# KangWelly/Assignment-for-AAE6102_GNSS-SDR

Hardware: AMD Instinct MI355X
Metric: correlator Msamples/s (acq+track), whole job (higher is better)
Workload: dtype int8 in; acquisition: f64 correlation + f64 fine search; tracking: f64

## Files before the change

### assignment-for-aae6102_gnss-sdr_amd/abi.py

```python
from __future__ import annotations

import ctypes as C
import os
import sys

MAX_SV = 64
MAX_TAPS = 32

OK, ENODATA, EIO, EARG, EDEVICE, EINDEX = 0, 1, 2, 3, 4, 5

FIELDS = ["P_i", "P_q", "E_i", "E_q", "L_i", "L_q", "PLLdiscri", "DLLdiscri", "codedelay",
          "remChip", "codeFreq", "carrierFreq", "remPhase", "remSample", "numSample",
          "delayValue", "absoluteSample", "codedelay2"]
NFIELDS = len(FIELDS)
OUT_DEVICE = 1
FIELDS_POS = ["P_i", "P_q", "E_i", "E_q", "L_i", "L_q", "carrError", "codeError", "codedelay",
              "remChip", "codeFreq", "carrFreq", "remCarrPhase", "absoluteSampleCodedelay",
              "numSample", "delayValue", "absoluteSample", "codedelay2"]

MC_TAPS = 25
MC_TAP_NAMES = ([f"E_{{}}{s}" for s in ["_060", "_055", "", "_045", "_040", "_035", "_030", "_025",
                                         "_020", "_015", "_010", "_005"]] + ["P_{}"] +
                [f"L_{{}}{s}" for s in ["005", "010", "015", "020", "025", "030", "035", "040", "045",
                                         "", "055", "060"]])


EPH_FIELDS = ["TOW", "TOW1", "sfb", "sfb1", "weeknum", "N", "health", "IODC", "TGD", "toc", "af2",
              "af1", "af0", "IODE2", "Crs", "deltan", "M0", "Cuc", "ecc", "Cus", "sqrta", "toe", "Cic",
              "omegae", "Cis", "i0", "Crc", "w", "omegadot", "IODE3", "idot", "updatetime",
              "updatetime_tow"]
EPH_NFIELDS = len(EPH_FIELDS)


class GnssNavOut(C.Structure):
    _fields_ = [("eph_cap", C.c_int32), ("eph", C.POINTER(C.c_double)),
                ("eph_len", C.POINTER(C.c_int32)), ("updateflag", C.POINTER(C.c_int32)),
                ("nav1", C.POINTER(C.c_int64)), ("sfb1", C.POINTER(C.c_int64))]


class GnssFile(C.Structure):
    _fields_ = [("path", C.c_char_p), ("data", C.c_void_p), ("dev_data", C.c_void_p),
                ("nbytes", C.c_uint64), ("skip", C.c_int64), ("dataType", C.c_int32),
                ("dataPrecision", C.c_int32)]


class GnssSignal(C.Structure):
    _fields_ = [("IF", C.c_double), ("Fs", C.c_double), ("codeFreqBasis", C.c_double),
                ("ms", C.c_double), ("Sample", C.c_int64), ("codelength", C.c_double)]


class GnssAcq(C.Structure):
    _fields_ = [("freqNum", C.c_int32), ("freqMin", C.c_double), ("freqStep", C.c_double),
                ("datalen", C.c_int32), ("L", C.c_int32), ("n_prn", C.c_int32),
                ("prn_list", C.POINTER(C.c_int32))]


class GnssAcquired(C.Structure):
    _fields_ = [("n", C.c_int32), ("sv", C.c_int32 * MAX_SV), ("SNR", C.c_double * MAX_SV),
                ("Doppler", C.c_double * MAX_SV), ("codedelay", C.c_int32 * MAX_SV),
                ("fineFreq", C.c_double * MAX_SV)]


class GnssAcqDiag(C.Structure):
    _fields_ = [("n", C.c_int32), ("prn", C.c_int32 * MAX_SV), ("SNR", C.c_double * MAX_SV),
                ("fbin", C.c_int32 * MAX_SV), ("codePhase", C.c_int32 * MAX_SV),
                ("peak", C.c_double * MAX_SV), ("peak2", C.c_double * MAX_SV)]


class GnssTrack(C.Structure):
    _fields_ = [("CorrelatorSpacing", C.c_double), ("DLLBW", C.c_double), ("DLLDamp", C.c_double),
                ("DLLGain", C.c_double), ("PLLBW", C.c_double), ("PLLDamp", C.c_double),
                ("PLLGain", C.c_double), ("msToProcessCT_1ms", C.c_int32),
                ("msToProcessCT_10ms", C.c_int32), ("n_taps", C.c_int32),
                ("tap_offsets", C.POINTER(C.c_double)), ("n_chan", C.c_int32),
                ("chan", C.POINTER(C.c_int32))]


class GnssTrackOut(C.Structure):
    _fields_ = [("max_len", C.c_int64), ("rec", C.POINTER(C.c_double)),
                ("taps", C.POINTER(C.c_double)), ("len", C.POINTER(C.c_int64)),
                ("countinx", C.POINTER(C.c_int32)), ("CN0_Eph", C.POINTER(C.c_double)),
                ("cn0_cap", C.c_int32), ("cn0_rows", C.c_int32), ("flags", C.c_int32),
                ("reserved", C.c_int32)]


class GnssTiming(C.Structure):
    _fields_ = [("acq_ms", C.c_double), ("acq_corr_ms", C.c_double), ("acq_fine_ms", C.c_double),
                ("track_ms", C.c_double), ("track_kernel_ms", C.c_double),
                ("track_launches", C.c_int64), ("track_channel_samples", C.c_int64),
                ("acq_hypothesis_samples", C.c_int64), ("h2d_ms", C.c_double),
                ("track10_kernel_ms", C.c_double), ("track10_launches", C.c_int64),
                ("track10_channel_samples", C.c_int64), ("h2d_bytes", C.c_int64),
                ("track_segments", C.c_int64)]


class GnssVtChan(C.Structure):
    _fields_ = [("prn", C.c_int32), ("pad", C.c_int32), ("file_ptr", C.c_int64), ("remChip", C.c_double),
                ("remCarrPhase", C.c_double), ("codeFreq", C.c_double), ("carrFreq", C.c_double),
                ("carrFreqBasis", C.c_double), ("oldCarrNco", C.c_double), ("oldCarrError", C.c_double),
                ("index_int", C.c_int32), ("snrIndex", C.c_int32), ("Zk", C.c_double * 20)]


class GnssVtOut(C.Structure):
    _fields_ = [(f, C.c_double) for f in ("E_i", "E_q", "P_i", "P_q", "L_i", "L_q", "carrError", "codeError",
                                          "carrNco", "remChip", "remCarrPhase", "codeFreq", "carrFreq")] + \
               [("numSample", C.c_int64), ("absoluteSample", C.c_int64), ("codedelay", C.c_double),
                ("CN0", C.c_double), ("cn0_row", C.c_int32), ("status", C.c_int32),
                ("deltaPr", C.c_double), ("prRate", C.c_double), ("sv_vel", C.c_double * 3)]


class GnssVtMcOut(C.Structure):
    _fields_ = GnssVtOut._fields_ + [("tap_i", C.c_double * MC_TAPS), ("tap_q", C.c_double * MC_TAPS)]


ADDED_STRUCTS = {"gnss_vt_mc_out": "GnssVtMcOut"}

VT_MAX_CH = 32
EPH_SV_FIELDS = ["sqrta", "deltan", "toe", "M0", "ecc", "w", "Cus", "Cuc", "Crs", "Crc", "Cis", "Cic", "i0",
                 "idot", "omegae", "omegadot", "toc", "af0", "af1", "af2", "TGD"]
GEO_XYZ2LLH, GEO_LLH2XYZ, GEO_XYZ2ENU, GEO_EROTCORR, GEO_IONO, GEO_TROP = range(6)


class GnssEphSv(C.Structure):
    _fields_ = [(f, C.c_double) for f in EPH_SV_FIELDS]


class GnssVtNavCfg(C.Structure):
    _fields_ = [("cnslxyz", C.c_double * 3), ("ALPHA", C.c_double * 4), ("BETA", C.c_double * 4),
                ("doy", C.c_double), ("cSpeed", C.c_double), ("Fc", C.c_double)]


class GnssVtNav(C.Structure):
    _fields_ = [("n", C.c_int32), ("pdi", C.c_int32), ("msIndex", C.c_int32), ("counterUptR", C.c_int32),
                ("counter_r", C.c_int32), ("prn", C.c_int32 * VT_MAX_CH), ("cfg", GnssVtNavCfg),
                ("Fs", C.c_double), ("IF", C.c_double), ("codeFreqBasis", C.c_double), ("ms", C.c_double),
                ("cnslxyz", C.c_double * 3), ("total_state", C.c_double * 8), ("state_cov", C.c_double * 64),
                ("R", C.c_double * (2 * VT_MAX_CH)), ("recordR2", C.c_double * (2 * VT_MAX_CH))] + \
               [(f, C.c_double * VT_MAX_CH) for f in ("transmitTime", "tot_est_tck", "predictedPr_last",
                                                     "counter_corr", "ionodel", "tropodel", "el", "az")] + \
               [("numSample", C.c_int64 * VT_MAX_CH), ("eph", GnssEphSv * VT_MAX_CH)]


class GnssVtNavSol(C.Structure):
    _fields_ = [("localTime", C.c_double)] + \
               [(f, C.c_double * 3) for f in ("usrPos", "usrVel", "usrPosENU", "usrVelENU", "usrPosLLH")] + \
               [("clkBias", C.c_double), ("clkDrift", C.c_double), ("state", C.c_double * 8),
                ("state_cov", C.c_double * 8), ("newZ", C.c_double * (2 * VT_MAX_CH)),
                ("meas_inno", C.c_double * (2 * VT_MAX_CH)), ("satEA", C.c_double * VT_MAX_CH),
                ("satAZ", C.c_double * VT_MAX_CH), ("predicted_z", C.c_double * (2 * VT_MAX_CH)),
                ("satePos", C.c_double * 3), ("sateVel", C.c_double * 3),
                ("svxyz_pos", (C.c_double * 3) * VT_MAX_CH), ("kalman_gain", (C.c_double * (2 * VT_MAX_CH)) * 8),
                ("R", C.c_double * (2 * VT_MAX_CH)), ("r_row", C.c_int32),
                ("reserved", C.c_int32)]


ENOCONV = 6
CT_POS_UPDATED, CT_POS_MULTICORR = 0, 1
NAVSOL_CT_FIELDS = [("rawPseudorange", 0), ("usrPos", 3), ("usrVel", 3), ("usrPosENU", 3), ("usrPosLLH", 3),
                    ("clkBias", 1), ("usrVelENU", 3), ("clkDrift", 1), ("DOP", 4), ("satEA", 0), ("satAZ", 0),
                    ("timeTransmit", 0), ("codePhaseMeas", 0), ("localTime", 1)]


class GnssCtPosCfg(C.Structure):
    _fields_ = [("n", C.c_int32), ("mode", C.c_int32), ("dataType", C.c_int32), ("msToProcessCT_1ms", C.c_int32),
                ("pdi", C.c_int32), ("reserved", C.c_int32), ("navSolPeriod", C.c_double), ("Fs", C.c_double),
                ("IF", C.c_double), ("codelength", C.c_double), ("ms", C.c_double), ("cSpeed", C.c_double),
                ("doy", C.c_double), ("cnslxyz", C.c_double * 3), ("ALPHA", C.c_double * 4),
                ("BETA", C.c_double * 4), ("countinx", C.c_int32 * VT_MAX_CH), ("nav1", C.c_int64 * VT_MAX_CH),
                ("sfb1", C.c_int64 * VT_MAX_CH), ("sampleStart", C.c_int64 * VT_MAX_CH),
                ("TOW1", C.c_double * VT_MAX_CH), ("eph", GnssEphSv * VT_MAX_CH)]


class GnssNavSolCt(C.Structure):
    _fields_ = [("cap", C.c_int64), ("rows", C.c_int64)] + \
               [(f, C.POINTER(C.c_double)) for f, _ in NAVSOL_CT_FIELDS] + \
               [("Index", C.POINTER(C.c_int64)), ("index", C.POINTER(C.c_int64)),
                ("carrFreqMeas", C.POINTER(C.c_double)), ("iters", C.POINTER(C.c_int32))]


ADDED_STRUCTS.update({"gnss_ct_pos_cfg": "GnssCtPosCfg", "gnss_nav_sol_ct": "GnssNavSolCt"})

ACF_DEFAULTS = dict(ind_start=1, numOverLap=100, corrSpacing=0.05, maxDelay=0.6,
                    a=(4092.9779845217, 340.423503277404, -2.99026922880033, 0.0251763660254827))
ACF_FIELDS = ["meanMax", "F1", "F2", "varDelay", "meanCodeDisc", "varCodeDisc"]


class GnssAcfCfg(C.Structure):
    _fields_ = [("n", C.c_int32), ("ind_start", C.c_int32), ("numOverLap", C.c_int32), ("reserved", C.c_int32),
                ("corrSpacing", C.c_double), ("maxDelay", C.c_double), ("a", C.c_double * 4),
                ("prn", C.c_int32 * VT_MAX_CH), ("ele", C.c_double * VT_MAX_CH)]


class GnssAcfOut(C.Structure):
    _fields_ = [("cap", C.c_int64), ("windows", C.POINTER(C.c_int64))] + \
               [(f, C.POINTER(C.c_double)) for f in ACF_FIELDS] + \
               [("maxCorrInd", C.c_void_p), ("corr", C.c_void_p)]


ADDED_STRUCTS.update({"gnss_acf_cfg": "GnssAcfCfg", "gnss_acf_out": "GnssAcfOut"})


class GnssSynthSv(C.Structure):
    _fields_ = [("prn", C.c_int32), ("doppler_hz", C.c_double), ("code_phase0", C.c_double),
                ("carr_phase0", C.c_double), ("cn0_dbhz", C.c_double), ("bit_seed", C.c_uint64),
                ("bit_phase_chips", C.c_double), ("lnav", C.c_int32), ("reserved", C.c_int32)]


class GnssSynth(C.Structure):
    _fields_ = [("Fs", C.c_double), ("IF", C.c_double), ("noise_sigma", C.c_double),
                ("seed", C.c_uint64), ("n_sv", C.c_int32), ("sv", GnssSynthSv * MAX_SV)]


MAX_RAYS = 128


class GnssSynthRay(C.Structure):
    _fields_ = [("sv", C.c_int32), ("reserved", C.c_int32), ("delay_chips", C.c_double), ("gain", C.c_double),
                ("phase0_cycles", C.c_double), ("fade_hz", C.c_double), ("t_on", C.c_uint64),
                ("t_off", C.c_uint64)]


class GnssSynthScene(C.Structure):
    _fields_ = [("Fs", C.c_double), ("IF", C.c_double), ("noise_sigma", C.c_double),
                ("seed", C.c_uint64), ("n_sv", C.c_int32), ("sv", GnssSynthSv * MAX_SV),
                ("los_gain", C.c_double * MAX_SV), ("n_ray", C.c_int32), ("ray", GnssSynthRay * MAX_RAYS)]


ADDED_STRUCTS.update({"gnss_synth_ray": "GnssSynthRay", "gnss_synth_scene": "GnssSynthScene"})


PROTOTYPES = {
    "gnss_abi_version": (C.c_int, []),
    "gnss_strerror": (C.c_char_p, [C.c_int]),
    "gnss_ctx_create": (C.c_int, [C.c_int, C.POINTER(C.c_void_p)]),
    "gnss_ctx_create_multi": (C.c_int, [C.POINTER(C.c_int), C.c_int, C.POINTER(C.c_void_p)]),
    "gnss_ctx_members": (C.c_int, [C.c_void_p]),
    "gnss_ctx_drop_record": (C.c_int, [C.c_void_p, C.c_void_p]),
    "gnss_ctx_resident_records": (C.c_int, [C.c_void_p]),
    "gnss_device_count": (C.c_int, []),
    "gnss_ctx_destroy": (None, [C.c_void_p]),
    "gnss_last_error": (C.c_char_p, [C.c_void_p]),
    "gnss_last_timing": (C.c_int, [C.c_void_p, C.POINTER(GnssTiming)]),
    "gnss_ctx_set_profiling": (C.c_int, [C.c_void_p, C.c_int]),
    "gnss_ctx_set_acq_precision": (C.c_int, [C.c_void_p, C.c_int]),
    "gnss_ctx_set_window": (C.c_int, [C.c_void_p, C.c_uint64]),
    "gnss_ctx_set_option": (C.c_int, [C.c_void_p, C.c_int, C.c_int64]),
    "gnss_dev_alloc": (C.c_int, [C.c_void_p, C.c_uint64, C.POINTER(C.c_void_p)]),
    "gnss_dev_free": (C.c_int, [C.c_void_p, C.c_void_p]),
    "gnss_dev_upload": (C.c_int, [C.c_void_p, C.c_void_p, C.c_void_p, C.c_uint64]),
    "gnss_dev_download": (C.c_int, [C.c_void_p, C.c_void_p, C.c_void_p, C.c_uint64]),
    "gnss_acquisition": (C.c_int, [C.c_void_p, C.POINTER(GnssFile), C.POINTER(GnssSignal),
                                   C.POINTER(GnssAcq), C.POINTER(GnssAcquired),
                                   C.POINTER(GnssAcqDiag)]),
    "gnss_tracking_ct": (C.c_int, [C.c_void_p, C.POINTER(GnssFile), C.POINTER(GnssSignal),
                                   C.POINTER(GnssTrack), C.POINTER(GnssAcquired),
                                   C.POINTER(GnssTrackOut)]),
    "gnss_tracking_ct_pos": (C.c_int, [C.c_void_p, C.POINTER(GnssFile), C.POINTER(GnssSignal),
                                       C.POINTER(GnssTrack), C.POINTER(GnssAcquired), C.c_int32,
                                       C.POINTER(C.c_int32), C.POINTER(GnssTrackOut)]),
    "gnss_tracking_ct_mc": (C.c_int, [C.c_void_p, C.POINTER(GnssFile), C.POINTER(GnssSignal),
                                      C.POINTER(GnssTrack), C.POINTER(GnssAcquired), C.c_int32,
                                      C.c_int32, C.POINTER(GnssTrackOut)]),
    "gnss_tracking_ct_multicorr": (C.c_int, [C.c_void_p, C.POINTER(GnssFile), C.POINTER(GnssSignal),
                                             C.POINTER(GnssTrack), C.POINTER(GnssAcquired), C.c_int32,
                                             C.POINTER(GnssTrackOut)]),
    "gnss_navi_decode": (C.c_int, [C.POINTER(GnssAcquired), C.POINTER(C.c_double),
                                   C.POINTER(C.c_int64), C.c_int64, C.POINTER(GnssNavOut)]),
    "gnss_lnav_bits": (C.c_int, [C.c_int32, C.c_int32, C.c_void_p]),
    "gnss_ca_code": (C.c_int, [C.c_int, C.c_void_p]),
    "gnss_correlate_step": (C.c_int, [C.c_void_p, C.POINTER(GnssFile), C.POINTER(GnssSignal),
                                      C.c_int, C.c_int, C.c_double, C.c_double, C.c_double,
                                      C.c_double, C.c_int64, C.c_int, C.POINTER(C.c_double),
                                      C.POINTER(C.c_double), C.POINTER(C.c_int64)]),
    "gnss_synth_if_device": (C.c_int, [C.c_void_p, C.POINTER(GnssSynth), C.c_uint64, C.c_uint64,
                                       C.c_void_p]),
    "gnss_synth_scene_device": (C.c_int, [C.c_void_p, C.POINTER(GnssSynthScene), C.c_uint64, C.c_uint64,
                                          C.c_void_p]),
    "gnss_synth_scene_host": (C.c_int, [C.POINTER(GnssSynthScene), C.c_uint64, C.c_uint64, C.c_void_p, C.c_int]),
    "gnss_tracking_vt_run": (C.c_int, [C.c_void_p, C.POINTER(GnssFile), C.POINTER(GnssSignal),
                                       C.POINTER(GnssTrack), C.c_int32, C.c_int32, C.c_int32,
                                       C.POINTER(GnssVtChan), C.POINTER(C.c_double), C.POINTER(GnssVtOut)]),
    "gnss_tracking_vt_step": (C.c_int, [C.c_void_p, C.POINTER(GnssFile), C.POINTER(GnssSignal),
                                        C.POINTER(GnssTrack), C.c_int32, C.c_int32, C.POINTER(GnssVtChan),
                                        C.POINTER(C.c_double), C.POINTER(GnssVtOut)]),
    "gnss_vt_nco_step": (C.c_int, [C.POINTER(GnssSignal), C.POINTER(GnssTrack), C.c_int32,
                                   C.POINTER(GnssVtChan), C.c_double, C.c_double, C.c_double,
                                   C.POINTER(GnssVtOut)]),
    "gnss_vt_prepare": (C.c_int, [C.POINTER(GnssSignal), C.c_int32, C.POINTER(GnssVtChan), C.c_double,
                                  C.POINTER(C.c_int32), C.POINTER(C.c_int64)]),
    "gnss_sv_pos_vel": (C.c_int, [C.POINTER(GnssEphSv), C.c_double, C.POINTER(C.c_double),
                                  C.POINTER(C.c_double), C.POINTER(C.c_double), C.POINTER(C.c_double),
                                  C.POINTER(C.c_double)]),
    "gnss_geo": (C.c_int, [C.c_int, C.POINTER(C.c_double), C.POINTER(C.c_double)]),
    "gnss_vt_nav_init": (C.c_int, [C.POINTER(GnssVtNavCfg), C.POINTER(GnssSignal), C.c_int32, C.c_int32,
                                   C.POINTER(C.c_int32), C.POINTER(GnssEphSv), C.POINTER(C.c_double),
                                   C.POINTER(C.c_double), C.c_double, C.c_double, C.POINTER(C.c_double),
                                   C.POINTER(GnssVtNav)]),
    "gnss_vt_nav_predict": (C.c_int, [C.POINTER(GnssVtNav), C.c_int32, C.c_int64, C.POINTER(C.c_double),
                                      C.POINTER(C.c_double), C.POINTER(C.c_double)]),
    "gnss_vt_nav_update": (C.c_int, [C.POINTER(GnssVtNav), C.POINTER(C.c_double), C.POINTER(C.c_double),
                                     C.POINTER(C.c_double), C.POINTER(GnssVtNavSol)]),
    "gnss_tracking_vt": (C.c_int, [C.c_void_p, C.POINTER(GnssFile), C.POINTER(GnssSignal), C.POINTER(GnssTrack),
                                   C.c_int32, C.c_int32, C.POINTER(GnssVtChan), C.POINTER(GnssVtNav),
                                   C.POINTER(GnssVtOut), C.POINTER(GnssVtNavSol)]),
    "gnss_tracking_vt_mc_run": (C.c_int, [C.c_void_p, C.POINTER(GnssFile), C.POINTER(GnssSignal),
                                          C.POINTER(GnssTrack), C.c_int32, C.c_int32, C.c_int32,
                                          C.POINTER(GnssVtChan), C.POINTER(C.c_double), C.POINTER(GnssVtMcOut)]),
    "gnss_tracking_vt_mc": (C.c_int, [C.c_void_p, C.POINTER(GnssFile), C.POINTER(GnssSignal), C.POINTER(GnssTrack),
                                      C.c_int32, C.c_int32, C.POINTER(GnssVtChan), C.POINTER(GnssVtNav),
                                      C.POINTER(GnssVtMcOut), C.POINTER(GnssVtNavSol)]),
    "gnss_vt_mc_prepare": (C.c_int, [C.POINTER(GnssSignal), C.c_int32, C.POINTER(GnssVtChan), C.c_double,
                                     C.POINTER(C.c_double), C.POINTER(C.c_double), C.POINTER(C.c_int64)]),
    "gnss_vt_mc_nco_step": (C.c_int, [C.POINTER(GnssSignal), C.POINTER(GnssTrack), C.c_int32,
                                      C.POINTER(GnssVtChan), C.c_double, C.POINTER(C.c_double),
                                      C.POINTER(C.c_double), C.POINTER(GnssVtMcOut)]),
    "gnss_vt_mc_nav_update": (C.c_int, [C.POINTER(GnssVtNav), C.POINTER(C.c_double), C.POINTER(C.c_double),
                                        C.POINTER(C.c_double), C.POINTER(GnssVtNavSol)]),
    "gnss_ct_pos_solve": (C.c_int, [C.c_void_p, C.POINTER(GnssCtPosCfg), C.POINTER(GnssTrackOut),
                                    C.POINTER(GnssNavSolCt)]),
    "gnss_acf_features": (C.c_int, [C.c_void_p, C.POINTER(GnssAcfCfg), C.POINTER(GnssTrackOut), C.c_int32,
                                    C.POINTER(GnssAcfOut)]),
    "gnss_lane_boundaries": (C.c_int, [C.POINTER(C.c_double), C.POINTER(C.c_double), C.c_int, C.c_int, C.c_double]),
    "gnss_ctx_lane_path": (C.c_int, [C.c_void_p]),
}

LIB_PATH = os.path.join(os.path.dirname(os.path.abspath(__file__)), "lib", "libgnss_mi355x.so")
_lib = None
_torch_first = False
LOADED_PATH = None

(OPT_FORCE_SUB, OPT_NO_PERSIST, OPT_FORCE_VPB, OPT_ACQ_ROCFFT, OPT_FINE_ROCFFT, OPT_ACQ_BATCH, OPT_ACQ_FUSED,
 OPT_ACQ_RING, OPT_ACQ_PIPE, OPT_VT_BLOCKS, OPT_FORCE_PEER, OPT_VT_SPAN, OPT_SLOT_PATH) = range(13)
MAX_DEVICES = 16


def require_torch():
    import torch
    if _lib is not None and not _torch_first:
        raise RuntimeError("import torch before the first gnss Context / abi.load() "
                           "(PyTorch-ROCm must bring up its HIP runtime first)")
    return torch


class GnssError(RuntimeError):
    def __init__(self, status, msg=""):
        self.status = status
        super().__init__(f"gnss status {status}: {msg}")


def load(path: str | None = None):
    global _lib
    if _lib is not None and path is None:
        return _lib
    p = path or os.environ.get("GNSS_LIB") or LIB_PATH
    if not os.path.exists(p):
        raise ImportError(f"{p} missing: the HIP extension is not built "
                          "(run `python -c 'import __graft_entry__ as g; g.build()'`)")
    global _torch_first
    if _lib is None:
        if "torch" not in sys.modules and os.environ.get("GNSS_NO_TORCH", "0") != "1":
            try:
                import torch
            except Exception:
                pass
        _torch_first = "torch" in sys.modules
    lib = C.CDLL(p)
    for name, (res, args) in PROTOTYPES.items():
        if p != LIB_PATH and not hasattr(lib, name):
            continue
        fn = getattr(lib, name)
        fn.restype = res
        fn.argtypes = args
    if path is None:
        global LOADED_PATH
        _lib = lib
        LOADED_PATH = os.path.abspath(p)
    return lib
```

### assignment-for-aae6102_gnss-sdr_amd/csrc/acq_fft.hip

```cpp
#include "gnss_internal.h"

#pragma clang fp contract(fast)

namespace gnss {

namespace {

constexpr int kRow = 2000;
constexpr int kRowPad = 2100;
constexpr int kRowThreads = 256;
constexpr int kColThreads = 256;

template <int P> struct PrimeTab;
template <> struct PrimeTab<13> {
    static constexpr double c[13] = {1.0, 0.8854560256532099, 0.5680647467311559, 0.120536680255323, -0.35460488704253545, -0.7485107481711012, -0.970941817426052, -0.9709418174260521, -0.7485107481711013, -0.3546048870425359, 0.1205366802553232, 0.5680647467311548, 0.88545602565321};
    static constexpr double s[13] = {0.0, 0.4647231720437685, 0.8229838658936564, 0.992708874098054, 0.9350162426854148, 0.6631226582407952, 0.23931566428755768, -0.23931566428755743, -0.663122658240795, -0.9350162426854147, -0.992708874098054, -0.822983865893657, -0.4647231720437684};
};
template <> struct PrimeTab<29> {
    static constexpr double c[29] = {1.0, 0.9766205557100867, 0.907575419670957, 0.7960930657056438, 0.6473862847818277, 0.46840844069979015, 0.26752833852922075, 0.05413890858541761, -0.16178199655276473, -0.37013815533991423, -0.5611870653623823, -0.7259954919231306, -0.8568571761675893, -0.9476531711828025, -0.9941379571543596, -0.9941379571543597, -0.9476531711828025, -0.8568571761675892, -0.7259954919231311, -0.5611870653623825, -0.37013815533991445, -0.16178199655276476, 0.0541389085854167, 0.2675283385292201, 0.4684084406997903, 0.6473862847818279, 0.796093065705644, 0.9075754196709569, 0.9766205557100867};
    static constexpr double s[29] = {0.0, 0.21497044021102407, 0.4198891015602646, 0.6051742151937652, 0.7621620551276365, 0.8835120444460229, 0.963549992519223, 0.9985334138511238, 0.9868265225415261, 0.9289767198167915, 0.8276889981568906, 0.6876994588534235, 0.5155538571770216, 0.3193015301359798, 0.10811901842394192, -0.10811901842394124, -0.31930153013597995, -0.5155538571770218, -0.6876994588534231, -0.8276889981568905, -0.9289767198167914, -0.9868265225415261, -0.9985334138511239, -0.9635499925192231, -0.8835120444460228, -0.7621620551276362, -0.6051742151937649, -0.41988910156026493, -0.21497044021102438};
};

template <class V> struct RealOf;
template <> struct RealOf<float2> { using T = float; };
template <> struct RealOf<double2> { using T = double; };
template <class V> using Re = typename RealOf<V>::T;

template <class V> __device__ __forceinline__ V mk(Re<V> x, Re<V> y)
{
    V r;
    r.x = x;
    r.y = y;
    return r;
}
__device__ __forceinline__ float fma2(float a, float b, float cd) { return __builtin_fmaf(a, b, cd); }
__device__ __forceinline__ double fma2(double a, double b, double cd) { return __builtin_fma(a, b, cd); }
template <class V> __device__ __forceinline__ V cadd(V a, V b) { return mk<V>(a.x + b.x, a.y + b.y); }
template <class V> __device__ __forceinline__ V csub(V a, V b) { return mk<V>(a.x - b.x, a.y - b.y); }
template <class V> __device__ __forceinline__ V cmul(V a, V b)
{
    return mk<V>(fma2(a.x, b.x, -(a.y * b.y)), fma2(a.x, b.y, a.y * b.x));
}
template <class V> __device__ __forceinline__ V cmulc(V a, V b)
{
    return mk<V>(fma2(a.x, b.x, a.y * b.y), fma2(a.y, b.x, -(a.x * b.y)));
}
template <int DIR, class V> __device__ __forceinline__ V mul_dj(V a)
{
    return DIR < 0 ? mk<V>(a.y, -a.x) : mk<V>(-a.y, a.x);
}
template <int DIR, class V> __device__ __forceinline__ V twid(V a, V tw)
{
    return DIR < 0 ? cmul(a, tw) : cmulc(a, tw);
}

template <int DIR, class V> __device__ __forceinline__ void dft4(V& a, V& b, V& c, V& d)
{
    const V t0 = cadd(a, c), t1 = csub(a, c), t2 = cadd(b, d), t3 = mul_dj<DIR>(csub(b, d));
    a = cadd(t0, t2);
    c = csub(t0, t2);
    b = cadd(t1, t3);
    d = csub(t1, t3);
}

template <int DIR, class V> __device__ __forceinline__ void dft5(V (&v)[5])
{
    using R = Re<V>;
    constexpr R c1 = (R)0.30901699437494745, c2 = (R)-0.8090169943749475;
    constexpr R s1 = (R)0.9510565162951535, s2 = (R)0.5877852522924731;
    const V t1 = cadd(v[1], v[4]), t2 = cadd(v[2], v[3]);
    const V t3 = csub(v[1], v[4]), t4 = csub(v[2], v[3]);
    const V b1 = mk<V>(v[0].x + c1 * t1.x + c2 * t2.x, v[0].y + c1 * t1.y + c2 * t2.y);
    const V b2 = mk<V>(v[0].x + c2 * t1.x + c1 * t2.x, v[0].y + c2 * t1.y + c1 * t2.y);
    const V e1 = mul_dj<DIR>(mk<V>(fma2(s1, t3.x, s2 * t4.x), fma2(s1, t3.y, s2 * t4.y)));
    const V e2 = mul_dj<DIR>(mk<V>(fma2(s2, t3.x, -(s1 * t4.x)), fma2(s2, t3.y, -(s1 * t4.y))));
    v[0] = mk<V>(v[0].x + t1.x + t2.x, v[0].y + t1.y + t2.y);
    v[1] = cadd(b1, e1);
    v[4] = csub(b1, e1);
    v[2] = cadd(b2, e2);
    v[3] = csub(b2, e2);
}

template <int DIR, class V> __device__ __forceinline__ void dft10(V (&v)[10])
{
    using R = Re<V>;
    constexpr R c[5] = {(R)1.0, (R)0.8090169943749475, (R)0.30901699437494745, (R)-0.30901699437494745,
                        (R)-0.8090169943749475};
    constexpr R s[5] = {(R)0.0, (R)0.5877852522924731, (R)0.9510565162951535, (R)0.9510565162951535,
                        (R)0.5877852522924731};
    V e[5] = {v[0], v[2], v[4], v[6], v[8]}, o[5] = {v[1], v[3], v[5], v[7], v[9]};
    dft5<DIR>(e);
    dft5<DIR>(o);
#pragma unroll
    for (int k = 0; k < 5; k++) {
        const V t = cmul(o[k], mk<V>(c[k], DIR < 0 ? -s[k] : s[k]));
        v[k] = cadd(e[k], t);
        v[k + 5] = csub(e[k], t);
    }
}

constexpr double kC16 = 0.9238795325112867, kS16 = 0.3826834323650898, kR2 = 0.7071067811865476;
constexpr double kTc16[10] = {1., kC16, kR2, kS16, 0., -kS16, -kR2, -kC16, -1., -kC16};
constexpr double kTs16[10] = {0., kS16, kR2, kC16, 1., kC16, kR2, kS16, 0., -kS16};

template <int DIR, class V> __device__ __forceinline__ void dft16(V (&v)[16])
{
    using R = Re<V>;
#pragma unroll
    for (int n2 = 0; n2 < 4; n2++) dft4<DIR>(v[n2], v[4 + n2], v[8 + n2], v[12 + n2]);
#pragma unroll
    for (int k1 = 1; k1 < 4; k1++)
#pragma unroll
        for (int n2 = 1; n2 < 4; n2++) {
            const int m = n2 * k1;
            const V w = mk<V>((R)kTc16[m], DIR < 0 ? (R)-kTs16[m] : (R)kTs16[m]);
            v[4 * k1 + n2] = cmul(v[4 * k1 + n2], w);
        }
    V o[16];
#pragma unroll
    for (int k1 = 0; k1 < 4; k1++) {
        V a = v[4 * k1], b = v[4 * k1 + 1], c = v[4 * k1 + 2], d = v[4 * k1 + 3];
        dft4<DIR>(a, b, c, d);
        o[k1] = a; o[k1 + 4] = b; o[k1 + 8] = c; o[k1 + 12] = d;
    }
#pragma unroll
    for (int i = 0; i < 16; i++) v[i] = o[i];
}

template <int P, int DIR, class V, class Put>
__device__ __forceinline__ void dft_prime(V (&v)[P], Put put)
{
    using R = Re<V>;
    constexpr int H = (P - 1) / 2;
    using T = PrimeTab<P>;
    const V x0 = v[0];
    V sum = x0;
#pragma unroll
    for (int n = 1; n <= H; n++) {
        const V a = cadd(v[n], v[P - n]), d = csub(v[n], v[P - n]);
        v[n] = a;
        v[P - n] = d;
        sum = cadd(sum, a);
    }
    put(0, sum);
#pragma unroll
    for (int k = 1; k <= H; k++) {
        R re = x0.x, im = x0.y, sr = 0, si = 0;
#pragma unroll
        for (int n = 1; n <= H; n++) {
            const int m = (n * k) % P;
            re += v[n].x * (R)T::c[m];
            im += v[n].y * (R)T::c[m];
            sr += v[P - n].y * (R)T::s[m];
            si += v[P - n].x * (R)T::s[m];
        }
        if (DIR < 0) {
            put(k, mk<V>(re + sr, im - si));
            put(P - k, mk<V>(re - sr, im + si));
        } else {
            put(k, mk<V>(re - sr, im + si));
            put(P - k, mk<V>(re + sr, im - si));
        }
    }
}

template <int DIR, int NS, class V, class TW>
__device__ __forceinline__ void stage5(V* a, const TW& tw, int tid)
{
    constexpr int NB = kRow / 5, PER = (NB + kRowThreads - 1) / kRowThreads;
    V v[PER][5];
#pragma unroll
    for (int q = 0; q < PER; q++) {
        const int j0 = tid + q * kRowThreads, j = j0 < NB ? j0 : NB - 1;
        const int k = j % NS;
#pragma unroll
        for (int i = 0; i < 5; i++) v[q][i] = a[j + i * NB];
        if (NS > 1) {
#pragma unroll
            for (int i = 1; i < 5; i++) v[q][i] = twid<DIR>(v[q][i], tw[i * k * (kRow / (NS * 5))]);
        }
        dft5<DIR>(v[q]);
    }
    __syncthreads();
#pragma unroll
    for (int q = 0; q < PER; q++) {
        const int j = tid + q * kRowThreads;
        if (j < NB) {
            const int k = j % NS, d = (j / NS) * NS * 5 + k;
#pragma unroll
            for (int i = 0; i < 5; i++) a[d + i * NS] = v[q][i];
        }
    }
    __syncthreads();
}

template <int DIR, class V, class TW>
__device__ __forceinline__ void fft2000(V* a, const TW& tw, int tid)
{
    stage5<DIR, 1>(a, tw, tid);
    stage5<DIR, 5>(a, tw, tid);
    stage5<DIR, 25>(a, tw, tid);
    constexpr int NB = kRow / 16;
    const int j = tid < NB ? tid : NB - 1;
    V v[16];
#pragma unroll
    for (int i = 0; i < 16; i++) v[i] = a[j + i * NB];
#pragma unroll
    for (int i = 1; i < 16; i++) v[i] = twid<DIR>(v[i], tw[i * j]);
    dft16<DIR>(v);
    __syncthreads();
    if (tid < NB) {
#pragma unroll
        for (int i = 0; i < 16; i++) a[tid + i * NB] = v[i];
    }
    __syncthreads();
}

constexpr double kTc20[13] = {1., 0.9510565162951535, 0.8090169943749475, 0.5877852522924731,
                              0.30901699437494745, 0., -0.30901699437494745, -0.5877852522924731,
                              -0.8090169943749475, -0.9510565162951535, -1., -0.9510565162951535,
                              -0.8090169943749475};
constexpr double kTs20[13] = {0., 0.30901699437494745, 0.5877852522924731, 0.8090169943749475,
                              0.9510565162951535, 1., 0.9510565162951535, 0.8090169943749475,
                              0.5877852522924731, 0.30901699437494745, 0., -0.30901699437494745,
                              -0.5877852522924731};
template <int DIR, class V> __device__ __forceinline__ void dft20(V (&v)[20])
{
    using R = Re<V>;
    V y[4][5];
#pragma unroll
    for (int n2 = 0; n2 < 4; n2++) {
#pragma unroll
        for (int n1 = 0; n1 < 5; n1++) y[n2][n1] = v[4 * n1 + n2];
        dft5<DIR>(y[n2]);
    }
#pragma unroll
    for (int n2 = 1; n2 < 4; n2++)
#pragma unroll
        for (int k1 = 1; k1 < 5; k1++) {
            const int m = n2 * k1;
            y[n2][k1] = cmul(y[n2][k1], mk<V>((R)kTc20[m], DIR < 0 ? (R)-kTs20[m] : (R)kTs20[m]));
        }
#pragma unroll
    for (int k1 = 0; k1 < 5; k1++) {
        V a = y[0][k1], b = y[1][k1], c = y[2][k1], d = y[3][k1];
        dft4<DIR>(a, b, c, d);
        v[k1] = a; v[k1 + 5] = b; v[k1 + 10] = c; v[k1 + 15] = d;
    }
}

template <int R, int DIR, class V> __device__ __forceinline__ void dft_r(V (&v)[R])
{
    if constexpr (R == 5) dft5<DIR>(v);
    else if constexpr (R == 10) dft10<DIR>(v);
    else if constexpr (R == 16) dft16<DIR>(v);
    else dft20<DIR>(v);
}

template <class V> struct TwIK {
    const V* t2;
    const V* t3;
};
template <int NS, class V>
__device__ __forceinline__ V tw_get(const V* tw, int, int, int m) { return tw[m]; }
template <int NS, class V>
__device__ __forceinline__ V tw_get(const TwIK<V>& tw, int i, int k, int m)
{
    static_assert(NS == 20 || NS == 200, "split twiddles: the radix-20-first stages");
    return NS == 20 ? tw.t2[(i - 1) * 20 + k] : tw.t3[(i - 1) * 200 + k];
}
constexpr int kTwIK = 9 * 20 + 9 * 200;
#ifndef GNSS_STAGED_LOADS
#define GNSS_STAGED_LOADS 1
#endif
template <class V>
__device__ __forceinline__ TwIK<V> load_row_tw_ik(V* s_t, const V* tw_row, int tid)
{
    auto src = [&](int e) {
        const bool t2 = e < 9 * 20;
        const int f = t2 ? e : e - 9 * 20;
        const int i = t2 ? f / 20 + 1 : f / 200 + 1, k = t2 ? f % 20 : f % 200;
        return t2 ? 10 * i * k : i * k;
    };
    if constexpr (GNSS_STAGED_LOADS) {
        constexpr int NIT = (kTwIK + kRowThreads - 1) / kRowThreads;
        V r[NIT];
#pragma unroll
        for (int q = 0; q < NIT; q++) {
            const int e0 = tid + q * kRowThreads;
            r[q] = tw_row[src(e0 < kTwIK ? e0 : kTwIK - 1)];
        }
#pragma unroll
        for (int q = 0; q < NIT; q++)
            if (tid + q * kRowThreads < kTwIK) s_t[tid + q * kRowThreads] = r[q];
    } else {
        for (int e = tid; e < kTwIK; e += kRowThreads) s_t[e] = tw_row[src(e)];
    }
    return TwIK<V>{s_t, s_t + 9 * 20};
}

template <int DIR, int R, int NS, int BATCH, class V, class TW, int SW = 0>
__device__ __forceinline__ void stage_batch(V* a, const TW& tw, int tid)
{
    constexpr int NB = kRow / R, TOT = NB * BATCH, PER = (TOT + kRowThreads - 1) / kRowThreads;
    static_assert(SW == 0 || (BATCH == 1 && ((SW == 1 && R == 20 && NS == 1) || (SW == 2 && R == 10 && NS == 20))),
                  "padded layout");
    V v[PER][R];
#pragma unroll
    for (int q = 0; q < PER; q++) {
        const int u0 = tid + q * kRowThreads, u = u0 < TOT ? u0 : TOT - 1;
        const int b = u / NB, j = u - b * NB, k = j % NS;
        const V* src = a + b * kRow;
        if constexpr (SW == 2) {
            const V* s0 = src + j + j / 20;
#pragma unroll
            for (int i = 0; i < R; i++) v[q][i] = s0[210 * i];
        } else {
#pragma unroll
            for (int i = 0; i < R; i++) v[q][i] = src[j + i * NB];
        }
        if constexpr (NS > 1) {
#pragma unroll
            for (int i = 1; i < R; i++) v[q][i] = twid<DIR>(v[q][i], tw_get<NS>(tw, i, k, i * k * (kRow / (NS * R))));
        }
        dft_r<R, DIR>(v[q]);
    }
    __syncthreads();
#pragma unroll
    for (int q = 0; q < PER; q++) {
        const int u = tid + q * kRowThreads;
        if (u < TOT) {
            const int b = u / NB, j = u - b * NB, k = j % NS, d = (j / NS) * NS * R + k;
            V* dst = a + b * kRow;
            if constexpr (SW == 1) {
#pragma unroll
                for (int i = 0; i < R; i++) dst[d + j + i] = v[q][i];
            } else {
#pragma unroll
                for (int i = 0; i < R; i++) dst[d + i * NS] = v[q][i];
            }
        }
    }
    __syncthreads();
}

template <int DIR, int BATCH, class V, class TW>
__device__ __forceinline__ void fft2000_batch(V* a, const TW& tw, int tid)
{
    stage_batch<DIR, 10, 1, BATCH>(a, tw, tid);
    stage_batch<DIR, 10, 10, BATCH>(a, tw, tid);
    stage_batch<DIR, 20, 100, BATCH>(a, tw, tid);
}

constexpr int kR20Out = 10;
template <int DIR, class V, class TW, class Put>
__device__ __forceinline__ void fft2000_r20first_put(V* a, const TW& tw, int tid, Put put)
{
    stage_batch<DIR, 20, 1, 1, V, TW, 1>(a, tw, tid);
    stage_batch<DIR, 10, 20, 1, V, TW, 2>(a, tw, tid);
    constexpr int R = 10, NB = kRow / R;
    const bool on = tid < NB;
    const int j = on ? tid : NB - 1;
    V v[R];
#pragma unroll
    for (int i = 0; i < R; i++) v[i] = a[j + i * NB];
#pragma unroll
    for (int i = 1; i < R; i++) v[i] = twid<DIR>(v[i], tw_get<NB>(tw, i, j, i * j));
    dft10<DIR>(v);
    if (on) {
#pragma unroll
        for (int i = 0; i < R; i++) put(i, j + i * NB, v[i]);
    }
    __syncthreads();
}

constexpr int kInvOut = kR20Out;
template <class TW>
__device__ __forceinline__ void inv_row_power_f64(double2* a, const TW& s_tw, double scale,
                                                  double (&acc)[kInvOut], int tid)
{
    fft2000_r20first_put<1>(a, s_tw, tid, [&](int i, int, double2 v) {
        acc[i] = __builtin_fma(__builtin_fma(v.x, v.x, v.y * v.y), scale, acc[i]);
    });
}

__device__ __forceinline__ double2 ld_nt(const double2* p)
{
    double2 v;
    v.x = __builtin_nontemporal_load(&p->x);
    v.y = __builtin_nontemporal_load(&p->y);
    return v;
}

template <class V>
__device__ __forceinline__ void load_row_tw(V* s_tw, const V* tw_row, int tid)
{
    for (int i = tid; i < kRow; i += kRowThreads) s_tw[i] = tw_row[i];
}


struct FwdSet {
    int nbins, nsig, nprn, bin0, nbc, codes;
    __device__ __forceinline__ int transform(int y) const
    {
        if (codes && y < nprn) return nsig + y;
        const int u = y - (codes ? nprn : 0), idx = u / nbc;
        return idx * nbins + bin0 + (u - idx * nbc);
    }
};

template <int P, class Src, class V>
__global__ __launch_bounds__(kRowThreads) void fwd_rows_kernel(
    const Src src, FwdSet fs, double IF, double freqMin, double freqStep,
    double Fs, const float* __restrict__ ca, double code_step, const V* __restrict__ tw_row,
    const V* __restrict__ tw_col, V* __restrict__ B)
{
    using R = Re<V>;
    constexpr int64_t S = (int64_t)P * kRow;
    __shared__ V s_a[kRowPad], s_tw[kTwIK];
    const int nbins = fs.nbins, nsig = fs.nsig;
    const int n2 = blockIdx.x, s = fs.transform(blockIdx.y), tid = threadIdx.x;
    const TwIK<V> twk = load_row_tw_ik(s_tw, tw_row, tid);
    constexpr int NIT = (kRow + kRowThreads - 1) / kRowThreads;
    if (s < nsig) {
        const int idx = s / nbins, bin = s - idx * nbins;
        const double f = (IF + (freqMin + freqStep * (double)bin)) / Fs;
        auto put = [&](int n1, double2 r) {
            const int64_t n = (int64_t)P * n1 + n2;
            double cyc = f * (double)(n + 1);
            cyc -= floor(cyc);
            R c, sn;
            if constexpr (sizeof(R) == 4) {
                const float ph = (float)cyc;
                c = __builtin_amdgcn_cosf(ph);
                sn = __builtin_amdgcn_sinf(ph);
            } else {
                sincospi(2.0 * cyc, &sn, &c);
            }
            const R xr = (R)r.x, xi = (R)r.y;
            s_a[n1] = mk<V>(fma2(xr, c, -(xi * sn)), fma2(xr, sn, xi * c));
        };
        if constexpr (GNSS_STAGED_LOADS) {
            double2 raw[NIT];
#pragma unroll
            for (int q = 0; q < NIT; q++) {
                const int m0 = tid + q * kRowThreads, n1 = m0 < kRow ? m0 : kRow - 1;
                raw[q] = src.at((int64_t)idx * S + (int64_t)P * n1 + n2);
            }
#pragma unroll
            for (int q = 0; q < NIT; q++)
                if (tid + q * kRowThreads < kRow) put(tid + q * kRowThreads, raw[q]);
        } else {
            for (int n1 = tid; n1 < kRow; n1 += kRowThreads) put(n1, src.at((int64_t)idx * S + (int64_t)P * n1 + n2));
        }
    } else {
        const float* cp = ca + (int64_t)(s - nsig) * 1023;
        auto chip = [&](int n1) {
            const int64_t n = (int64_t)P * n1 + n2;
            const int64_t ci = (int64_t)ceil((double)(n + 1) * code_step);
            return (ci - 1) % 1023;
        };
        if constexpr (GNSS_STAGED_LOADS) {
            float cv[NIT];
#pragma unroll
            for (int q = 0; q < NIT; q++) {
                const int m0 = tid + q * kRowThreads;
                cv[q] = cp[chip(m0 < kRow ? m0 : kRow - 1)];
            }
#pragma unroll
            for (int q = 0; q < NIT; q++)
                if (tid + q * kRowThreads < kRow) s_a[tid + q * kRowThreads] = mk<V>((R)cv[q], (R)0);
        } else {
            for (int n1 = tid; n1 < kRow; n1 += kRowThreads) s_a[n1] = mk<V>((R)cp[chip(n1)], (R)0);
        }
    }
    __syncthreads();
    V* o = B + ((int64_t)s * P + n2) * kRow;
    const V* twc = tw_col + (int64_t)n2 * kRow;
    fft2000_r20first_put<-1>(s_a, twk, tid, [&](int, int k1, V v) { o[k1] = cmul(v, twc[k1]); });
}

template <int P, class V>
__global__ __launch_bounds__(kColThreads) void fwd_cols_kernel(FwdSet fs, const V* __restrict__ B, V* __restrict__ X)
{
    const int k1 = blockIdx.x * kColThreads + threadIdx.x, s = fs.transform(blockIdx.y);
    if (k1 >= kRow) return;
    const V* b = B + (int64_t)s * P * kRow + k1;
    V v[P];
#pragma unroll
    for (int i = 0; i < P; i++) v[i] = b[(int64_t)i * kRow];
    V* x = X + (int64_t)s * P * kRow + k1;
    dft_prime<P, -1>(v, [&](int k, V y) { x[(int64_t)k * kRow] = y; });
}

template <class V> __device__ __forceinline__ V buf_ld(__amdgpu_buffer_rsrc_t r, int voff, int soff);
template <> __device__ __forceinline__ double2 buf_ld<double2>(__amdgpu_buffer_rsrc_t r, int voff, int soff)
{
    typedef unsigned u4 __attribute__((ext_vector_type(4)));
    const u4 v = __builtin_amdgcn_raw_buffer_load_b128(r, voff, soff, 0);
    return make_double2(__hiloint2double((int)v.y, (int)v.x), __hiloint2double((int)v.w, (int)v.z));
}
template <> __device__ __forceinline__ float2 buf_ld<float2>(__amdgpu_buffer_rsrc_t r, int voff, int soff)
{
    typedef unsigned u2 __attribute__((ext_vector_type(2)));
    const u2 v = __builtin_amdgcn_raw_buffer_load_b64(r, voff, soff, 0);
    return make_float2(__uint_as_float(v.x), __uint_as_float(v.y));
}
#ifndef GNSS_COLS_BUF
#define GNSS_COLS_BUF 1
#endif
#ifndef GNSS_COLS_GROUP
#define GNSS_COLS_GROUP 8
#endif
#ifndef GNSS_TW_ROWS
#define GNSS_TW_ROWS 1
#endif
#ifndef GNSS_INVCOLS_WPE
#define GNSS_INVCOLS_WPE 0
#endif
template <int P, class V>
__device__ __forceinline__ void inv_cols_body(
    int bx, int t, const V* __restrict__ C, const V* __restrict__ X, int nbins, int nprn, int datalen,
    int first_pair, const V* __restrict__ tw_col, V* __restrict__ A)
{
    const int k1 = bx * kColThreads + threadIdx.x;
    if (k1 >= kRow) return;
    const int q = first_pair + t / datalen, idx = t % datalen;
    const int bin = q / nprn, p = q - bin * nprn;
    V v[P];
    if (GNSS_COLS_BUF == 2) {
        constexpr int kB = P * kRow * (int)sizeof(V), G = GNSS_COLS_GROUP;
        const __amdgpu_buffer_rsrc_t rc = __builtin_amdgcn_make_buffer_rsrc(
            (void*)(C + (int64_t)p * P * kRow), (short)0, kB, 0x00020000);
        const __amdgpu_buffer_rsrc_t rx = __builtin_amdgcn_make_buffer_rsrc(
            (void*)(X + ((int64_t)idx * nbins + bin) * P * kRow), (short)0, kB, 0x00020000);
        const int vo = k1 * (int)sizeof(V);
        V ca[G], xa[G];
#pragma unroll
        for (int i = 0; i < G; i++) {
            const int r = (i < P ? i : P - 1) * kRow * (int)sizeof(V);
            ca[i] = buf_ld<V>(rc, vo, r);
            xa[i] = buf_ld<V>(rx, vo, r);
        }
#pragma unroll
        for (int g = 0; g < P; g += G) {
            V cb[G], xb[G];
#pragma unroll
            for (int i = 0; i < G; i++)
                if (g + G + i < P) {
                    cb[i] = buf_ld<V>(rc, vo, (g + G + i) * kRow * (int)sizeof(V));
                    xb[i] = buf_ld<V>(rx, vo, (g + G + i) * kRow * (int)sizeof(V));
                }
            __builtin_amdgcn_sched_barrier(0);
#pragma unroll
            for (int i = 0; i < G; i++)
                if (g + i < P) v[g + i] = cmulc(ca[i], xa[i]);
#pragma unroll
            for (int i = 0; i < G; i++) { ca[i] = cb[i]; xa[i] = xb[i]; }
        }
    } else if (GNSS_COLS_BUF) {
        constexpr int kB = P * kRow * (int)sizeof(V), G = GNSS_COLS_GROUP;
        const __amdgpu_buffer_rsrc_t rc = __builtin_amdgcn_make_buffer_rsrc(
            (void*)(C + (int64_t)p * P * kRow), (short)0, kB, 0x00020000);
        const __amdgpu_buffer_rsrc_t rx = __builtin_amdgcn_make_buffer_rsrc(
            (void*)(X + ((int64_t)idx * nbins + bin) * P * kRow), (short)0, kB, 0x00020000);
        const int vo = k1 * (int)sizeof(V);
#pragma unroll
        for (int i = 0; i < P; i++) v[i] = buf_ld<V>(rc, vo, i * kRow * (int)sizeof(V));
        V xa[G];
#pragma unroll
        for (int i = 0; i < G; i++) xa[i] = buf_ld<V>(rx, vo, (i < P ? i : P - 1) * kRow * (int)sizeof(V));
#pragma unroll
        for (int g = 0; g < P; g += G) {
            V xb[G];
#pragma unroll
            for (int i = 0; i < G; i++)
                if (g + G + i < P) xb[i] = buf_ld<V>(rx, vo, (g + G + i) * kRow * (int)sizeof(V));
            __builtin_amdgcn_sched_barrier(0);
#pragma unroll
            for (int i = 0; i < G; i++)
                if (g + i < P) v[g + i] = cmulc(v[g + i], xa[i]);
#pragma unroll
            for (int i = 0; i < G; i++) xa[i] = xb[i];
        }
    } else {
        const V* c = C + (int64_t)p * P * kRow + k1;
        const V* x = X + ((int64_t)idx * nbins + bin) * P * kRow + k1;
#pragma unroll
        for (int i = 0; i < P; i++) v[i] = cmulc(c[(int64_t)i * kRow], x[(int64_t)i * kRow]);
    }
    V* a = A + (int64_t)t * P * kRow + k1;
    const V* tw = tw_col + k1;
    dft_prime<P, 1>(v, [&](int k, V y) {
        const V z = GNSS_TW_ROWS ? y : cmulc(y, tw[(int64_t)k * kRow]);
        __builtin_nontemporal_store(z.x, &a[(int64_t)k * kRow].x);
        __builtin_nontemporal_store(z.y, &a[(int64_t)k * kRow].y);
    });
}

template <int P, class V>
__global__ __launch_bounds__(kColThreads)
#if GNSS_INVCOLS_WPE > 0
__attribute__((amdgpu_waves_per_eu(GNSS_INVCOLS_WPE, GNSS_INVCOLS_WPE)))
#endif
void inv_cols_kernel(
    const V* __restrict__ C, const V* __restrict__ X, int nbins, int nprn, int datalen,
    int first_pair, const V* __restrict__ tw_col, V* __restrict__ A)
{
    inv_cols_body<P, V>(blockIdx.x, blockIdx.y, C, X, nbins, nprn, datalen, first_pair, tw_col, A);
}

template <int P>
__global__ __launch_bounds__(kRowThreads) void inv_rows_kernel(
    const float2* __restrict__ A, int nprn, int datalen, int first_pair, float scale,
    const float2* __restrict__ tw_row, const float2* __restrict__ tw_col, float* __restrict__ corr, int nbins)
{
    constexpr int Q = (kRow + kRowThreads - 1) / kRowThreads;
    constexpr int V4 = kRow / 2;
    constexpr int QV = (V4 + kRowThreads - 1) / kRowThreads;
    static_assert(QV == 4, "row copy is written for 4 float4 per lane");
    __shared__ float4 s_a4[2 * V4];
    __shared__ float2 s_tw[kRow];
    float2* s_a = reinterpret_cast<float2*>(s_a4);
    const int tau2 = blockIdx.x, g = blockIdx.y, tid = threadIdx.x;
    load_row_tw(s_tw, tw_row, tid);
    float acc[Q];
#pragma unroll
    for (int i = 0; i < Q; i++) acc[i] = 0.f;
    const float4* src = reinterpret_cast<const float4*>(A + ((int64_t)g * datalen * P + tau2) * kRow);
    auto ld = [&](int idx, int i) {
        const int e = tid + i * kRowThreads;
        const int r = idx < datalen ? idx : datalen - 1;
        const float4* q = src + (int64_t)r * P * V4 + (e < V4 ? e : V4 - 1);
        float4 v;
        v.x = __builtin_nontemporal_load(&q->x);
        v.y = __builtin_nontemporal_load(&q->y);
        v.z = __builtin_nontemporal_load(&q->z);
        v.w = __builtin_nontemporal_load(&q->w);
        return v;
    };
    float4 tw4[QV];
#pragma unroll
    for (int i = 0; i < QV; i++) {
        const int e = tid + i * kRowThreads;
        tw4[i] = reinterpret_cast<const float4*>(tw_col + (int64_t)tau2 * kRow)[e < V4 ? e : V4 - 1];
    }
    auto st = [&](int h, int i, float4 v) {
        const int e = tid + i * kRowThreads;
        if (GNSS_TW_ROWS) {
            const float2 lo = cmulc(make_float2(v.x, v.y), make_float2(tw4[i].x, tw4[i].y));
            const float2 hi = cmulc(make_float2(v.z, v.w), make_float2(tw4[i].z, tw4[i].w));
            v = make_float4(lo.x, lo.y, hi.x, hi.y);
        }
        if (e < V4) s_a4[h * V4 + e] = v;
    };
    float4 a0 = ld(0, 0), a1 = ld(0, 1), a2 = ld(0, 2), a3 = ld(0, 3);
    float4 b0 = ld(1, 0), b1 = ld(1, 1), b2 = ld(1, 2), b3 = ld(1, 3);
    for (int idx = 0; idx < datalen; idx += 2) {
        st(0, 0, a0); st(0, 1, a1); st(0, 2, a2); st(0, 3, a3);
        st(1, 0, b0); st(1, 1, b1); st(1, 2, b2); st(1, 3, b3);
        if (idx + 2 < datalen) {
            a0 = ld(idx + 2, 0); a1 = ld(idx + 2, 1); a2 = ld(idx + 2, 2); a3 = ld(idx + 2, 3);
            b0 = ld(idx + 3, 0); b1 = ld(idx + 3, 1); b2 = ld(idx + 3, 2); b3 = ld(idx + 3, 3);
        }
        __syncthreads();
        fft2000_batch<1, 2>(s_a, s_tw, tid);
        const bool second = idx + 1 < datalen;
#pragma unroll
        for (int i = 0; i < Q; i++) {
            const int t1 = tid + i * kRowThreads, t = t1 < kRow ? t1 : kRow - 1;
            const float2 v = s_a[t], w = s_a[kRow + t];
            acc[i] += fma2(v.x, v.x, v.y * v.y) * scale;
            if (second) acc[i] += fma2(w.x, w.x, w.y * w.y) * scale;
        }
        __syncthreads();
    }
    const int q = first_pair + g;
    const int bin = q / nprn, p = q - bin * nprn;
    float* o = corr + (((int64_t)p * nbins + bin) * P + tau2) * kRow;
#pragma unroll
    for (int i = 0; i < Q; i++) {
        const int t1 = tid + i * kRowThreads;
        if (t1 < kRow) o[t1] = acc[i];
    }
}

template <int P>
__device__ __forceinline__ void inv_rows_f64_body(
    int tau2, int g, const double2* __restrict__ A, int nprn, int datalen, int first_pair, double scale,
    const double2* __restrict__ tw_row, const double2* __restrict__ tw_col, double* __restrict__ corr, int nbins)
{
    constexpr int Q = (kRow + kRowThreads - 1) / kRowThreads;
    __shared__ double2 s_a[kRowPad], s_tw[kTwIK];
    const int tid = threadIdx.x;
    const TwIK<double2> twk = load_row_tw_ik(s_tw, tw_row, tid);
    double acc[kInvOut];
#pragma unroll
    for (int i = 0; i < kInvOut; i++) acc[i] = 0.0;
    const double2* src = A + ((int64_t)g * datalen * P + tau2) * kRow;
    static_assert(Q == 8, "row prefetch is written for 8 values per lane");
    const int e7 = tid + 7 * kRowThreads < kRow ? tid + 7 * kRowThreads : kRow - 1;
    double2 n0, n1, n2, n3, n4, n5, n6, n7;
#define GNSS_LD(IDX)                                                                         \
    {                                                                                        \
        const double2* r = src + (int64_t)(IDX) * P * kRow + tid;                              \
        n0 = ld_nt(r); n1 = ld_nt(r + kRowThreads); n2 = ld_nt(r + 2 * kRowThreads);           \
        n3 = ld_nt(r + 3 * kRowThreads); n4 = ld_nt(r + 4 * kRowThreads);                      \
        n5 = ld_nt(r + 5 * kRowThreads); n6 = ld_nt(r + 6 * kRowThreads); n7 = ld_nt(r + e7 - tid); \
    }
    double2 w0, w1, w2, w3, w4, w5, w6, w7;
    if (GNSS_TW_ROWS) {
        const double2* t = tw_col + (int64_t)tau2 * kRow + tid;
        w0 = t[0]; w1 = t[kRowThreads]; w2 = t[2 * kRowThreads]; w3 = t[3 * kRowThreads];
        w4 = t[4 * kRowThreads]; w5 = t[5 * kRowThreads]; w6 = t[6 * kRowThreads]; w7 = t[e7 - tid];
    }
    GNSS_LD(0)
    for (int idx = 0; idx < datalen; idx++) {
        if (GNSS_TW_ROWS) {
            n0 = cmulc(n0, w0); n1 = cmulc(n1, w1); n2 = cmulc(n2, w2); n3 = cmulc(n3, w3);
            n4 = cmulc(n4, w4); n5 = cmulc(n5, w5); n6 = cmulc(n6, w6); n7 = cmulc(n7, w7);
        }
        s_a[tid] = n0; s_a[tid + kRowThreads] = n1; s_a[tid + 2 * kRowThreads] = n2;
        s_a[tid + 3 * kRowThreads] = n3; s_a[tid + 4 * kRowThreads] = n4;
        s_a[tid + 5 * kRowThreads] = n5; s_a[tid + 6 * kRowThreads] = n6;
        if (tid + 7 * kRowThreads < kRow) s_a[tid + 7 * kRowThreads] = n7;
        if (idx + 1 < datalen) GNSS_LD(idx + 1)
#undef GNSS_LD
        __syncthreads();
        inv_row_power_f64(s_a, twk, scale, acc, tid);
    }
    const int q = first_pair + g;
    const int bin = q / nprn, p = q - bin * nprn;
    double* o = corr + (((int64_t)p * nbins + bin) * P + tau2) * kRow;
    if (tid < kRow / kInvOut) {
#pragma unroll
        for (int i = 0; i < kInvOut; i++) o[tid + i * (kRow / kInvOut)] = acc[i];
    }
}

template <int P>
__global__ __launch_bounds__(kRowThreads) void inv_rows_kernel_f64(
    const double2* __restrict__ A, int nprn, int datalen, int first_pair, double scale,
    const double2* __restrict__ tw_row, const double2* __restrict__ tw_col, double* __restrict__ corr, int nbins)
{
    inv_rows_f64_body<P>(blockIdx.x, blockIdx.y, A, nprn, datalen, first_pair, scale, tw_row, tw_col, corr, nbins);
}

template <int P>
__global__ __launch_bounds__(kRowThreads) void inv_pair_kernel_f64(
    const double2* __restrict__ C, const double2* __restrict__ X, int nbins, int nprn, int datalen,
    int cols_first, int cols_n, double2* __restrict__ Acols, int rows_first, int rows_n,
    const double2* __restrict__ Arows, double scale, const double2* __restrict__ tw_row,
    const double2* __restrict__ tw_col, double* __restrict__ corr, int front)
{
    constexpr int kCx = (kRow + kColThreads - 1) / kColThreads;
    const int64_t nr = (int64_t)P * rows_n, T = nr + (int64_t)kCx * cols_n * datalen;
    const int64_t F = nr ? std::max<int64_t>(nr, T * front / 100) : 1;
    const int64_t i = blockIdx.x;
    const int64_t r0 = i < F ? i * nr / F : nr, r1 = i < F ? (i + 1) * nr / F : nr;
    if (r1 > r0) {
        const int g = (int)(r0 / P), tau2 = (int)(r0 - (int64_t)g * P);
        inv_rows_f64_body<P>(tau2, g, Arows, nprn, datalen, rows_first, scale, tw_row, tw_col, corr, nbins);
    } else {
        const int c = (int)(i - r0), t = c / kCx;
        inv_cols_body<P, double2>(c - t * kCx, t, C, X, nbins, nprn, datalen, cols_first, tw_col, Acols);
    }
}

constexpr int kFuseX = 8;
constexpr int kFuseSlots = 4;
constexpr int kFuseLine = 32;
constexpr int kFuseChunks = (kRow + kColThreads - 1) / kColThreads;
constexpr unsigned kFuseSpin = 1u << 22;
struct FuseSync {
    unsigned arrive[kFuseX * kFuseLine];
    unsigned total[kFuseLine];
    unsigned err[kFuseLine];
    unsigned ready[kFuseX * kFuseSlots * kFuseLine];
    unsigned freed[kFuseX * kFuseSlots * kFuseLine];
};

__device__ __forceinline__ unsigned ld_sc1(const unsigned* p)
{
    return __hip_atomic_load(p, __ATOMIC_RELAXED, __HIP_MEMORY_SCOPE_AGENT);
}
__device__ __forceinline__ unsigned add_dev(unsigned* p, unsigned v)
{
    return __hip_atomic_fetch_add(p, v, __ATOMIC_RELAXED, __HIP_MEMORY_SCOPE_AGENT);
}
__device__ __forceinline__ bool wait_ge(const unsigned* p, unsigned want, FuseSync* sy)
{
    for (unsigned n = 0; n < kFuseSpin; n++) {
        if (ld_sc1(p) >= want) return true;
        if (ld_sc1(sy->err)) return false;
        __builtin_amdgcn_s_sleep(8);
    }
    add_dev(sy->err, 1u);
    return false;
}

template <int P>
__global__ __launch_bounds__(kRowThreads, 2) void inv_fused_kernel_f64(
    const double2* __restrict__ C, const double2* __restrict__ X, int nbins, int nprn, int datalen,
    int npairs, int nslot, double scale, const double2* __restrict__ tw_row, const double2* __restrict__ tw_col,
    double2* __restrict__ ring, FuseSync* __restrict__ sy, double* __restrict__ corr)
{
    constexpr int Q = (kRow + kRowThreads - 1) / kRowThreads;
    constexpr int64_t S = (int64_t)P * kRow;
    __shared__ double2 s_a[kRowPad], s_tw[kTwIK];
    __shared__ int s_role[6];
    const int tid = threadIdx.x;
    if (tid == 0) {
        unsigned xcc;
        asm volatile("s_getreg_b32 %0, hwreg(HW_REG_XCC_ID, 0, 4)" : "=s"(xcc));
        xcc &= kFuseX - 1;
        const unsigned rank = add_dev(&sy->arrive[xcc * kFuseLine], 1u);
        add_dev(sy->total, 1u);
        int ok = wait_ge(sy->total, gridDim.x, sy) ? 1 : 0;
        int na = 0, xa = -1, nw = 0;
        for (int x = 0; x < kFuseX; x++) {
            const int w = (int)ld_sc1(&sy->arrive[x * kFuseLine]);
            if (w >= P + 4) {
                if (x == (int)xcc) { xa = na; nw = w; }
                na++;
            }
        }
        if (na == 0) ok = 0;
        if (!ok && rank == 0 && xcc == 0) add_dev(sy->err, 1u);
        s_role[0] = (int)xcc; s_role[1] = (int)rank; s_role[2] = nw; s_role[3] = xa; s_role[4] = na;
        s_role[5] = ok;
    }
    __syncthreads();
    const int xcc = s_role[0], rank = s_role[1], nw = s_role[2], xa = s_role[3], na = s_role[4];
    if (!s_role[5] || xa < 0) return;
    const int nr = P, nc = nw - P;
    const int npx = (npairs - xa + na - 1) / na;
    const int ntr = npx * datalen;
    unsigned* ready = &sy->ready[xcc * kFuseSlots * kFuseLine];
    unsigned* freed = &sy->freed[xcc * kFuseSlots * kFuseLine];
    double2* ring_x = ring + (int64_t)xcc * kFuseSlots * S;

    if (rank >= nr) {
        const int w = rank - nr;
        for (int it = w; it < ntr * kFuseChunks; it += nc) {
            const int j = it / kFuseChunks, ch = it - j * kFuseChunks, slot = j % nslot;
            if (tid == 0) s_role[5] = wait_ge(&freed[slot * kFuseLine], (unsigned)(j / nslot * nr), sy);
            __syncthreads();
            if (!s_role[5]) return;
            const int pi = j / datalen, ms = j - pi * datalen;
            const int q = xa + pi * na, bin = q / nprn, p = q - bin * nprn;
            const int k1 = ch * kColThreads + tid;
            if (k1 < kRow) {
                const double2* c = C + (int64_t)p * S + k1;
                const double2* x = X + ((int64_t)ms * nbins + bin) * S + k1;
                double2 v[P];
#pragma unroll
                for (int i = 0; i < P; i++) v[i] = cmulc(c[(int64_t)i * kRow], ld_nt(x + (int64_t)i * kRow));
                double2* a = ring_x + (int64_t)slot * S + k1;
                const double2* tw = tw_col + k1;
                dft_prime<P, 1>(v, [&](int k, double2 y) {
                    a[(int64_t)k * kRow] = GNSS_TW_ROWS ? y : cmulc(y, tw[(int64_t)k * kRow]);
                });
            }
            asm volatile("s_waitcnt vmcnt(0)" ::: "memory");
            __syncthreads();
            if (tid == 0) add_dev(&ready[slot * kFuseLine], 1u);
        }
        return;
    }
    const int tau2 = rank;
    const TwIK<double2> twk = load_row_tw_ik(s_tw, tw_row, tid);
    double acc[kInvOut];
#pragma unroll
    for (int i = 0; i < kInvOut; i++) acc[i] = 0.0;
    const __amdgpu_buffer_rsrc_t rs = __builtin_amdgcn_make_buffer_rsrc(
        ring_x, (short)0, (int)(kFuseSlots * S * sizeof(double2)), 0x00020000);
    for (int j = 0; j < ntr; j++) {
        const int slot = j % nslot;
        if (tid == 0) s_role[5] = wait_ge(&ready[slot * kFuseLine], (unsigned)((j / nslot + 1) * kFuseChunks), sy);
        __syncthreads();
        if (!s_role[5]) return;
        const int row0 = (int)(((int64_t)slot * S + (int64_t)tau2 * kRow) * 16);
#pragma unroll
        for (int i = 0; i < Q; i++) {
            const int e = tid + i * kRowThreads;
            if (e < kRow) {
                typedef unsigned u4 __attribute__((ext_vector_type(4)));
                const u4 v = __builtin_amdgcn_raw_buffer_load_b128(rs, row0 + e * 16, 0, 16 );
                const double2 y = make_double2(__hiloint2double((int)v.y, (int)v.x), __hiloint2double((int)v.w, (int)v.z));
                s_a[e] = GNSS_TW_ROWS ? cmulc(y, tw_col[(int64_t)tau2 * kRow + e]) : y;
            }
        }
        __syncthreads();
        if (tid == 0) add_dev(&freed[slot * kFuseLine], 1u);
        inv_row_power_f64(s_a, twk, scale, acc, tid);
        const int pi = j / datalen, ms = j - pi * datalen;
        if (ms == datalen - 1) {
            const int q = xa + pi * na, bin = q / nprn, p = q - bin * nprn;
            double* o = corr + (((int64_t)p * nbins + bin) * P + tau2) * kRow;
#pragma unroll
            for (int i = 0; i < kInvOut; i++) {
                if (tid < kRow / kInvOut) o[tid + i * (kRow / kInvOut)] = acc[i];
                acc[i] = 0.0;
            }
        }
    }
}


constexpr int kFineT = 10;
constexpr int kFineJC = 16;

__global__ void fine_twiddle_kernel(double2* __restrict__ t, int64_t len, int64_t div, int64_t row)
{
    const int64_t x = (int64_t)blockIdx.x * blockDim.x + threadIdx.x;
    if (x >= len) return;
    const int64_t m = row ? (x / row) * (x % row) : x;
    double s, c;
    sincospi(-2.0 * (double)m / (double)div, &s, &c);
    t[x] = make_double2(c, s);
}

__global__ void fine_twik_kernel(const double2* __restrict__ tw_row, double2* __restrict__ t)
{
    const int e = blockIdx.x * blockDim.x + threadIdx.x;
    if (e >= kTwIK) return;
    const bool t2 = e < 9 * 20;
    const int f = t2 ? e : e - 9 * 20;
    const int i = t2 ? f / 20 + 1 : f / 200 + 1, k = t2 ? f % 20 : f % 200;
    t[e] = tw_row[t2 ? 10 * i * k : i * k];
}

__device__ __forceinline__ int64_t fine_code_of(int64_t n, double invFs, double invFc, double codelength)
{
    const double cvi = floor((invFs * (double)(n + 1)) / invFc);
    return (int64_t)fmod(cvi, codelength);
}

#ifndef GNSS_FINE_PREP
#define GNSS_FINE_PREP 1
#endif
#ifndef GNSS_FINE_TWIK
#define GNSS_FINE_TWIK 1
#endif
template <class Src> struct SrcElem;
template <> struct SrcElem<SrcIQ8> {
    using T = char2;
    static constexpr int kTM = 32;
    __device__ static T get(const SrcIQ8& s, int64_t n) { return reinterpret_cast<const char2*>(s.p)[n]; }
    static SrcIQ8 wrap(const T* p) { return SrcIQ8{reinterpret_cast<const int8_t*>(p)}; }
};
template <> struct SrcElem<SrcC64> {
    using T = double2;
    static constexpr int kTM = 8;
    __device__ static T get(const SrcC64& s, int64_t n) { return s.p[n]; }
    static SrcC64 wrap(const T* p) { return SrcC64{p}; }
};
template <int P, class Src>
__global__ __launch_bounds__(kRowThreads) void fine_prep_kernel(
    const Src src, const int32_t* __restrict__ cd, int64_t S, double invFs, double invFc, double codelength,
    const float* __restrict__ ca0, typename SrcElem<Src>::T* __restrict__ xt0, float* __restrict__ ct0)
{
    using T = typename SrcElem<Src>::T;
    constexpr int PT = P * kFineT, TM = SrcElem<Src>::kTM;
    constexpr int64_t M = (int64_t)PT * kRow;
    __shared__ T s_x[TM * PT];
    __shared__ float s_c[TM * PT];
    const float* ca = ca0 + (int64_t)blockIdx.y * 1023;
    const int m0 = blockIdx.x * TM, tid = threadIdx.x;
    const int tm = kRow - m0 < TM ? kRow - m0 : TM;
    const int64_t base = S - cd[blockIdx.y] - 1, n0 = (int64_t)PT * m0;
    for (int e = tid; e < tm * PT; e += kRowThreads) {
        s_x[e] = SrcElem<Src>::get(src, base + n0 + e);
        s_c[e] = ca[fine_code_of(n0 + e, invFs, invFc, codelength)];
    }
    __syncthreads();
    T* xt = xt0 + (int64_t)blockIdx.y * M;
    float* ct = ct0 + (int64_t)blockIdx.y * M;
    for (int e = tid; e < tm * PT; e += kRowThreads) {
        const int rho = e / tm, c = e - rho * tm;
        xt[(int64_t)rho * kRow + m0 + c] = s_x[c * PT + rho];
        ct[(int64_t)rho * kRow + m0 + c] = s_c[c * PT + rho];
    }
}

template <int P, class Src>
__global__ __launch_bounds__(kRowThreads) void fine_rows_kernel(
    const Src src, const float* __restrict__ ct, const int32_t* __restrict__ cd, int64_t S,
    const float* __restrict__ ca0, double invFs, double invFc, double codelength, int D, int64_t N,
    const double2* __restrict__ tw_row, const double2* __restrict__ twik, const double2* __restrict__ tabA,
    const double2* __restrict__ tabB, double2* __restrict__ E0)
{
    constexpr int T = kFineT;
    const int64_t base = S - cd[blockIdx.z] - 1;
    const float* ca = ca0 + (int64_t)blockIdx.z * 1023;
    double2* E = E0 + (int64_t)blockIdx.z * N;
    __shared__ double2 s_a[kRowPad];
    const int rho = blockIdx.x, r = blockIdx.y, tid = threadIdx.x;
    const int m2 = rho / P, n2 = rho - m2 * P;
    auto sample = [&](int m1) { return (int64_t)P * T * m1 + (int64_t)P * m2 + n2; };
    auto code_of = [&](int64_t n) { return fine_code_of(n, invFs, invFc, codelength); };
    if constexpr (GNSS_FINE_PREP) {
        constexpr int NIT = (kRow + kRowThreads - 1) / kRowThreads;
        const int64_t row0 = ((int64_t)blockIdx.z * P * T + rho) * kRow;
        double2 raw[NIT], ta[NIT];
        float cv[NIT];
#pragma unroll
        for (int q = 0; q < NIT; q++) {
            const int m10 = tid + q * kRowThreads, m1 = m10 < kRow ? m10 : kRow - 1;
            cv[q] = ct[row0 + m1];
            raw[q] = src.at(row0 + m1);
            ta[q] = tabA[(int64_t)r * kRow + m1];
        }
#pragma unroll
        for (int q = 0; q < NIT; q++) {
            const int m1 = tid + q * kRowThreads;
            const double code = (double)cv[q];
            const double2 x = make_double2(raw[q].x * code, raw[q].y * code);
            if (m1 < kRow) s_a[m1] = cmul(x, ta[q]);
        }
    } else if constexpr (GNSS_STAGED_LOADS) {
        constexpr int NIT = (kRow + kRowThreads - 1) / kRowThreads;
        double2 raw[NIT], ta[NIT];
        float cv[NIT];
#pragma unroll
        for (int q = 0; q < NIT; q++) {
            const int m10 = tid + q * kRowThreads, m1 = m10 < kRow ? m10 : kRow - 1;
            const int64_t n = sample(m1);
            cv[q] = ca[code_of(n)];
            raw[q] = src.at(base + n);
            ta[q] = tabA[(int64_t)r * kRow + m1];
        }
#pragma unroll
        for (int q = 0; q < NIT; q++) {
            const int m1 = tid + q * kRowThreads;
            const double code = (double)cv[q];
            const double2 x = make_double2(raw[q].x * code, raw[q].y * code);
            if (m1 < kRow) s_a[m1] = cmul(x, ta[q]);
        }
    } else {
        for (int m1 = tid; m1 < kRow; m1 += kRowThreads) {
            const int64_t n = sample(m1);
            const double code = (double)ca[code_of(n)];
            const double2 raw = src.at(base + n);
            const double2 x = make_double2(raw.x * code, raw.y * code);
            s_a[m1] = cmul(x, tabA[(int64_t)r * kRow + m1]);
        }
    }
    __syncthreads();
    double sn, cs;
    const int64_t e = ((int64_t)(P * m2 + n2) * r) % N;
    sincospi(-2.0 * (double)e / (double)N, &sn, &cs);
    const double2 cb = make_double2(cs, sn);
    double2* o = E + (((int64_t)r * P + n2) * T + m2) * kRow;
    const double2* tb = tabB + m2 * kRow;
    auto put = [&](int, int j1, double2 v) { o[j1] = cmul(cmul(v, cb), tb[j1]); };
    if constexpr (GNSS_FINE_TWIK)
        fft2000_r20first_put<-1>(s_a, TwIK<double2>{twik, twik + 9 * 20}, tid, put);
    else
        fft2000_r20first_put<-1>(s_a, tw_row, tid, put);
}

struct FineBest {
    double m;
    int64_t i;
};

__device__ __forceinline__ void best_merge(double& m, int64_t& i, double m2, int64_t i2)
{
    if (m2 > m || (m2 == m && i2 < i)) { m = m2; i = i2; }
}

template <int P>
__global__ __launch_bounds__(kColThreads) void fine_cols_kernel(
    const double2* __restrict__ E0, int D, int64_t N, int shifted, const double2* __restrict__ tabK,
    const double2* __restrict__ tabS, FineBest* __restrict__ part0)
{
    constexpr int T = kFineT, JC = kFineJC;
    const double2* E = E0 + (int64_t)blockIdx.z * N;
    FineBest* part = part0 + (int64_t)blockIdx.z * gridDim.x * gridDim.y;
    static_assert(P * T * JC * sizeof(double2) + (kColThreads / 64) * sizeof(double) * 2 <= 80 * 1024,
                  "fine_cols LDS tile: two blocks per CU of gfx950's 160 KiB");
    __shared__ double2 s_e[P * T * JC];
    __shared__ FineBest s_b[kColThreads / 64];
    const int r = blockIdx.y, j10 = blockIdx.x * JC, tid = threadIdx.x;
    auto at = [&](int e) {
        const int jj = e % JC, nm = e / JC;
        return E + ((int64_t)r * P * T + nm) * kRow + j10 + jj;
    };
    if constexpr (GNSS_STAGED_LOADS) {
        constexpr int NE = P * T * JC, NIT = (NE + kColThreads - 1) / kColThreads;
        double2 st[NIT];
#pragma unroll
        for (int q = 0; q < NIT; q++) {
            const int e0 = tid + q * kColThreads;
            st[q] = *at(e0 < NE ? e0 : NE - 1);
        }
#pragma unroll
        for (int q = 0; q < NIT; q++)
            if (tid + q * kColThreads < NE) s_e[tid + q * kColThreads] = st[q];
    } else {
        for (int e = tid; e < P * T * JC; e += kColThreads) s_e[e] = *at(e);
    }
    __syncthreads();
    for (int pr = tid; pr < P * JC; pr += kColThreads) {
        const int n2 = pr / JC, jj = pr - n2 * JC;
        double2 v[T];
#pragma unroll
        for (int m2 = 0; m2 < T; m2++) v[m2] = s_e[(n2 * T + m2) * JC + jj];
        dft10<-1>(v);
        const double2 tk = tabK[n2 * kRow + j10 + jj];
#pragma unroll
        for (int j2 = 0; j2 < T; j2++)
            s_e[(n2 * T + j2) * JC + jj] = cmul(v[j2], j2 ? cmul(tk, tabS[(n2 * j2) % (P * T)]) : tk);
    }
    __syncthreads();
    double bm = -1.0;
    int64_t bi = INT64_MAX;
    const int64_t half = N / 2;
    for (int pr = tid; pr < T * JC; pr += kColThreads) {
        const int j2 = pr / JC, jj = pr - j2 * JC;
        double2 v[P];
#pragma unroll
        for (int n2 = 0; n2 < P; n2++) v[n2] = s_e[(n2 * T + j2) * JC + jj];
        const int64_t k1 = j10 + jj + (int64_t)kRow * j2;
        dft_prime<P, -1>(v, [&](int k2, double2 y) {
            const int64_t q = k1 + (int64_t)T * kRow * k2;
            const int64_t k = (int64_t)D * q + r;
            int64_t i = k;
            if (shifted == 1) { i = k + half; if (i >= N) i -= N; }
            else if (shifted == 2 && N - k < k) i = N - k;
            best_merge(bm, bi, hypot(y.x, y.y), i);
        });
    }
#pragma unroll
    for (int o = 32; o > 0; o >>= 1) {
        const double m2 = __shfl_xor(bm, o, 64);
        const int64_t i2 = __shfl_xor(bi, o, 64);
        best_merge(bm, bi, m2, i2);
    }
    if ((tid & 63) == 0) s_b[tid >> 6] = FineBest{bm, bi};
    __syncthreads();
    if (tid == 0) {
        for (int w = 1; w < kColThreads / 64; w++) best_merge(bm, bi, s_b[w].m, s_b[w].i);
        part[(int64_t)r * gridDim.x + blockIdx.x] = FineBest{bm, bi};
    }
}

__global__ void fine_best_final_kernel(const FineBest* __restrict__ part0, int nblk,
                                       int64_t* __restrict__ kbest0)
{
    const FineBest* part = part0 + (int64_t)blockIdx.x * nblk;
    int64_t* kbest = kbest0 + blockIdx.x;
    double bm = -1.0;
    int64_t bi = INT64_MAX;
    for (int k = threadIdx.x; k < nblk; k += blockDim.x) best_merge(bm, bi, part[k].m, part[k].i);
#pragma unroll
    for (int o = 32; o > 0; o >>= 1) {
        const double m2 = __shfl_xor(bm, o, 64);
        const int64_t i2 = __shfl_xor(bi, o, 64);
        best_merge(bm, bi, m2, i2);
    }
    __shared__ FineBest s_b[4];
    if ((threadIdx.x & 63) == 0) s_b[threadIdx.x >> 6] = FineBest{bm, bi};
    __syncthreads();
    if (threadIdx.x == 0) {
        for (int w = 1; w < (int)(blockDim.x >> 6); w++) best_merge(bm, bi, s_b[w].m, s_b[w].i);
        *kbest = bi + 1;
    }
}

}

bool acq_fft_supported(int64_t S) { return S == 13 * kRow || S == 29 * kRow; }

template <class V>
hipError_t launch_acq_fft_forward(const int8_t* iq, const double2* xs, int64_t S, int datalen, int nbins,
                                  double IF, double freqMin, double freqStep, double Fs, const float* ca,
                                  int nprn, double codeFreqBasis, const V* tw_row,
                                  const V* tw_col, V* B, V* X, hipStream_t s, int bin0, int nbc, bool codes)
{
    const int nsig = datalen * nbins;
    if (nbc < 0) nbc = nbins - bin0;
    if (bin0 < 0 || nbc < 0 || bin0 + nbc > nbins) return hipErrorInvalidValue;
    const FwdSet fs{nbins, nsig, nprn, bin0, nbc > 0 ? nbc : 1, codes ? 1 : 0};
    const int ntr = (codes ? nprn : 0) + datalen * nbc;
    if (ntr == 0) return hipSuccess;
    const double step = codeFreqBasis / Fs;
#define GNSS_FWD(P_)                                                                            \
    if (S == (int64_t)P_ * kRow) {                                                              \
        if (xs)                                                                                 \
            hipLaunchKernelGGL((fwd_rows_kernel<P_, SrcC64, V>), dim3(P_, ntr), dim3(kRowThreads), 0, s, \
                               SrcC64{xs}, fs, IF, freqMin, freqStep, Fs, ca, step, tw_row, tw_col, B); \
        else                                                                                    \
            hipLaunchKernelGGL((fwd_rows_kernel<P_, SrcIQ8, V>), dim3(P_, ntr), dim3(kRowThreads), 0, s, \
                               SrcIQ8{iq}, fs, IF, freqMin, freqStep, Fs, ca, step, tw_row, tw_col, B); \
        hipLaunchKernelGGL((fwd_cols_kernel<P_, V>), dim3((kRow + kColThreads - 1) / kColThreads, ntr), \
                           dim3(kColThreads), 0, s, fs, B, X);                                  \
        return hipGetLastError();                                                               \
    }
    GNSS_FWD(13) GNSS_FWD(29)
#undef GNSS_FWD
    return hipErrorInvalidValue;
}
template hipError_t launch_acq_fft_forward<float2>(const int8_t*, const double2*, int64_t, int, int, double,
                                                   double, double, double, const float*, int, double,
                                                   const float2*, const float2*, float2*, float2*, hipStream_t, int,
                                                   int, bool);
template hipError_t launch_acq_fft_forward<double2>(const int8_t*, const double2*, int64_t, int, int, double,
                                                    double, double, double, const float*, int, double,
                                                    const double2*, const double2*, double2*, double2*,
                                                    hipStream_t, int, int, bool);

hipError_t launch_acq_fft_correlate(const float2* C, const float2* X, int64_t S, int datalen,
                                    int nbins, int nprn, int first_pair, int npair,
                                    const float2* tw_row, const float2* tw_col, float2* A,
                                    float* corr, hipStream_t s, int parts)
{
    const float scale = (float)(1.0 / ((double)S * (double)S));
#define GNSS_INV(P_)                                                                            \
    if (S == (int64_t)P_ * kRow) {                                                              \
        if (parts & kAcqCols)                                                                   \
        hipLaunchKernelGGL((inv_cols_kernel<P_, float2>),                                       \
                           dim3((kRow + kColThreads - 1) / kColThreads, npair * datalen),       \
                           dim3(kColThreads), 0, s, C, X, nbins, nprn, datalen, first_pair,     \
                           tw_col, A);                                                          \
        if (parts & kAcqRows)                                                                   \
        hipLaunchKernelGGL(inv_rows_kernel<P_>, dim3(P_, npair), dim3(kRowThreads), 0, s, A, nprn, \
                           datalen, first_pair, scale, tw_row, tw_col, corr, nbins);            \
        return hipGetLastError();                                                               \
    }
    GNSS_INV(13) GNSS_INV(29)
#undef GNSS_INV
    return hipErrorInvalidValue;
}

hipError_t launch_acq_fft_correlate(const double2* C, const double2* X, int64_t S, int datalen,
                                    int nbins, int nprn, int first_pair, int npair,
                                    const double2* tw_row, const double2* tw_col, double2* A,
                                    double* corr, hipStream_t s, int parts)
{
    const double scale = 1.0 / ((double)S * (double)S);
#define GNSS_INV(P_)                                                                            \
    if (S == (int64_t)P_ * kRow) {                                                              \
        if (parts & kAcqCols)                                                                   \
        hipLaunchKernelGGL((inv_cols_kernel<P_, double2>),                                      \
                           dim3((kRow + kColThreads - 1) / kColThreads, npair * datalen),       \
                           dim3(kColThreads), 0, s, C, X, nbins, nprn, datalen, first_pair,     \
                           tw_col, A);                                                          \
        if (parts & kAcqRows)                                                                   \
        hipLaunchKernelGGL(inv_rows_kernel_f64<P_>, dim3(P_, npair), dim3(kRowThreads), 0, s, A, nprn, \
                           datalen, first_pair, scale, tw_row, tw_col, corr, nbins);            \
        return hipGetLastError();                                                               \
    }
    GNSS_INV(13) GNSS_INV(29)
#undef GNSS_INV
    return hipErrorInvalidValue;
}

hipError_t launch_acq_fft_pair(const double2* C, const double2* X, int64_t S, int datalen, int nbins, int nprn,
                               int cols_first, int cols_n, double2* Acols, int rows_first, int rows_n,
                               const double2* Arows, const double2* tw_row, const double2* tw_col, double* corr,
                               int front, hipStream_t s)
{
    if (front < 1 || front > 100 || cols_n < 0 || rows_n < 0) return hipErrorInvalidValue;
    const double scale = 1.0 / ((double)S * (double)S);
    constexpr int kCx = (kRow + kColThreads - 1) / kColThreads;
#define GNSS_PAIR(P_)                                                                           \
    if (S == (int64_t)P_ * kRow) {                                                              \
        const int64_t nblk = (int64_t)P_ * rows_n + (int64_t)kCx * cols_n * datalen;             \
        if (nblk == 0) return hipSuccess;                                                       \
        if (nblk > INT32_MAX) return hipErrorInvalidConfiguration;                              \
        hipLaunchKernelGGL(inv_pair_kernel_f64<P_>, dim3((unsigned)nblk), dim3(kRowThreads), 0, s, C, X, nbins, \
                           nprn, datalen, cols_first, cols_n, Acols, rows_first, rows_n, Arows, scale, tw_row, \
                           tw_col, corr, front);                                                \
        return hipGetLastError();                                                               \
    }
    static_assert(kColThreads == kRowThreads, "the paired launch runs both bodies in one block shape");
    GNSS_PAIR(13) GNSS_PAIR(29)
#undef GNSS_PAIR
    return hipErrorInvalidValue;
}

size_t acq_fused_sync_bytes() { return sizeof(FuseSync); }
size_t acq_fused_err_offset() { return offsetof(FuseSync, err); }
size_t acq_fused_ring_bytes(int64_t S) { return sizeof(double2) * (size_t)kFuseX * kFuseSlots * (size_t)S; }

hipError_t launch_acq_fft_correlate_fused(const double2* C, const double2* X, int64_t S, int datalen, int nbins,
                                          int nprn, int nslot, const double2* tw_row, const double2* tw_col,
                                          double2* ring, void* sync, double* corr, hipStream_t s)
{
    if (nslot < 2 || nslot > kFuseSlots) return hipErrorInvalidValue;
    const double scale = 1.0 / ((double)S * (double)S);
    int dev = 0, ncu = 0;
    hipError_t e = hipGetDevice(&dev);
    if (e == hipSuccess) e = hipDeviceGetAttribute(&ncu, hipDeviceAttributeMultiprocessorCount, dev);
    if (e == hipSuccess) e = hipMemsetAsync(sync, 0, sizeof(FuseSync), s);
    if (e != hipSuccess) return e;
    FuseSync* sy = static_cast<FuseSync*>(sync);
#define GNSS_FUSED(P_)                                                                          \
    if (S == (int64_t)P_ * kRow) {                                                              \
        int occ = 0;                                                                            \
        e = hipOccupancyMaxActiveBlocksPerMultiprocessor(&occ, inv_fused_kernel_f64<P_>, kRowThreads, 0); \
        if (e != hipSuccess) return e;                                                          \
        const int grid = ncu * std::min(occ, 2);                                                \
        if (grid < 1) return hipErrorInvalidConfiguration;                                      \
        hipLaunchKernelGGL(inv_fused_kernel_f64<P_>, dim3(grid), dim3(kRowThreads), 0, s, C, X, nbins, nprn, \
                           datalen, nbins * nprn, nslot, scale, tw_row, tw_col, ring, sy, corr); \
        return hipGetLastError();                                                               \
    }
    GNSS_FUSED(13) GNSS_FUSED(29)
#undef GNSS_FUSED
    return hipErrorInvalidValue;
}

bool fine_fft_supported(int64_t S, int L) { return acq_fft_supported(S) && L == kFineT; }

namespace {
struct FineLayout {
    int64_t M, N, tabs, slab, part;
};
FineLayout fine_layout(int64_t S, int L, int datalen)
{
    FineLayout f;
    f.M = (int64_t)L * S;
    f.N = f.M * datalen;
    f.tabs = kRow + (int64_t)kRow * datalen + (int64_t)kFineT * kRow + S + f.M / kRow + kTwIK;
    f.slab = f.N;
    f.part = (int64_t)datalen * (kRow / kFineJC);
    return f;
}
}

static size_t fine_prep_offset(const FineLayout& f, int nsv)
{
    const size_t b = sizeof(double2) * (size_t)(f.tabs + (int64_t)nsv * f.slab) + sizeof(FineBest) * (size_t)(nsv * f.part);
    return (b + 255) & ~(size_t)255;
}
size_t fine_fft_scratch_bytes(int64_t S, int L, int datalen, int nsv)
{
    const FineLayout f = fine_layout(S, L, datalen);
    if (!GNSS_FINE_PREP) return fine_prep_offset(f, nsv);
    return fine_prep_offset(f, nsv) + (size_t)nsv * f.M * (sizeof(double2) + sizeof(float));
}

hipError_t launch_fine_fft_tables(int64_t S, int L, int datalen, void* scratch, hipStream_t s)
{
    const int64_t M = (int64_t)L * S;
    double2* tw_row = static_cast<double2*>(scratch);
    double2* tabA = tw_row + kRow;
    double2* tabB = tabA + (int64_t)kRow * datalen;
    double2* tabK = tabB + (int64_t)kFineT * kRow;
    double2* tabS = tabK + S;
    const int64_t lens[5] = {kRow, (int64_t)kRow * datalen, (int64_t)kFineT * kRow, S, M / kRow};
    const int64_t divs[5] = {kRow, (int64_t)kRow * datalen, (int64_t)kFineT * kRow, M, M / kRow};
    const int64_t rows[5] = {0, kRow, kRow, kRow, 0};
    double2* tabs[5] = {tw_row, tabA, tabB, tabK, tabS};
    for (int t = 0; t < 5; t++)
        hipLaunchKernelGGL(fine_twiddle_kernel, dim3((unsigned)((lens[t] + 255) / 256)), dim3(256), 0,
                           s, tabs[t], lens[t], divs[t], rows[t]);
    hipLaunchKernelGGL(fine_twik_kernel, dim3((kTwIK + 255) / 256), dim3(256), 0, s, tw_row, tabS + M / kRow);
    return hipGetLastError();
}

hipError_t launch_fine_fft_argmax(const int8_t* iq, const double2* xs, int64_t S, int L, int datalen,
                                  const int32_t* cd, int nsv, const float* ca, double Fs, double codeFreqBasis,
                                  double codelength, int shifted, void* scratch, int64_t* kbest, hipStream_t s)
{
    if (nsv < 1 || nsv > 65535) return hipErrorInvalidValue;
    const FineLayout f = fine_layout(S, L, datalen);
    const int64_t N = f.N;
    double2* tw_row = static_cast<double2*>(scratch);
    double2* tabA = tw_row + kRow;
    double2* tabB = tabA + (int64_t)kRow * datalen;
    double2* tabK = tabB + (int64_t)kFineT * kRow;
    double2* tabS = tabK + S;
    double2* E = tw_row + f.tabs;
    FineBest* part = reinterpret_cast<FineBest*>(E + (int64_t)nsv * f.slab);
    char* prep = static_cast<char*>(scratch) + fine_prep_offset(f, nsv);
    float* ct = reinterpret_cast<float*>(prep + (size_t)nsv * f.M * sizeof(double2));
    const int nblk = kRow / kFineJC;
    auto rows = [&](auto src, auto* xt, auto kern, auto prep_kern, int tm) {
        using SrcT = decltype(src);
        if (GNSS_FINE_PREP) {
            hipLaunchKernelGGL(prep_kern, dim3((kRow + tm - 1) / tm, nsv), dim3(kRowThreads), 0, s, src, cd, S, 1 / Fs,
                               1 / codeFreqBasis, codelength, ca, xt, ct);
            src = SrcElem<SrcT>::wrap(xt);
        }
        hipLaunchKernelGGL(kern, dim3((unsigned)(f.M / kRow), datalen, nsv), dim3(kRowThreads), 0, s, src, ct, cd, S,
                           ca, 1 / Fs, 1 / codeFreqBasis, codelength, datalen, N, tw_row, tabS + f.M / kRow, tabA,
                           tabB, E);
    };
#define GNSS_FINE(P_)                                                                           \
    if (S == (int64_t)P_ * kRow) {                                                              \
        if (xs)                                                                                 \
            rows(SrcC64{xs}, reinterpret_cast<double2*>(prep), fine_rows_kernel<P_, SrcC64>,    \
                 fine_prep_kernel<P_, SrcC64>, SrcElem<SrcC64>::kTM);                           \
        else                                                                                    \
            rows(SrcIQ8{iq}, reinterpret_cast<char2*>(prep), fine_rows_kernel<P_, SrcIQ8>,      \
                 fine_prep_kernel<P_, SrcIQ8>, SrcElem<SrcIQ8>::kTM);                           \
        hipLaunchKernelGGL(fine_cols_kernel<P_>, dim3(nblk, datalen, nsv), dim3(kColThreads), 0, s, E, \
                           datalen, N, shifted, tabK, tabS, part);                                    \
        hipLaunchKernelGGL(fine_best_final_kernel, dim3(nsv), dim3(256), 0, s, part, nblk * datalen, \
                           kbest);                                                              \
        return hipGetLastError();                                                               \
    }
    GNSS_FINE(13) GNSS_FINE(29)
#undef GNSS_FINE
    return hipErrorInvalidValue;
}

}
```

### assignment-for-aae6102_gnss-sdr_amd/csrc/api_acq.cpp

```cpp
#include <cmath>
#include <cstring>
#include <vector>

#include "host.h"

using namespace gnss;
using namespace gnss::host;

namespace {
constexpr int kAcqPipeDefault = 2;
#ifndef GNSS_ACQ_FWD_SPLIT
#define GNSS_ACQ_FWD_SPLIT 1
#endif
constexpr bool kAcqFwdSplit = GNSS_ACQ_FWD_SPLIT;
constexpr int kAcqPairFront = 60;
constexpr int kFineBatch = 16;

template <class V> struct CplxReal;
template <> struct CplxReal<float2> { using T = float; };
template <> struct CplxReal<double2> { using T = double; };

template <class V>
int acq_search(gnss_ctx* ctx, const int8_t* blk, const double2* xa, int64_t S, int dl, int nb, int np,
               const gnss_signal* sg, const gnss_acq* acq, const float* ca, typename CplxReal<V>::T* corr,
               Events& e_all, int* perm, DevBuf& fsync)
{
    const int dbl = sizeof(V) == sizeof(double2) ? 1 : 0;
    const size_t csz = sizeof(V);
    const int nsig = dl * nb;
    int st = GNSS_OK;
    if (acq_fft_supported(S) && !ctx->opt[GNSS_OPT_ACQ_ROCFFT]) {
        DevBuf d_twr, d_twc, B, X, A;
        const int P = (int)(S / 2000);
        *perm = P;
        const bool have_tw = ctx->acq_tw_S == S && ctx->acq_tw_dbl == dbl;
        HIP_TRY(d_twr.alloc(ctx, "acq.d_twr", 2000 * csz));
        HIP_TRY(d_twc.alloc(ctx, "acq.d_twc", (size_t)P * 2000 * csz));
        if (!have_tw) {
            std::vector<V> twr(2000), twc((size_t)P * 2000);
            for (int m = 0; m < 2000; m++) {
                const double a = -2.0 * M_PI * (double)m / 2000.0;
                twr[m].x = std::cos(a);
                twr[m].y = std::sin(a);
            }
            for (int m = 0; m < P; m++)
                for (int k = 0; k < 2000; k++) {
                    const double a = -2.0 * M_PI * (double)((int64_t)m * k % S) / (double)S;
                    twc[(size_t)m * 2000 + k].x = std::cos(a);
                    twc[(size_t)m * 2000 + k].y = std::sin(a);
                }
            HIP_TRY(hipMemcpyAsync(d_twr.p, twr.data(), twr.size() * csz, hipMemcpyHostToDevice, ctx->stream));
            HIP_TRY(hipMemcpyAsync(d_twc.p, twc.data(), twc.size() * csz, hipMemcpyHostToDevice, ctx->stream));
            HIP_TRY(hipStreamSynchronize(ctx->stream));
            ctx->acq_tw_S = S;
            ctx->acq_tw_dbl = dbl;
        }
        const size_t ntr = (size_t)nsig + np;
        HIP_TRY(B.alloc(ctx, "acq.B", csz * ntr * S));
        HIP_TRY(X.alloc(ctx, "acq.X", csz * ntr * S));
        const int npairs = nb * np;
        if (dbl && ctx->opt[GNSS_OPT_ACQ_FUSED]) {
            DevBuf ring;
            const int nslot = ctx->opt[GNSS_OPT_ACQ_RING] ? (int)ctx->opt[GNSS_OPT_ACQ_RING] : 3;
            HIP_TRY(ring.alloc(ctx, "acq.ring", acq_fused_ring_bytes(S)));
            HIP_TRY(fsync.alloc(ctx, "acq.fsync", acq_fused_sync_bytes()));
            HIP_TRY(hipStreamSynchronize(ctx->stream));
            HIP_TRY(hipEventRecord(e_all.a, ctx->stream));
            HIP_TRY(launch_acq_fft_forward<V>(blk, xa, S, dl, nb, sg->IF, acq->freqMin, acq->freqStep, sg->Fs, ca,
                                              np, sg->codeFreqBasis, d_twr.as<V>(), d_twc.as<V>(), B.as<V>(),
                                              X.as<V>(), ctx->stream));
            const V* C = X.as<V>() + (size_t)nsig * S;
            HIP_TRY(launch_acq_fft_correlate_fused(reinterpret_cast<const double2*>(C), X.as<double2>(), S, dl, nb,
                                                   np, nslot, d_twr.as<double2>(), d_twc.as<double2>(),
                                                   ring.as<double2>(), fsync.p, reinterpret_cast<double*>(corr),
                                                   ctx->stream));
            return GNSS_OK;
        }
        const int target = (int)std::max<int64_t>(1, ((int64_t)1 << 30) / ((int64_t)dl * S * (int64_t)csz));
        const int nbat = (npairs + target - 1) / target;
        int batch = (npairs + nbat - 1) / nbat;
        if (ctx->opt[GNSS_OPT_ACQ_BATCH] > 0)
            batch = (int)std::min<int64_t>(ctx->opt[GNSS_OPT_ACQ_BATCH], (int64_t)npairs);
        batch = std::max(1, std::min(batch, npairs));
        const int64_t pipe = ctx->opt[GNSS_OPT_ACQ_PIPE] ? ctx->opt[GNSS_OPT_ACQ_PIPE] : kAcqPipeDefault;
        const bool pair = dbl && pipe == 3 && npairs > batch;
        const bool two = (pipe == 2 || (pipe == 3 && !dbl)) && npairs > batch;
        hipStream_t s_cols = ctx->stream, s_rows = ctx->stream2;
        const size_t abuf = (size_t)batch * dl * S;
        HIP_TRY(A.alloc(ctx, "acq.A", csz * abuf * (two || pair ? 2 : 1)));
        HIP_TRY(hipStreamSynchronize(ctx->stream));
        HIP_TRY(hipEventRecord(e_all.a, ctx->stream));
        const bool fwd_split = kAcqFwdSplit && two;
        auto fwd = [&](int bin0, int nbc, bool codes) {
            return launch_acq_fft_forward<V>(blk, xa, S, dl, nb, sg->IF, acq->freqMin, acq->freqStep, sg->Fs, ca, np,
                                             sg->codeFreqBasis, d_twr.as<V>(), d_twc.as<V>(), B.as<V>(), X.as<V>(),
                                             ctx->stream, bin0, nbc, codes);
        };
        int fwd_bins = 0;
        if (fwd_split) {
            const int need = std::min(nb, (std::min(batch, npairs) - 1) / np + 1);
            HIP_TRY(fwd(0, need, true));
            fwd_bins = need;
        } else {
            HIP_TRY(fwd(0, -1, true));
            fwd_bins = nb;
        }
        const V* C = X.as<V>() + (size_t)nsig * S;
        if (pair) {
            const char* fe = probe_env("GNSS_PAIR_FRONT");
            const int front = fe ? atoi(fe) : kAcqPairFront;
            const int nbt = (npairs + batch - 1) / batch;
            double2* Ah[2] = {reinterpret_cast<double2*>(A.p), reinterpret_cast<double2*>(A.p) + abuf};
            for (int b = 0; b <= nbt; b++) {
                const int cq = b * batch, rq = (b - 1) * batch;
                const int nc = b < nbt ? std::min(batch, npairs - cq) : 0;
                const int nr = b > 0 ? std::min(batch, npairs - rq) : 0;
                HIP_TRY(launch_acq_fft_pair(reinterpret_cast<const double2*>(C), X.as<double2>(), S, dl, nb, np, cq,
                                            nc, Ah[b & 1], rq, nr, Ah[(b + 1) & 1], d_twr.as<double2>(),
                                            d_twc.as<double2>(), reinterpret_cast<double*>(corr), front,
                                            ctx->stream));
            }
            return GNSS_OK;
        }
        if (!two) {
            for (int q0 = 0; q0 < npairs; q0 += batch) {
                const int nq = std::min(batch, npairs - q0);
                HIP_TRY(launch_acq_fft_correlate(C, X.as<V>(), S, dl, nb, np, q0, nq, d_twr.as<V>(),
                                                 d_twc.as<V>(), A.as<V>(), corr, ctx->stream));
            }
            return GNSS_OK;
        }
        auto pipelined = [&]() -> int {
            int last = 0;
            for (int q0 = 0, b = 0; q0 < npairs; q0 += batch, b++) {
                const int nq = std::min(batch, npairs - q0);
                const int h = b & 1;
                V* Ah = A.as<V>() + (size_t)h * abuf;
                if (fwd_split) {
                    const int need = std::min(nb, (q0 + nq - 1) / np + 1);
                    if (need > fwd_bins) HIP_TRY(fwd(fwd_bins, need - fwd_bins, false));
                    fwd_bins = std::max(fwd_bins, need);
                }
                if (b >= 2) HIP_TRY(hipStreamWaitEvent(s_cols, ctx->ev_rows[h], 0));
                HIP_TRY(launch_acq_fft_correlate(C, X.as<V>(), S, dl, nb, np, q0, nq, d_twr.as<V>(), d_twc.as<V>(),
                                                 Ah, corr, s_cols, kAcqCols));
                HIP_TRY(hipEventRecord(ctx->ev_cols[h], s_cols));
                HIP_TRY(hipStreamWaitEvent(s_rows, ctx->ev_cols[h], 0));
                HIP_TRY(launch_acq_fft_correlate(C, X.as<V>(), S, dl, nb, np, q0, nq, d_twr.as<V>(), d_twc.as<V>(),
                                                 Ah, corr, s_rows, kAcqRows));
                HIP_TRY(hipEventRecord(ctx->ev_rows[h], s_rows));
                last = h;
            }
            HIP_TRY(hipStreamWaitEvent(ctx->stream, ctx->ev_rows[last], 0));
            return GNSS_OK;
        };
        const int pst = pipelined();
        if (pst != GNSS_OK) (void)hipStreamSynchronize(s_rows);
        return pst;
    }
    *perm = 0;
    DevBuf sig, code, y;
    HIP_TRY(sig.alloc(ctx, "acq.sig", csz * (size_t)nsig * S));
    HIP_TRY(code.alloc(ctx, "acq.code", csz * (size_t)np * S));
    const size_t per_prn = csz * (size_t)nsig * S;
    const int chunk = (int)std::max<size_t>(1, std::min<size_t>((size_t)np, ((size_t)4 << 30) / per_prn));
    HIP_TRY(y.alloc(ctx, "acq.y", per_prn * (size_t)chunk));
    rocfft_plan pl;
    if ((st = get_plan(ctx, S, nsig, dbl, 0, &pl))) return st;
    if ((st = get_plan(ctx, S, np, dbl, 0, &pl))) return st;
    for (int p0 = 0; p0 < np; p0 += chunk) {
        const int pc = std::min(chunk, np - p0);
        if ((st = get_plan(ctx, S, (size_t)pc * nsig, dbl, 1, &pl))) return st;
    }
    HIP_TRY(hipEventRecord(e_all.a, ctx->stream));
    HIP_TRY(launch_acq_wipe(blk, xa, S, dl, nb, sg->IF, acq->freqMin, acq->freqStep, sg->Fs, sig.as<V>(), ctx->stream));
    if ((st = run_fft(ctx, sig.p, S, nsig, dbl, 0))) return st;
    HIP_TRY(launch_acq_code(ca, nullptr, np, S, sg->codeFreqBasis, sg->Fs, code.as<V>(), ctx->stream));
    if ((st = run_fft(ctx, code.p, S, np, dbl, 0))) return st;
    for (int p0 = 0; p0 < np; p0 += chunk) {
        const int pc = std::min(chunk, np - p0);
        HIP_TRY(launch_acq_mul(code.as<V>() + (size_t)p0 * S, sig.as<V>(), pc, nsig, S, y.as<V>(), ctx->stream));
        if ((st = run_fft(ctx, y.p, S, (size_t)pc * nsig, dbl, 1))) return st;
        HIP_TRY(launch_acq_power(y.as<V>(), pc, nb, dl, S, 0, corr + (size_t)p0 * nb * S, ctx->stream));
    }
    return GNSS_OK;
}
}

static int group_acquisition(gnss_ctx* g, const gnss_file* file, const gnss_signal* sg, const gnss_acq* acq,
                             gnss_acquired* out, gnss_acq_diag* diag)
{
    if (!file || !sg || !acq || !out) return GNSS_EARG;
    memset(out, 0, sizeof(*out));
    if (diag) memset(diag, 0, sizeof(*diag));
    g->timing = gnss_timing{};
    std::vector<int32_t> prns;
    if (acq->n_prn > 0 && acq->prn_list) prns.assign(acq->prn_list, acq->prn_list + acq->n_prn);
    else for (int i = 1; i <= 32; i++) prns.push_back(i);
    if (prns.size() > GNSS_MAX_SV) return fail(g, GNSS_EARG, "too many PRNs");
    const int M = (int)g->members.size();
    const auto shards = group::deal((int)prns.size(), M);
    std::vector<std::vector<int32_t>> plist((size_t)M);
    for (int k = 0; k < M; k++)
        for (int i : shards[(size_t)k]) plist[(size_t)k].push_back(prns[(size_t)i]);
    std::vector<gnss_acquired> outs((size_t)M);
    std::vector<gnss_acq_diag> diags((size_t)M);
    std::vector<int> st((size_t)M, GNSS_ENODATA);
    std::vector<char> ran((size_t)M, 0);
    for_members(g, [&](int k) {
        memset(&outs[(size_t)k], 0, sizeof(gnss_acquired));
        memset(&diags[(size_t)k], 0, sizeof(gnss_acq_diag));
        if (plist[(size_t)k].empty()) return;
        gnss_acq a = *acq;
        a.n_prn = (int32_t)plist[(size_t)k].size();
        a.prn_list = plist[(size_t)k].data();
        st[(size_t)k] = gnss_acquisition(g->members[(size_t)k], file, sg, &a, &outs[(size_t)k],
                                         diag ? &diags[(size_t)k] : nullptr);
        ran[(size_t)k] = 1;
    });
    std::vector<gnss_timing> tm;
    for (int k = 0; k < M; k++)
        if (ran[(size_t)k]) tm.push_back(g->members[(size_t)k]->timing);
    g->timing = group::combine_timing(tm);
    for (int k = 0; k < M; k++)
        if (st[(size_t)k] != GNSS_OK && st[(size_t)k] != GNSS_ENODATA)
            return fail(g, st[(size_t)k], "member %d (device %d): %s", k, g->members[(size_t)k]->device,
                        g->members[(size_t)k]->err.c_str());
    if (!group::merge_acquired(prns, shards, outs, diag ? &diags : nullptr, out, diag))
        return fail(g, GNSS_EDEVICE, "multi-device acquisition: member results do not match their PRN shards");
    const int status = group::acquisition_status(st, out->n);
    if (status == GNSS_ENODATA) return fail(g, GNSS_ENODATA, "No satellites acquired");
    return status;
}

extern "C" {

int gnss_acquisition(gnss_ctx* ctx, const gnss_file* file, const gnss_signal* sg,
                     const gnss_acq* acq, gnss_acquired* out, gnss_acq_diag* diag)
{
    if (!ctx || !file || !sg || !acq || !out) return GNSS_EARG;
    if (!ctx->members.empty()) return group_acquisition(ctx, file, sg, acq, out, diag);
    memset(out, 0, sizeof(*out));
    if (diag) memset(diag, 0, sizeof(*diag));
    ctx->timing = gnss_timing{};
    HIP_TRY(hipSetDevice(ctx->device));
    const int prec = file->dataPrecision, dtyp = file->dataType;
    if ((prec != 1 && prec != 2) || (dtyp != 1 && dtyp != 2))
        return fail(ctx, GNSS_EARG, "dataPrecision must be 1 (int8) or 2 (int16), dataType 1 (I) or 2 (I/Q)");
    if (prec == 2 && dtyp == 1)
        return fail(ctx, GNSS_EINDEX, "int16 real record: rawsignal has Sample*datalen/2 samples (MATLAB index error)");
    const int64_t bps = (int64_t)prec * dtyp;
    const bool iq8 = prec == 1 && dtyp == 2;
    const int64_t S = sg->Sample;
    const int nb = acq->freqNum, dl = acq->datalen, L = acq->L;
    if (S <= 0 || nb <= 0 || dl <= 0 || L <= 0) return fail(ctx, GNSS_EARG, "bad acquisition sizes");

    std::vector<int32_t> prns;
    if (acq->n_prn > 0 && acq->prn_list) prns.assign(acq->prn_list, acq->prn_list + acq->n_prn);
    else for (int i = 1; i <= 32; i++) prns.push_back(i);
    if (prns.size() > GNSS_MAX_SV) return fail(ctx, GNSS_EARG, "too many PRNs");
    for (int p : prns) if (p < 1 || p > 51) return fail(ctx, GNSS_EARG, "PRN %d out of range", p);
    const int np = (int)prns.size();

    const int64_t off = file->skip * S * file->dataPrecision * file->dataType;
    const int64_t need = S * bps * std::max<int64_t>(dl, L + 1);
    const int64_t flen = file_length(file);
    if (flen < off + S * bps * dl) return fail(ctx, GNSS_EIO, "IF record too short for acquisition");
    IfWindow w;
    int st = stage_window(ctx, file, off, off + need, w);
    if (st) return st;
    const int8_t* blk = w.ptr + (off - w.base);
    DevBuf xs_acq, xs_fine, xs_sums;
    Events e_conv;
    if (!iq8) {
        const int64_t nfine = flen >= off + S * bps * (L + 1) ? S * (L + 1) : 0;
        HIP_TRY(xs_acq.alloc(ctx, "acq.xs", sizeof(double2) * (size_t)(S * dl)));
        if (nfine) HIP_TRY(xs_fine.alloc(ctx, "acq.xs_fine", sizeof(double2) * (size_t)nfine));
        HIP_TRY(xs_sums.alloc(ctx, "acq.xs_sums", 32));
        HIP_TRY(hipEventRecord(e_conv.a, ctx->stream));
        HIP_TRY(launch_stage_cpx(blk, prec, dtyp, S * dl, xs_acq.as<double2>(), xs_sums.as<unsigned long long>(),
                                 ctx->stream));
        if (nfine)
            HIP_TRY(launch_stage_cpx(blk, prec, dtyp, nfine, xs_fine.as<double2>(),
                                     xs_sums.as<unsigned long long>() + 2, ctx->stream));
        HIP_TRY(hipEventRecord(e_conv.b, ctx->stream));
    }
    const double2* xa = iq8 ? nullptr : xs_acq.as<double2>();
    const double2* xf = iq8 ? nullptr : xs_fine.as<double2>();

    std::vector<float> cah((size_t)np * 1023);
    for (int i = 0; i < np; i++) generate_ca(prns[i], &cah[(size_t)i * 1023]);
    DevBuf ca, corr, peaks, scratch;
    HIP_TRY(ca.alloc(ctx, "acq.ca", cah.size() * sizeof(float)));
    HIP_TRY(hipMemcpyAsync(ca.p, cah.data(), cah.size() * sizeof(float), hipMemcpyHostToDevice, ctx->stream));
    const int dbl = ctx->acq_fp64 ? 1 : 0;
    HIP_TRY(corr.alloc(ctx, "acq.corr", (dbl ? sizeof(double) : sizeof(float)) * (size_t)np * nb * S));
    HIP_TRY(peaks.alloc(ctx, "acq.peaks", sizeof(AcqPeak) * (size_t)np));
    HIP_TRY(scratch.alloc(ctx, "acq.scratch", acq_scratch_bytes(np, np)));
    Events e_all, e_corr;
    int perm = 0;
    DevBuf fsync;
    if (dbl)
        st = acq_search<double2>(ctx, blk, xa, S, dl, nb, np, sg, acq, ca.as<float>(), corr.as<double>(), e_all,
                                 &perm, fsync);
    else
        st = acq_search<float2>(ctx, blk, xa, S, dl, nb, np, sg, acq, ca.as<float>(), corr.as<float>(), e_all,
                                &perm, fsync);
    if (st) return st;
    const int cshift = (int)std::ceil(sg->Fs / sg->codeFreqBasis);
    if (dbl)
        HIP_TRY(launch_acq_peak(corr.as<double>(), np, nb, S, cshift, perm, peaks.as<AcqPeak>(), scratch.p,
                                ctx->stream));
    else
        HIP_TRY(launch_acq_peak(corr.as<float>(), np, nb, S, cshift, perm, peaks.as<AcqPeak>(), scratch.p,
                                ctx->stream));
    HIP_TRY(hipEventRecord(e_corr.b, ctx->stream));
    std::vector<AcqPeak> ph((size_t)np);
    HIP_TRY(hipMemcpyAsync(ph.data(), peaks.p, sizeof(AcqPeak) * (size_t)np, hipMemcpyDeviceToHost, ctx->stream));
    unsigned fused_err = 0;
    if (fsync.p)
        HIP_TRY(hipMemcpyAsync(&fused_err, static_cast<char*>(fsync.p) + acq_fused_err_offset(), sizeof(unsigned),
                               hipMemcpyDeviceToHost, ctx->stream));
    HIP_TRY(hipStreamSynchronize(ctx->stream));
    if (fused_err)
        return fail(ctx, GNSS_EDEVICE, "fused correlator: a pipeline wait timed out (grid not resident)");
    ctx->timing.acq_hypothesis_samples = (int64_t)np * nb * dl * S;

    std::vector<int> acq_idx;
    for (int i = 0; i < np; i++) {
        if (diag) {
            int k = diag->n++;
            diag->prn[k] = prns[i];
            diag->SNR[k] = ph[i].snr;
            diag->fbin[k] = ph[i].fbin + 1;
            diag->codePhase[k] = ph[i].cp + 1;
            diag->peak[k] = ph[i].peak;
            diag->peak2[k] = ph[i].peak2;
        }
        if (ph[i].snr >= 12) {
            int k = out->n++;
            out->sv[k] = prns[i];
            out->SNR[k] = ph[i].snr;
            out->Doppler[k] = acq->freqMin + acq->freqStep * (double)ph[i].fbin;
            out->codedelay[k] = ph[i].cp;
            acq_idx.push_back(i);
        }
    }
    if (out->n == 0) {
        HIP_TRY(hipEventRecord(e_all.b, ctx->stream));
        HIP_TRY(hipEventSynchronize(e_all.b));
        ctx->timing.acq_ms = e_all.ms();
        ctx->timing.acq_corr_ms = ctx->timing.acq_ms;
        return fail(ctx, GNSS_ENODATA, "No satellites acquired");
    }

    if (flen < off + S * bps * (L + 1)) return fail(ctx, GNSS_EIO, "IF record too short for fine search");
    const int fshift = dtyp == 2 ? 1 : 2;
    const int na = out->n;
    const int64_t N = (int64_t)L * S * dl;
    if (N % 2) return fail(ctx, GNSS_EINDEX, "odd fftlength: MATLAB indexes past the end (:116)");
    std::vector<float> caf((size_t)na * 1023);
    std::vector<int32_t> cdh((size_t)na);
    for (int k = 0; k < na; k++) {
        generate_ca(out->sv[k], &caf[(size_t)k * 1023]);
        cdh[k] = out->codedelay[k];
    }
    DevBuf fca, fcd, fx, kb;
    HIP_TRY(fca.alloc(ctx, "acq.fca", caf.size() * sizeof(float)));
    HIP_TRY(fcd.alloc(ctx, "acq.fcd", cdh.size() * sizeof(int32_t)));
    HIP_TRY(kb.alloc(ctx, "acq.kb", sizeof(int64_t) * (size_t)na));
    HIP_TRY(hipMemcpyAsync(fca.p, caf.data(), caf.size() * sizeof(float), hipMemcpyHostToDevice, ctx->stream));
    HIP_TRY(hipMemcpyAsync(fcd.p, cdh.data(), cdh.size() * sizeof(int32_t), hipMemcpyHostToDevice, ctx->stream));
    const bool own_fine = fine_fft_supported(S, L) && !ctx->opt[GNSS_OPT_FINE_ROCFFT];
    Events e_fine;
    if (own_fine) {
        const int fb = std::min(na, kFineBatch);
        HIP_TRY(fx.alloc(ctx, "acq.fx", fine_fft_scratch_bytes(S, L, dl, fb)));
        HIP_TRY(hipEventRecord(e_fine.a, ctx->stream));
        HIP_TRY(launch_fine_fft_tables(S, L, dl, fx.p, ctx->stream));
        for (int k0 = 0; k0 < na; k0 += fb) {
            const int nk = std::min(fb, na - k0);
            HIP_TRY(launch_fine_fft_argmax(blk, xf, S, L, dl, fcd.as<int32_t>() + k0, nk,
                                           fca.as<float>() + (size_t)k0 * 1023, sg->Fs, sg->codeFreqBasis,
                                           sg->codelength, fshift, fx.p, kb.as<int64_t>() + k0, ctx->stream));
        }
    } else {
        HIP_TRY(fx.alloc(ctx, "acq.fx", sizeof(double2) * (size_t)na * N));
        rocfft_plan pl;
        if ((st = get_plan(ctx, N, na, 1, 0, &pl))) return st;
        HIP_TRY(hipEventRecord(e_fine.a, ctx->stream));
        HIP_TRY(launch_fine_build(blk, xf, S, L, fcd.as<int32_t>(), fca.as<float>(), na, sg->Fs, sg->codeFreqBasis,
                                  sg->codelength, N, fx.as<double2>(), ctx->stream));
        if ((st = run_fft(ctx, fx.p, N, na, 1, 0))) return st;
        DevBuf fscr;
        HIP_TRY(fscr.alloc(ctx, "acq.fscr", acq_scratch_bytes(1, na)));
        HIP_TRY(launch_fine_argmax(fx.as<double2>(), na, N, fshift, fscr.p, kb.as<int64_t>(), ctx->stream));
    }
    HIP_TRY(hipEventRecord(e_fine.b, ctx->stream));
    HIP_TRY(hipEventRecord(e_all.b, ctx->stream));
    std::vector<int64_t> kh((size_t)na);
    HIP_TRY(hipMemcpyAsync(kh.data(), kb.p, sizeof(int64_t) * (size_t)na, hipMemcpyDeviceToHost, ctx->stream));
    HIP_TRY(hipStreamSynchronize(ctx->stream));
    for (int k = 0; k < na; k++) {
        const double K = (double)kh[k];
        out->fineFreq[k] = (file->dataType == 2) ? (-K * (sg->Fs / (double)N) + sg->Fs / 2) : (K * (sg->Fs / (double)N));
    }
    {
        float f = 0;
        (void)hipEventElapsedTime(&f, e_all.a, e_corr.b);
        ctx->timing.acq_corr_ms = f;
    }
    ctx->timing.acq_fine_ms = e_fine.ms();
    ctx->timing.acq_ms = e_all.ms() + (iq8 ? 0.0 : e_conv.ms());
    return GNSS_OK;
}

}
```

### assignment-for-aae6102_gnss-sdr_amd/csrc/gnss_internal.h

```cpp
#pragma once

#include <hip/hip_runtime.h>
#include <stdint.h>

#include "../../include/gnss_mi355x.h"

#define GNSS_HD __host__ __device__ __forceinline__

namespace gnss {

struct Colon {
    double a, d, c;
    int64_t n;
};

GNSS_HD Colon colon_make(double a, double d, double b)
{
    Colon r{a, d, b, -1};
    if (!(a - a == 0) || !(d - d == 0) || !(b - b == 0)) return r;
    if (d == 0 || (a < b && d < 0) || (b < a && d > 0)) return r;
    double tol = 2.0 * 2.220446049250313e-16 * fmax(fabs(a), fabs(b));
    double sig = d > 0 ? 1.0 : -1.0;
    double n;
    if (a == floor(a) && d == 1) {
        n = floor(b) - a;
    } else if (a == floor(a) && d == floor(d)) {
        double q = floor(a / d);
        double rr = a - q * d;
        n = floor((b - rr) / d) - q;
    } else {
        n = round((b - a) / d);
        if (sig * (a + n * d - b) > tol) n = n - 1;
    }
    double c = a + n * d;
    if (sig * (c - b) > -tol) c = b;
    r.c = c;
    r.n = (int64_t)n;
    return r;
}

GNSS_HD Colon colon_make_hint(double a, double d, double b, int64_t hint)
{
    const double X = b - a;
    const double r = fma(-(double)hint, d, X);
    if (!(d > 0) || !(fabs(r) < 0.4 * d) || a == floor(a)) return colon_make(a, d, b);
    Colon o{a, d, b, hint};
    const double tol = 2.0 * 2.220446049250313e-16 * fmax(fabs(a), fabs(b));
    double n = (double)hint;
    if (a + n * d - b > tol) n = n - 1;
    double c = a + n * d;
    if (c - b > -tol) c = b;
    o.c = c;
    o.n = (int64_t)n;
    return o;
}

GNSS_HD Colon colon_make_hint2(double a, double d, double b, int64_t hint, double hd)
{
    const double X = b - a;
    const double r = fma(-hd, d, X);
    if (!(d > 0) || !(fabs(r) < 0.4 * d) || a == floor(a)) return colon_make(a, d, b);
    const double tol = 2.0 * 2.220446049250313e-16 * fmax(fabs(a), fabs(b));
    const bool dec = a + hd * d - b > tol;
    const double nd = dec ? hd - 1 : hd;
    double c = a + nd * d;
    if (c - b > -tol) c = b;
    return Colon{a, d, c, dec ? hint - 1 : hint};
}

GNSS_HD double colon_elem(const Colon& r, int64_t k)
{
    if (2 * k == r.n) return (r.a + r.c) / 2;
    if (k <= r.n / 2) return r.a + (double)k * r.d;
    return r.c - (double)(r.n - k) * r.d;
}

GNSS_HD int ca_index(int64_t chip)
{
    int64_t r = (chip + 1022) % 1023;
    return (int)(r < 0 ? r + 1023 : r);
}

GNSS_HD unsigned ca_index32(int chip)
{
    return (unsigned)(chip + 1022) % 1023u;
}

GNSS_HD double fmod_pos(double x, double y)
{
    const double q = trunc(x / y);
    double r = __builtin_fma(-q, y, x);
    if (r < 0) r += y;
    return r;
}

constexpr double kTwoPi = 2.0 * 3.14159265358979323846;
constexpr double kTwoPiLo = 2.4492935982947064e-16;
constexpr double kInvTwoPi = 1.0 / kTwoPi;

GNSS_HD double div_round_fix(double x, double b, double q1)
{
    const double r1 = __builtin_fma(-q1, b, x);
    int64_t bits = __builtin_bit_cast(int64_t, q1);
    const int64_t mag = bits & 0x7fffffffffffffffLL;
    const bool away = (r1 > 0) == (q1 > 0);
    const double ulp = __builtin_bit_cast(double, (mag & 0x7ff0000000000000LL) - (52LL << 52));
    const double h = ((mag & 0x000fffffffffffffLL) != 0 || away) ? 0.5 * ulp : 0.25 * ulp;
    if (r1 != 0 && __builtin_fabs(r1) > h * b) bits += away ? 1 : -1;
    return __builtin_bit_cast(double, bits);
}

GNSS_HD double div_const(double x, double b, double rb)
{
    const double q = x * rb;
    const double r = __builtin_fma(-q, b, x);
    return div_round_fix(x, b, __builtin_fma(r, rb, q));
}

GNSS_HD double div_markstein(double x, double b, double rb)
{
    const double q = x * rb;
    const double r = __builtin_fma(-q, b, x);
    return __builtin_fma(r, rb, q);
}

__device__ __forceinline__ void sincos_small(double x, double* sn, double* cs)
{
    constexpr double kTwoOverPi = 6.36619772367581382433e-01;
    constexpr double kPio2Hi = 1.57079632673412561417e+00;
    constexpr double kPio2Lo = 6.07710050650619224932e-11;
    const double q = rint(x * kTwoOverPi);
    double y = __builtin_fma(-q, kPio2Hi, x);
    const double t = q * kPio2Lo;
    const double yh = y - t;
    const double yl = (y - yh) - t;
    y = yh;
    const double z = y * y;
    const double rs = __builtin_fma(z, __builtin_fma(z, __builtin_fma(z, __builtin_fma(z,
        1.58969099521155010221e-10, -2.50507602534068634195e-08), 2.75573137070700676789e-06),
        -1.98412698298579493134e-04), 8.33333333332248946124e-03);
    const double rc = z * __builtin_fma(z, __builtin_fma(z, __builtin_fma(z, __builtin_fma(z,
        __builtin_fma(z, -1.13596475577881948265e-11, 2.08757232129817482790e-09),
        -2.75573143513906633035e-07), 2.48015872894767294178e-05), -1.38888888888741095749e-03),
        4.16666666666666019037e-02);
    const double v = z * y;
    const double s = y - ((z * (0.5 * yl - v * rs) - yl) - v * -1.66666666666666324348e-01);
    const double hz = 0.5 * z;
    const double w = 1.0 - hz;
    const double c = w + (((1.0 - w) - hz) + (z * rc - y * yl));
    const int n = (int)q & 3;
    const double a = (n & 1) ? c : s, b = (n & 1) ? s : c;
    *sn = (n & 2) ? -a : a;
    *cs = ((n + 1) & 2) ? -b : b;
}


typedef unsigned u32x4 __attribute__((ext_vector_type(4)));
constexpr int kBufRsrcWord3 = 0x00020000;
constexpr int kPolSc1 = 16;

__device__ __forceinline__ void publish16(__amdgpu_buffer_rsrc_t r, int unit, double v, unsigned tag)
{
    const unsigned long long w = (unsigned long long)__double_as_longlong(v);
    const u32x4 g = {(unsigned)w, tag, (unsigned)(w >> 32), tag};
    __builtin_amdgcn_raw_buffer_store_b128(g, r, unit * 16, 0, kPolSc1);
}
__device__ __forceinline__ u32x4 load16(__amdgpu_buffer_rsrc_t r, int unit)
{
    return __builtin_amdgcn_raw_buffer_load_b128(r, unit * 16, 0, kPolSc1);
}
constexpr int kPolSys = 17;
__device__ __forceinline__ void publish16_sys(__amdgpu_buffer_rsrc_t r, int unit, double v, unsigned tag)
{
    const unsigned long long w = (unsigned long long)__double_as_longlong(v);
    const u32x4 g = {(unsigned)w, tag, (unsigned)(w >> 32), tag};
    __builtin_amdgcn_raw_buffer_store_b128(g, r, unit * 16, 0, kPolSys);
}
__device__ __forceinline__ u32x4 load16_sys(__amdgpu_buffer_rsrc_t r, int unit)
{
    return __builtin_amdgcn_raw_buffer_load_b128(r, unit * 16, 0, kPolSys);
}
__device__ __forceinline__ double value16(u32x4 g)
{
    return __longlong_as_double((long long)(((unsigned long long)g.z << 32) | g.x));
}

struct TrkChan {
    double remChip, remPhase, remSample;
    double carrier_outputLast, PLLdiscriLast, code_outputLast, DLLdiscriLast;
    double codeFreq, carrierFreqBasis, carrierFreq;
    double Zk[20];
    int64_t numSample;
    int64_t pos;
    int64_t Index;
    int64_t nstep;
    int64_t slot;
    int64_t n1_target;
    int64_t codedelay0;
    int32_t index_int, snrIndex;
    int32_t sv1;
    int32_t prn;
    int32_t status;
    int32_t countinx;
};

struct TrkParams {
    double Fs, codeFreqBasis, ms, codelength;
    double S;
    double tau1code, tau2code, tau1carr, tau2carr;
    double dataBytesPerSample;
    double inv_Fs;
    int32_t exact_div;
    int64_t buf_base;
    int64_t buf_len;
    int64_t file_len;
    int32_t ntaps, iE, iP, iL;
    int32_t nsv;
    int32_t nch;
    int32_t rec_cap;
    int32_t cn0_cap;
    int32_t probe;
    int32_t bps, fmt;
    const long long* pref_i;
    const long long* pref_q;
    const short* stage16;
    double taps[GNSS_MAX_TAPS];
    double qcap_dmax;
    double dll_r, dll_t1, dll_t10, pll_r, pll_t1, pll_t10;
    int32_t conv;
    int32_t chip_off;
    int32_t given;
    double tap_post[GNSS_MAX_TAPS];
    int32_t regcap;
};

constexpr int kLaneMax = 32;

struct StepDesc {
    int64_t n, delayValue, A, g_first, g_last, Index;
    double remSample, d, inv_d, f, phi0, dhi, dlo, remChip_next, remPhase_next;
    double mu_r, mu_i;
    double phi[kLaneMax];
    double2 rcs[kLaneMax];
    double tap_a[GNSS_MAX_TAPS], tap_c[GNSS_MAX_TAPS];
    double rc0;
    int32_t pdi, phaseC;
    int32_t bad;
    int32_t bad_tap;
};

struct TrkBuffers {
    const int8_t* iq;
    TrkChan* chan;
    TrkChan* snap;
    StepDesc* desc;
    const unsigned* ca_bits;
    double* partial;
    unsigned int* arrive;
    double* rec;
    double* taps_rec;
    double* cn0_1;
    double* cn0_10;
    int64_t* dvpre;
    double* p_i_1ms;
    double* dbg_sums;
    unsigned long long* stamps;
    unsigned long long* pgran;
    unsigned* run_err;
    int32_t n1;
};

struct TrkDev {
    const TrkParams* p;
    const TrkBuffers* b;
};

hipError_t launch_track_step(const TrkParams& p, const TrkBuffers& b, const TrkDev& d,
                             int blocks_per_chan, int sub, hipStream_t s);
hipError_t launch_track_run(const TrkParams& p, const TrkBuffers& b, const TrkDev& d,
                            int blocks_per_chan, int vblocks_per_block, int sub, int nsteps, unsigned tag0,
                            hipStream_t s);
int track_run_blocks_per_cu(const TrkParams& p, int sub, bool vblocks = false);
hipError_t launch_track_prepare(const TrkParams& p, const TrkBuffers& b, const TrkDev& d, int pdi,
                                int phaseC, hipStream_t s);
hipError_t launch_track_snapshot(const TrkParams& p, const TrkBuffers& b, const TrkDev& d, hipStream_t s);
hipError_t launch_track_bitedge(const TrkParams& p, const TrkBuffers& b, const TrkDev& d, hipStream_t s);
hipError_t launch_track_phase_c_init(const TrkParams& p, const TrkBuffers& b, const TrkDev& d,
                                     int64_t skip, hipStream_t s);
hipError_t launch_track_expand(const double* src, int64_t rec_cap, int stride, int nf, int nch,
                               const int64_t* job, double* dst, int64_t ML, int64_t n10, int ntaps,
                               hipStream_t s);

#ifndef GNSS_PROBE_BUILD
#define GNSS_PROBE_BUILD 0
#endif
constexpr bool kProbe = GNSS_PROBE_BUILD != 0;
#ifndef GNSS_XCHG_SLEEP
#define GNSS_XCHG_SLEEP 0
#endif
#ifndef GNSS_XCD_LOCAL
#define GNSS_XCD_LOCAL 0
#endif

constexpr int kTrkThreads = 256;
constexpr int kArriveStride = 64;
constexpr int kArrivePerChan = 9;
constexpr int kStampSlots = 2200;
constexpr int kMaxBpc = 1024;
constexpr int kMaxBpcRun = 256;
constexpr int run_bpc_cap(int ntaps) { return ntaps > 3 ? 192 : kMaxBpcRun; }
constexpr int kMaxVpb = 16;
#ifndef GNSS_QCAP
#define GNSS_QCAP 0
#endif
constexpr double kTapSpan = 30.0;
constexpr int kQcapMax = 8;

inline int max_taps_in_lane(const double* taps, const double* post, int n, int M, double dmax)
{
    const double w = (M - 1) * dmax + 1e-9;
    int best = 0;
    for (int a = 0; a < n; a++) {
        const double x = taps[a] + (post ? post[a] : 0.0);
        int c = 0;
        for (int b = 0; b < n; b++) {
            double f = (taps[b] + (post ? post[b] : 0.0)) - x;
            f -= floor(f);
            if (f < w || f > 1.0 - 1e-9) c++;
        }
        best = c > best ? c : best;
    }
    return best;
}
inline int lane_boundaries(const double* taps, const double* post, int n, int M, double dmax)
{
    const double w = (M - 1) * dmax + 1e-9;
    auto off = [&](int s) { return taps[s] + (post ? post[s] : 0.0); };
    auto same = [&](int a, int b) {
        const double f = off(a) - off(b), r = f - floor(f);
        return r < 1e-9 || r > 1.0 - 1e-9;
    };
    int best = 0;
    for (int a = 0; a < n; a++) {
        int c = 0, multi = 0;
        for (int b = 0; b < n; b++) {
            bool first = true;
            int size = 0;
            for (int e = 0; e < n; e++) {
                if (!same(b, e)) continue;
                if (e < b) first = false;
                size++;
            }
            if (!first) continue;
            double f = off(b) - off(a);
            f -= floor(f);
            if (f < w || f > 1.0 - 1e-9) {
                c++;
                multi += size > 1;
            }
        }
        c += multi > 1 ? multi : 1;
        best = c > best ? c : best;
    }
    return best;
}
constexpr int kRegCapMax = 2;
inline bool lane_regcap(const TrkParams& p, int sub) { return p.ntaps <= 3 && ((p.regcap >> sub) & 1) != 0; }
inline int regcap_mask(const TrkParams& p, double dmax, int64_t force)
{
    int m = 0;
    for (int sub = 1; sub <= 4 && force != 1 && p.ntaps <= 3; sub++)
        if (force == 2 || lane_boundaries(p.taps, p.tap_post, p.ntaps, 8 * sub, dmax) <= kRegCapMax) m |= 1 << sub;
    return m;
}
constexpr int kDeferSlots = 4;
constexpr int gran_region_b(int ntaps) { return ntaps > 3 ? 2 * kMaxBpcRun * 6 : 0; }
constexpr int gran_slot_b(int ntaps) { return 2 * ntaps * kMaxBpcRun; }
constexpr int gran_per_chan(int ntaps)
{
    return ntaps > 3 ? gran_region_b(ntaps) + kDeferSlots * gran_slot_b(ntaps) : 2 * kMaxBpcRun * 2 * ntaps;
}
constexpr int kDescWords = (int)(sizeof(StepDesc) / 4);

struct AcqPeak {
    double peak;
    int32_t fbin;
    int32_t cp;
    double snr;
    double peak2;
};

hipError_t launch_acq_wipe(const int8_t* iq, const double2* xs, int64_t S, int datalen, int nbins, double IF,
                           double freqMin, double freqStep, double Fs, float2* out, hipStream_t s);
hipError_t launch_acq_code(const float* ca, const int32_t* prn_slot, int nprn, int64_t S,
                           double codeFreqBasis, double Fs, float2* out, hipStream_t s);
hipError_t launch_acq_mul(const float2* code_spec, const float2* sig_spec, int nprn, int nsig,
                          int64_t S, float2* out, hipStream_t s);
hipError_t launch_acq_power(const float2* y, int nprn, int nbins, int datalen, int64_t S,
                            int first_ms, float* corr, hipStream_t s);
hipError_t launch_acq_wipe(const int8_t* iq, const double2* xs, int64_t S, int datalen, int nbins, double IF,
                           double freqMin, double freqStep, double Fs, double2* out, hipStream_t s);
hipError_t launch_acq_code(const float* ca, const int32_t* prn_slot, int nprn, int64_t S,
                           double codeFreqBasis, double Fs, double2* out, hipStream_t s);
hipError_t launch_acq_mul(const double2* code_spec, const double2* sig_spec, int nprn, int nsig,
                          int64_t S, double2* out, hipStream_t s);
hipError_t launch_acq_power(const double2* y, int nprn, int nbins, int datalen, int64_t S,
                            int first_ms, double* corr, hipStream_t s);
hipError_t launch_acq_peak(const float* corr, int nprn, int nbins, int64_t S, int cshift,
                           int perm, AcqPeak* out, void* scratch, hipStream_t s);
hipError_t launch_acq_peak(const double* corr, int nprn, int nbins, int64_t S, int cshift,
                           int perm, AcqPeak* out, void* scratch, hipStream_t s);

bool acq_fft_supported(int64_t S);
template <class V>
hipError_t launch_acq_fft_forward(const int8_t* iq, const double2* xs, int64_t S, int datalen, int nbins, double IF,
                                  double freqMin, double freqStep, double Fs, const float* ca,
                                  int nprn, double codeFreqBasis, const V* tw_row,
                                  const V* tw_col, V* B, V* X, hipStream_t s, int bin0 = 0, int nbc = -1,
                                  bool codes = true);
constexpr int kAcqCols = 1, kAcqRows = 2;
hipError_t launch_acq_fft_correlate(const float2* C, const float2* X, int64_t S, int datalen,
                                    int nbins, int nprn, int first_pair, int npair,
                                    const float2* tw_row, const float2* tw_col, float2* A,
                                    float* corr, hipStream_t s, int parts = kAcqCols | kAcqRows);
hipError_t launch_acq_fft_correlate(const double2* C, const double2* X, int64_t S, int datalen,
                                    int nbins, int nprn, int first_pair, int npair,
                                    const double2* tw_row, const double2* tw_col, double2* A,
                                    double* corr, hipStream_t s, int parts = kAcqCols | kAcqRows);
hipError_t launch_acq_fft_pair(const double2* C, const double2* X, int64_t S, int datalen, int nbins, int nprn,
                               int cols_first, int cols_n, double2* Acols, int rows_first, int rows_n,
                               const double2* Arows, const double2* tw_row, const double2* tw_col, double* corr,
                               int front, hipStream_t s);
size_t acq_fused_sync_bytes();
size_t acq_fused_err_offset();
size_t acq_fused_ring_bytes(int64_t S);
hipError_t launch_acq_fft_correlate_fused(const double2* C, const double2* X, int64_t S, int datalen, int nbins,
                                          int nprn, int nslot, const double2* tw_row, const double2* tw_col,
                                          double2* ring, void* sync, double* corr, hipStream_t s);
bool fine_fft_supported(int64_t S, int L);
size_t fine_fft_scratch_bytes(int64_t S, int L, int datalen, int nsv);
hipError_t launch_fine_fft_tables(int64_t S, int L, int datalen, void* scratch, hipStream_t s);
hipError_t launch_fine_fft_argmax(const int8_t* iq, const double2* xs, int64_t S, int L, int datalen,
                                  const int32_t* cd, int nsv, const float* ca, double Fs, double codeFreqBasis,
                                  double codelength, int shifted, void* scratch, int64_t* kbest, hipStream_t s);
hipError_t launch_fine_build(const int8_t* iq, const double2* xs, int64_t S, int L, const int32_t* codedelay,
                             const float* ca, int nsv, double Fs, double codeFreqBasis,
                             double codelength, int64_t N, double2* out, hipStream_t s);
hipError_t launch_fine_argmax(const double2* F, int nsv, int64_t N, int shifted, void* scratch,
                              int64_t* kbest, hipStream_t s);

size_t acq_scratch_bytes(int nprn, int nsv);

hipError_t launch_stage_cpx(const int8_t* src, int prec, int type, int64_t nsamp, double2* out,
                            unsigned long long* sums, hipStream_t s);
hipError_t launch_real8_to_iq8(const int8_t* src, int64_t n, int8_t* dst, hipStream_t s);
size_t prefix16_scratch_bytes(int64_t ngroups);
hipError_t launch_prefix16(const short* src, int64_t ngroups, long long* pref_i, long long* pref_q,
                           void* scratch, size_t scratch_bytes, hipStream_t s);

struct SrcIQ8 {
    const int8_t* p;
    __device__ __forceinline__ double2 at(int64_t n) const
    {
        const char2 r = *reinterpret_cast<const char2*>(p + 2 * n);
        return make_double2((double)r.x, (double)r.y);
    }
};
struct SrcC64 {
    const double2* p;
    __device__ __forceinline__ double2 at(int64_t n) const { return p[n]; }
};


GNSS_HD double cn0_moment(const double* Z, double T)
{
    double mean = 0;
    for (int k = 0; k < 20; k++) mean += Z[k];
    mean = mean / 20;
    double var = 0;
    for (int k = 0; k < 20; k++) var += (Z[k] - mean) * (Z[k] - mean);
    var = var / 19;
    const double m2v = mean * mean - var;
    const double scale = 1 / T;
    if (m2v >= 0) {
        const double NA2 = sqrt(m2v);
        const double varIQ = 0.5 * (mean - NA2);
        return fabs(10 * log10(scale * NA2 / (2 * varIQ)));
    }
    const double y = sqrt(-m2v);
    const double nr = 0, ni = scale * y;
    const double dr = 2 * (0.5 * mean), di = 2 * (0.5 * -y);
    const double den = dr * dr + di * di;
    const double zr = (nr * dr + ni * di) / den, zi = (ni * dr - nr * di) / den;
    const double lr = 10 * (log(hypot(zr, zi)) / log(10.0));
    const double li = 10 * (atan2(zi, zr) / log(10.0));
    return hypot(lr, li);
}

GNSS_HD double vt_spacing(int i1)
{
    return colon_elem(colon_make(0.7, -0.05, -0.7), i1 - 1);
}

struct VtPrep {
    int64_t n;
    int64_t j[3];
    int bad;
};
GNSS_HD VtPrep vt_prepare(double Fs, double codelength, int pdi, double remChip, double codeFreq_old,
                          double codeFreq_new)
{
    VtPrep p{0, {1, 1, 1}, GNSS_OK};
    const double ns = ceil((codelength * pdi - remChip) / (codeFreq_old / Fs));
    if (!(ns >= 1) || ns > 1e9) {
        p.bad = GNSS_EINDEX;
        return p;
    }
    p.n = (int64_t)ns;
    const double cps = codeFreq_new / Fs;
    const int sp[3] = {5, 15, 25};
    const int64_t len = 1023 * (int64_t)pdi + 2;
    for (int s = 0; s < 3; s++) {
        const double spc = vt_spacing(sp[s]);
        const double a = (0 + spc) + remChip;
        const Colon c = colon_make(a, cps, ((double)(p.n - 1) * cps + spc) + remChip);
        if (c.n != p.n - 1) p.bad = GNSS_EINDEX;
        double j = ceil(a) + 1;
        if (j > 1025) j = 1025;
        if (!(j >= 1) || j > (double)len) p.bad = GNSS_EINDEX;
        p.j[s] = p.bad ? 1 : (int64_t)j;
    }
    return p;
}

template <class CaAt>
GNSS_HD int vt_code_at(int64_t j, int pdi, CaAt ca)
{
    const int64_t len = 1023 * (int64_t)pdi + 2;
    return j == 1 ? ca(1022) : j == len ? ca(0) : ca((int)((j - 2) % 1023));
}

GNSS_HD double vt_rem_carr_phase(double carrFreq, int64_t n, double Fs, double remCarrPhase)
{
    const double W = kTwoPi * (carrFreq * ((double)n / Fs)) + remCarrPhase;
    return fmod(W, kTwoPi);
}

struct VtPll {
    double carrError, carrNco, carrFreq;
};
GNSS_HD VtPll vt_pll(const gnss_vt_chan& c, int pdi, double tau1carr, double tau2carr, double P_i, double P_q)
{
    VtPll r;
    r.carrError = atan(P_q / P_i) / (2.0 * 3.14159265358979323846);
    r.carrNco = c.oldCarrNco + (tau2carr / tau1carr) * (r.carrError - c.oldCarrError) +
                r.carrError * (pdi * 1e-3 / tau1carr);
    r.carrFreq = c.carrFreqBasis + r.carrNco;
    return r;
}

GNSS_HD int vt_finish(double Fs, double ms, int pdi, int bps, double tau1carr, double tau2carr,
                      gnss_vt_chan* c, const VtPrep& p, const int* code, double codeFreq_new, double sI,
                      double sQ, gnss_vt_out* o)
{
    const int64_t n = p.n;
    const double cps = codeFreq_new / Fs;
    const double sp = vt_spacing(15);
    const Colon col = colon_make((0 + sp) + c->remChip, cps, ((double)(n - 1) * cps + sp) + c->remChip);
    if (col.n != n - 1) return GNSS_EINDEX;
    const double remChip = (colon_elem(col, n - 1) + cps) - 1023 * pdi;
    const double remCarrPhase = vt_rem_carr_phase(c->carrFreq, n, Fs, c->remCarrPhase);
    o->E_i = code[0] * sI;
    o->E_q = code[0] * sQ;
    o->P_i = code[1] * sI;
    o->P_q = code[1] * sQ;
    o->L_i = code[2] * sI;
    o->L_q = code[2] * sQ;
    o->CN0 = 0;
    o->cn0_row = 0;
    c->index_int += 1;
    c->Zk[c->index_int - 1] = o->P_i * o->P_i + o->P_q * o->P_q;
    if (c->index_int % 20 == 0) {
        o->CN0 = cn0_moment(c->Zk, 1 * ms * pdi);
        o->cn0_row = c->snrIndex;
        c->index_int = 0;
        c->snrIndex += 1;
    }
    const VtPll pll = vt_pll(*c, pdi, tau1carr, tau2carr, o->P_i, o->P_q);
    const double carrError = pll.carrError, carrNco = pll.carrNco, carrFreq = pll.carrFreq;
    const double E = sqrt(o->E_i * o->E_i + o->E_q * o->E_q);
    const double L = sqrt(o->L_i * o->L_i + o->L_q * o->L_q);
    o->codeError = -0.5 * (E - L) / (E + L);
    o->carrError = carrError;
    o->carrNco = carrNco;
    o->remChip = remChip;
    o->remCarrPhase = remCarrPhase;
    o->codeFreq = codeFreq_new;
    o->carrFreq = carrFreq;
    o->numSample = n;
    const int64_t absS = c->file_ptr + n * bps;
    o->absoluteSample = absS;
    o->codedelay = fmod_pos((double)absS / bps, Fs * ms);
    o->status = GNSS_OK;
    c->file_ptr = absS;
    c->remChip = remChip;
    c->remCarrPhase = remCarrPhase;
    c->codeFreq = codeFreq_new;
    c->carrFreq = carrFreq;
    c->oldCarrNco = carrNco;
    c->oldCarrError = carrError;
    return GNSS_OK;
}

struct VtOrbit {
    double t;
    double sv[3], vel[3], clkm, clkv, grp;
    int st;
};
double vt_transmit_next(const gnss_vt_nav& v, int i, int64_t numSample);
void vt_orbit(const gnss_vt_nav& v, int i, double t, VtOrbit* o);
int vt_nav_predict_at(gnss_vt_nav* v, int i, int64_t numSample, const VtOrbit* ahead, double* codeFreq,
                      double* deltaPr, double sv_vel[3]);
struct VtGain {
    int st;
    double H[2 * GNSS_VT_MAX_CH * 8], K[8 * 2 * GNSS_VT_MAX_CH], cov[64], T[64];
    double prr_pred[GNSS_VT_MAX_CH], clkv[GNSS_VT_MAX_CH], sv_unrot[GNSS_VT_MAX_CH][3];
    double svr_last[3], vel_last[3], localTime;
};
void vt_nav_gain(const gnss_vt_nav& v, VtGain* g);
int vt_nav_correct(gnss_vt_nav* v, const VtGain& g, const double* codeError, const double* codeFreq,
                   const double* carrFreq, gnss_vt_navsol* sol, bool minus_if = false);
inline double vt_remchip_next(double Fs, int pdi, double remChip, double codeFreq_new, int64_t n)
{
    const double cps = codeFreq_new / Fs;
    const double sp = vt_spacing(15);
    const Colon col = colon_make((0 + sp) + remChip, cps, ((double)(n - 1) * cps + sp) + remChip);
    return (colon_elem(col, n - 1) + cps) - 1023 * pdi;
}

GNSS_HD void calc_loop_coef(double LBW, double zeta, double k, double& t1, double& t2)
{
    const double Wn = LBW * 8 * zeta / (4 * (zeta * zeta) + 1);
    t1 = k / (Wn * Wn);
    t2 = 2.0 * zeta / Wn;
}

struct VtRunArgs {
    const uint8_t* rec;
    int64_t base, len;
    int64_t file_len;
    gnss_vt_chan* chans;
    const double* codeFreq;
    gnss_vt_out* out;
    const unsigned* ca_bits;
    double Fs, ms, codelength, tau1carr, tau2carr;
    int n, nsteps, pdi, prec, dtype;
};
hipError_t launch_vt_run(const VtRunArgs& a, hipStream_t s);
struct VtStepArgs {
    const uint8_t* rec;
    double Fs;
    int real8;
    unsigned seq;
    double* part;
    double* sums;
    unsigned* done;
    unsigned* ticket;
    int64_t off[GNSS_VT_MAX_CH];
    int64_t ns[GNSS_VT_MAX_CH];
    double f[GNSS_VT_MAX_CH];
    double phi0[GNSS_VT_MAX_CH];
    double rfs[GNSS_VT_MAX_CH];
};
hipError_t launch_vt_step(const VtStepArgs& a, int n, int nb, hipStream_t s);
struct alignas(16) VtGran {
    uint64_t lo, hi;
};
inline void vt_gran_put(VtGran* g, uint64_t bits, unsigned tag)
{
    __atomic_store_n(&g->lo, (bits & 0xffffffffull) | ((uint64_t)tag << 32), __ATOMIC_RELAXED);
    __atomic_store_n(&g->hi, (bits >> 32) | ((uint64_t)tag << 32), __ATOMIC_RELAXED);
}
inline bool vt_gran_get(const VtGran* g, unsigned tag, uint64_t* bits)
{
    const uint64_t lo = __atomic_load_n(&g->lo, __ATOMIC_ACQUIRE), hi = __atomic_load_n(&g->hi, __ATOMIC_ACQUIRE);
    if ((unsigned)(lo >> 32) != tag || (unsigned)(hi >> 32) != tag) return false;
    *bits = (lo & 0xffffffffull) | (hi << 32);
    return true;
}
struct VtBlockStep {
    int64_t off, ns;
    double f, phi0;
    double rfs;
};
constexpr unsigned kVtLoopStop = 0xffffffffu;
constexpr int kVtStepWords = 5;
struct VtLoopArgs {
    const uint8_t* rec;
    int64_t rec_len;
    double Fs;
    int real8;
    unsigned seq0;
    const VtGran* mail;
    VtGran* sums;
    uint64_t timeout;
    void* gstep;
    void* gpart;
    unsigned long long* stamps;
};
constexpr int kVtStampSteps = 2000;
constexpr int kVtLoopMaxBlocks = 1024;
constexpr double kVtLoopTimeoutS = 10;
hipError_t launch_vt_loop(const VtLoopArgs& a, int n, int nb, hipStream_t s);
int vt_loop_resident_blocks(int device);
constexpr int kVtStepThreads = 256;
constexpr int kVtStepSamples = 8 * kVtStepThreads;
constexpr int kVtLoopSamples = 3 * kVtStepThreads;
void ca_chips(int prn, float* out);

hipError_t launch_synth_if(const gnss_synth& cfg, const float* ca, uint64_t sample0,
                           uint64_t nsamples, int8_t* dst, hipStream_t s);

}
```

### assignment-for-aae6102_gnss-sdr_amd/csrc/host.h

```cpp
#pragma once

#include <hip/hip_runtime.h>
#include <rocfft/rocfft.h>

#include <algorithm>
#include <cstdint>
#include <cstdlib>
#include <map>
#include <string>
#include <thread>
#include <tuple>
#include <utility>
#include <vector>

#include "gnss_internal.h"
#include "group.h"

struct gnss_ctx {
    int device = 0;
    hipStream_t stream = nullptr;
    hipStream_t stream2 = nullptr;
    hipEvent_t ev_cols[2] = {}, ev_rows[2] = {};
    std::string err;
    gnss_timing timing{};
    int profiling = 0;
    std::map<std::tuple<size_t, size_t, int, int>, rocfft_plan> plans;
    void* fft_work = nullptr;
    size_t fft_work_size = 0;
    std::map<std::string, std::pair<void*, size_t>> pool;
    std::map<std::string, std::pair<void*, size_t>> pinned;
    int64_t acq_tw_S = 0;
    int acq_tw_dbl = -1;
    int acq_fp64 = 1;
    uint64_t window = 0;
    int64_t opt[GNSS_OPT_COUNT] = {};
    int lane_path = 0;
    std::vector<gnss_ctx*> members;
    bool member = false;
    int fail_chan = -1;
    gnss::group::ResidentCache<void*> resident;
};

namespace gnss {
namespace host {

inline const char* probe_env(const char* name)
{
    return GNSS_PROBE_BUILD ? getenv(name) : nullptr;
}

constexpr int kVtSpan = 2000;

int fail(gnss_ctx* ctx, int code, const char* fmt, ...) __attribute__((format(printf, 3, 4)));

#define HIP_TRY(expr)                                                                         \
    do {                                                                                       \
        hipError_t e_ = (expr);                                                                \
        if (e_ != hipSuccess)                                                                  \
            return ::gnss::host::fail(ctx, GNSS_EDEVICE, "%s:%d %s: %s", __FILE__, __LINE__,   \
                                      #expr, hipGetErrorString(e_));                           \
    } while (0)

template <class T>
T* pinned_buffer(gnss_ctx* ctx, const char* key, size_t count, unsigned flags = hipHostMallocDefault)
{
    auto& e = ctx->pinned[key];
    const size_t want = std::max<size_t>(count * sizeof(T), 16);
    if (e.second < want) {
        if (e.first) (void)hipHostFree(e.first);
        e = {nullptr, 0};
        if (hipHostMalloc(&e.first, want, flags) != hipSuccess) return nullptr;
        e.second = want;
    }
    return static_cast<T*>(e.first);
}

struct DevBuf {
    void* p = nullptr;
    size_t n = 0;
    bool pooled = false;
    DevBuf() = default;
    DevBuf(const DevBuf&) = delete;
    DevBuf& operator=(const DevBuf&) = delete;
    ~DevBuf() { release(); }
    void release()
    {
        if (p && !pooled) (void)hipFree(p);
        p = nullptr;
        pooled = false;
    }
    hipError_t alloc(size_t bytes)
    {
        release();
        n = bytes;
        return hipMalloc(&p, bytes ? bytes : 16);
    }
    hipError_t alloc(gnss_ctx* ctx, const char* key, size_t bytes)
    {
        release();
        auto& e = ctx->pool[key];
        const size_t want = bytes ? bytes : 16;
        if (e.second < want) {
            if (e.first) (void)hipFree(e.first);
            e = {nullptr, 0};
            const hipError_t r = hipMalloc(&e.first, want);
            if (r != hipSuccess) {
                e.first = nullptr;
                return r;
            }
            e.second = want;
        }
        p = e.first;
        n = bytes;
        pooled = true;
        return hipSuccess;
    }
    template <class T> T* as() const { return reinterpret_cast<T*>(p); }
};

template <class F>
void parallel_for(int n, F f)
{
    const int nt = std::max(1, std::min({n, 16, (int)std::thread::hardware_concurrency()}));
    if (nt <= 1) {
        for (int i = 0; i < n; i++) f(i);
        return;
    }
    std::vector<std::thread> th;
    th.reserve((size_t)nt);
    for (int t = 0; t < nt; t++)
        th.emplace_back([&, t]() {
            for (int i = t; i < n; i += nt) f(i);
        });
    for (auto& x : th) x.join();
}

struct Events {
    hipEvent_t a = nullptr, b = nullptr;
    Events() { (void)hipEventCreate(&a); (void)hipEventCreate(&b); }
    ~Events() { (void)hipEventDestroy(a); (void)hipEventDestroy(b); }
    double ms() const { float f = 0; (void)hipEventElapsedTime(&f, a, b); return f; }
};

int64_t file_length(const gnss_file* f);

struct IfWindow {
    DevBuf own;
    const int8_t* ptr = nullptr;
    int64_t base = 0, len = 0;
};

int stage_into(gnss_ctx* ctx, const gnss_file* f, int64_t lo, int64_t hi, int8_t* dst);
int stage_window(gnss_ctx* ctx, const gnss_file* f, int64_t lo, int64_t hi, IfWindow& w);
int pointer_device(const void* p);
int drop_resident(gnss_ctx* ctx, const void* p, uint64_t n);

int get_plan(gnss_ctx* ctx, size_t len, size_t batch, int dbl, int inverse, rocfft_plan* out);
int run_fft(gnss_ctx* ctx, void* data, size_t len, size_t batch, int dbl, int inverse);

inline int fast_div_exact(double Fs, int64_t kmax) { return group::reciprocal_exact_cached(Fs, kmax); }

void generate_ca(int prn, float* out);
void ca_bits(int prn, unsigned* out32);

bool lane_rate_admitted(const gnss_signal* sg, double codeFreq_max);
int refuse_lane_rate(gnss_ctx* ctx, const gnss_signal* sg, double codeFreq_max);

template <class F>
void for_members(gnss_ctx* g, F fn)
{
    std::vector<int> devs;
    for (gnss_ctx* m : g->members) devs.push_back(m->device);
    std::vector<std::thread> th;
    for (const std::vector<int>& ks : group::by_device(devs))
        th.emplace_back([&fn, ks]() {
            for (int k : ks) fn(k);
        });
    for (auto& t : th) t.join();
}

}
}
```

### include/gnss_mi355x.h

```cpp
#ifndef GNSS_MI355X_H
#define GNSS_MI355X_H

#include <stdint.h>
#include <stddef.h>

#ifdef __cplusplus
extern "C" {
#endif

#define GNSS_ABI_VERSION 13

#define GNSS_OK         0
#define GNSS_ENODATA    1
#define GNSS_EIO        2
#define GNSS_EARG       3
#define GNSS_EDEVICE    4
#define GNSS_EINDEX     5

#define GNSS_MAX_SV     64
#define GNSS_MAX_TAPS   32


typedef struct gnss_file {
    const char   *path;
    const int8_t *data;
    const void   *dev_data;
    uint64_t      nbytes;
    int64_t       skip;
    int32_t       dataType;
    int32_t       dataPrecision;
} gnss_file;

typedef struct gnss_signal {
    double  IF;
    double  Fs;
    double  codeFreqBasis;
    double  ms;
    int64_t Sample;
    double  codelength;
} gnss_signal;

typedef struct gnss_acq {
    int32_t        freqNum;
    double         freqMin;
    double         freqStep;
    int32_t        datalen;
    int32_t        L;
    int32_t        n_prn;
    const int32_t *prn_list;
} gnss_acq;

typedef struct gnss_acquired {
    int32_t n;
    int32_t sv[GNSS_MAX_SV];
    double  SNR[GNSS_MAX_SV];
    double  Doppler[GNSS_MAX_SV];
    int32_t codedelay[GNSS_MAX_SV];
    double  fineFreq[GNSS_MAX_SV];
} gnss_acquired;

typedef struct gnss_acq_diag {
    int32_t n;
    int32_t prn[GNSS_MAX_SV];
    double  SNR[GNSS_MAX_SV];
    int32_t fbin[GNSS_MAX_SV];
    int32_t codePhase[GNSS_MAX_SV];
    double  peak[GNSS_MAX_SV];
    double  peak2[GNSS_MAX_SV];
} gnss_acq_diag;

typedef struct gnss_track {
    double  CorrelatorSpacing;
    double  DLLBW, DLLDamp, DLLGain;
    double  PLLBW, PLLDamp, PLLGain;
    int32_t msToProcessCT_1ms;
    int32_t msToProcessCT_10ms;
    int32_t        n_taps;
    const double  *tap_offsets;
    int32_t        n_chan;
    const int32_t *chan;
} gnss_track;

enum gnss_track_field {
    GNSS_F_P_i = 0, GNSS_F_P_q, GNSS_F_E_i, GNSS_F_E_q, GNSS_F_L_i, GNSS_F_L_q,
    GNSS_F_PLLdiscri, GNSS_F_DLLdiscri, GNSS_F_codedelay, GNSS_F_remChip,
    GNSS_F_codeFreq, GNSS_F_carrierFreq, GNSS_F_remPhase, GNSS_F_remSample,
    GNSS_F_numSample, GNSS_F_delayValue, GNSS_F_absoluteSample, GNSS_F_codedelay2,
    GNSS_NFIELDS
};

#define GNSS_F_carrError               GNSS_F_PLLdiscri
#define GNSS_F_codeError               GNSS_F_DLLdiscri
#define GNSS_F_carrFreq                GNSS_F_carrierFreq
#define GNSS_F_remCarrPhase            GNSS_F_remPhase
#define GNSS_F_absoluteSampleCodedelay GNSS_F_remSample

#define GNSS_OUT_DEVICE 1
typedef struct gnss_track_out {
    int64_t  max_len;
    double  *rec;
    double  *taps;
    int64_t *len;
    int32_t *countinx;
    double  *CN0_Eph;
    int32_t  cn0_cap;
    int32_t  cn0_rows;
    int32_t  flags;
    int32_t  reserved;
} gnss_track_out;

typedef struct gnss_timing {
    double acq_ms;
    double acq_corr_ms;
    double acq_fine_ms;
    double track_ms;
    double track_kernel_ms;
    int64_t track_launches;
    int64_t track_channel_samples;
    int64_t acq_hypothesis_samples;
    double h2d_ms;
    double  track10_kernel_ms;
    int64_t track10_launches;
    int64_t track10_channel_samples;
    int64_t h2d_bytes;
    int64_t track_segments;
} gnss_timing;

typedef struct gnss_ctx gnss_ctx;

int         gnss_abi_version(void);
const char *gnss_strerror(int status);

int  gnss_ctx_create(int device, gnss_ctx **out);
#define GNSS_MAX_DEVICES 16
int  gnss_ctx_create_multi(const int *devices, int n, gnss_ctx **out);
int  gnss_ctx_drop_record(gnss_ctx *ctx, const void *dev_ptr);
int  gnss_ctx_resident_records(const gnss_ctx *ctx);
int  gnss_device_count(void);
int  gnss_ctx_members(const gnss_ctx *ctx);
void gnss_ctx_destroy(gnss_ctx *ctx);
const char *gnss_last_error(const gnss_ctx *ctx);
int  gnss_last_timing(const gnss_ctx *ctx, gnss_timing *out);
int  gnss_ctx_set_profiling(gnss_ctx *ctx, int enable);
int  gnss_ctx_set_acq_precision(gnss_ctx *ctx, int fp64);
int  gnss_ctx_set_window(gnss_ctx *ctx, uint64_t bytes);
#define GNSS_OPT_FORCE_SUB    0
#define GNSS_OPT_NO_PERSIST   1
#define GNSS_OPT_FORCE_VPB    2
#define GNSS_OPT_ACQ_ROCFFT   3
#define GNSS_OPT_FINE_ROCFFT  4
#define GNSS_OPT_ACQ_BATCH    5
#define GNSS_OPT_ACQ_FUSED    6
#define GNSS_OPT_ACQ_RING     7
#define GNSS_OPT_ACQ_PIPE     8
#define GNSS_OPT_VT_BLOCKS    9
#define GNSS_OPT_FORCE_PEER   10
#define GNSS_OPT_VT_SPAN      11
#define GNSS_OPT_SLOT_PATH    12
#define GNSS_OPT_COUNT        13
int  gnss_ctx_set_option(gnss_ctx *ctx, int key, int64_t value);
int  gnss_lane_boundaries(const double *taps, const double *post, int n_taps, int lane_samples,
                          double cps_max);
int  gnss_ctx_lane_path(const gnss_ctx *ctx);

int  gnss_dev_alloc(gnss_ctx *ctx, uint64_t nbytes, void **dev_ptr);
int  gnss_dev_free(gnss_ctx *ctx, void *dev_ptr);
int  gnss_dev_upload(gnss_ctx *ctx, void *dev_dst, const void *host_src, uint64_t nbytes);
int  gnss_dev_download(gnss_ctx *ctx, void *host_dst, const void *dev_src, uint64_t nbytes);

int gnss_acquisition(gnss_ctx *ctx, const gnss_file *file, const gnss_signal *signal,
                     const gnss_acq *acq, gnss_acquired *out, gnss_acq_diag *diag);

int gnss_tracking_ct(gnss_ctx *ctx, const gnss_file *file, const gnss_signal *signal,
                     const gnss_track *track, const gnss_acquired *acquired,
                     gnss_track_out *out);

int gnss_tracking_ct_pos(gnss_ctx *ctx, const gnss_file *file, const gnss_signal *signal,
                         const gnss_track *track, const gnss_acquired *acquired, int32_t ctPOS,
                         const int32_t *countinx, gnss_track_out *out);

#define GNSS_MC_TAPS 25

int gnss_tracking_ct_multicorr(gnss_ctx *ctx, const gnss_file *file, const gnss_signal *signal,
                               const gnss_track *track, const gnss_acquired *acquired,
                               int32_t datalength, gnss_track_out *out);
int gnss_tracking_ct_mc(gnss_ctx *ctx, const gnss_file *file, const gnss_signal *signal,
                        const gnss_track *track, const gnss_acquired *acquired, int32_t msPosCT,
                        int32_t pdi, gnss_track_out *out);

enum gnss_eph_field {
    GNSS_E_TOW = 0, GNSS_E_TOW1, GNSS_E_sfb, GNSS_E_sfb1, GNSS_E_weeknum, GNSS_E_N, GNSS_E_health,
    GNSS_E_IODC, GNSS_E_TGD, GNSS_E_toc, GNSS_E_af2, GNSS_E_af1, GNSS_E_af0, GNSS_E_IODE2, GNSS_E_Crs,
    GNSS_E_deltan, GNSS_E_M0, GNSS_E_Cuc, GNSS_E_ecc, GNSS_E_Cus, GNSS_E_sqrta, GNSS_E_toe, GNSS_E_Cic,
    GNSS_E_omegae, GNSS_E_Cis, GNSS_E_i0, GNSS_E_Crc, GNSS_E_w, GNSS_E_omegadot, GNSS_E_IODE3,
    GNSS_E_idot, GNSS_E_updatetime, GNSS_E_updatetime_tow,
    GNSS_EPH_NFIELDS
};

typedef struct gnss_nav_out {
    int32_t  eph_cap;
    double  *eph;
    int32_t *eph_len;
    int32_t *updateflag;
    int64_t *nav1;
    int64_t *sfb1;
} gnss_nav_out;

int gnss_navi_decode(const gnss_acquired *acquired, const double *P_i, const int64_t *len,
                     int64_t stride, gnss_nav_out *out);

int gnss_correlate_step(gnss_ctx *ctx, const gnss_file *file, const gnss_signal *signal,
                        int prn, int pdi, double remChip, double codeFreq, double carrierFreq,
                        double remPhase, int64_t pos_bytes, int n_taps, const double *taps,
                        double *sums_out, int64_t *numSample_out);

typedef struct gnss_vt_chan {
    int32_t prn;
    int32_t pad;
    int64_t file_ptr;
    double  remChip;
    double  remCarrPhase;
    double  codeFreq;
    double  carrFreq;
    double  carrFreqBasis;
    double  oldCarrNco, oldCarrError;
    int32_t index_int;
    int32_t snrIndex;
    double  Zk[20];
} gnss_vt_chan;

typedef struct gnss_vt_out {
    double  E_i, E_q, P_i, P_q, L_i, L_q;
    double  carrError, codeError, carrNco;
    double  remChip, remCarrPhase, codeFreq, carrFreq;
    int64_t numSample, absoluteSample;
    double  codedelay;
    double  CN0;
    int32_t cn0_row;
    int32_t status;
    double  deltaPr;
    double  prRate;
    double  sv_vel[3];
} gnss_vt_out;

int gnss_tracking_vt_run(gnss_ctx *ctx, const gnss_file *file, const gnss_signal *signal,
                         const gnss_track *track, int32_t pdi, int32_t n, int32_t nsteps,
                         gnss_vt_chan *chans, const double *codeFreq_new, gnss_vt_out *out);

int gnss_tracking_vt_step(gnss_ctx *ctx, const gnss_file *file, const gnss_signal *signal,
                          const gnss_track *track, int32_t pdi, int32_t n, gnss_vt_chan *chans,
                          const double *codeFreq_new, gnss_vt_out *out);

int gnss_vt_nco_step(const gnss_signal *signal, const gnss_track *track, int32_t pdi,
                     gnss_vt_chan *chan, double codeFreq_new, double sumI, double sumQ,
                     gnss_vt_out *out);

int gnss_vt_prepare(const gnss_signal *signal, int32_t pdi, const gnss_vt_chan *chan,
                    double codeFreq_new, int32_t code_out[3], int64_t *numSample);

#define GNSS_VT_MAX_CH 32
#define GNSS_VT_MAX_BLOCKS 1024

typedef struct gnss_eph_sv {
    double sqrta, deltan, toe, M0, ecc, w, Cus, Cuc, Crs, Crc, Cis, Cic, i0, idot, omegae, omegadot;
    double toc, af0, af1, af2, TGD;
} gnss_eph_sv;

typedef struct gnss_vt_nav_cfg {
    double cnslxyz[3];
    double ALPHA[4];
    double BETA[4];
    double doy;
    double cSpeed;
    double Fc;
} gnss_vt_nav_cfg;

typedef struct gnss_vt_nav {
    int32_t n, pdi;
    int32_t msIndex;
    int32_t counterUptR, counter_r;
    int32_t prn[GNSS_VT_MAX_CH];
    gnss_vt_nav_cfg cfg;
    double  Fs, IF, codeFreqBasis, ms;
    double  cnslxyz[3];
    double  total_state[8];
    double  state_cov[64];
    double  R[2 * GNSS_VT_MAX_CH];
    double  recordR2[2 * GNSS_VT_MAX_CH];
    double  transmitTime[GNSS_VT_MAX_CH];
    double  tot_est_tck[GNSS_VT_MAX_CH];
    double  predictedPr_last[GNSS_VT_MAX_CH];
    double  counter_corr[GNSS_VT_MAX_CH];
    double  ionodel[GNSS_VT_MAX_CH], tropodel[GNSS_VT_MAX_CH];
    double  el[GNSS_VT_MAX_CH], az[GNSS_VT_MAX_CH];
    int64_t numSample[GNSS_VT_MAX_CH];
    gnss_eph_sv eph[GNSS_VT_MAX_CH];
} gnss_vt_nav;

typedef struct gnss_vt_navsol {
    double localTime;
    double usrPos[3], usrVel[3];
    double usrPosENU[3], usrVelENU[3], usrPosLLH[3];
    double clkBias, clkDrift;
    double state[8];
    double state_cov[8];
    double newZ[2 * GNSS_VT_MAX_CH];
    double meas_inno[2 * GNSS_VT_MAX_CH];
    double satEA[GNSS_VT_MAX_CH], satAZ[GNSS_VT_MAX_CH];
    double predicted_z[2 * GNSS_VT_MAX_CH];
    double satePos[3], sateVel[3];
    double svxyz_pos[GNSS_VT_MAX_CH][3];
    double kalman_gain[8][2 * GNSS_VT_MAX_CH];
    double R[2 * GNSS_VT_MAX_CH];
    int32_t r_row;
    int32_t reserved;
} gnss_vt_navsol;

int gnss_sv_pos_vel(const gnss_eph_sv *eph, double t, double pos[3], double vel[3],
                    double *clkcorr_m, double *clkcorr_m_vel, double *grpdel);
#define GNSS_GEO_XYZ2LLH  0
#define GNSS_GEO_LLH2XYZ  1
#define GNSS_GEO_XYZ2ENU  2
#define GNSS_GEO_EROTCORR 3
#define GNSS_GEO_IONO     4
#define GNSS_GEO_TROP     5
int gnss_geo(int fn, const double *in, double *out);

int gnss_vt_nav_init(const gnss_vt_nav_cfg *cfg, const gnss_signal *signal, int32_t pdi, int32_t n,
                     const int32_t *prn, const gnss_eph_sv *eph, const double usrPos[3],
                     const double usrVel[3], double clkBias, double clkDrift,
                     const double *timeTransmit, gnss_vt_nav *nav);

int gnss_vt_nav_predict(gnss_vt_nav *nav, int32_t i, int64_t numSample, double *codeFreq,
                        double *deltaPr, double sv_vel[3]);

int gnss_vt_nav_update(gnss_vt_nav *nav, const double *codeError, const double *codeFreq,
                       const double *carrFreq, gnss_vt_navsol *sol);

int gnss_tracking_vt(gnss_ctx *ctx, const gnss_file *file, const gnss_signal *signal,
                     const gnss_track *track, int32_t n, int32_t nsteps, gnss_vt_chan *chans,
                     gnss_vt_nav *nav, gnss_vt_out *out, gnss_vt_navsol *sol);

#define GNSS_VT_MC_TAPS 25

typedef struct gnss_vt_mc_out {
    double  E_i, E_q, P_i, P_q, L_i, L_q;
    double  carrError, codeError, carrNco;
    double  remChip, remCarrPhase, codeFreq, carrFreq;
    int64_t numSample, absoluteSample;
    double  codedelay;
    double  CN0;
    int32_t cn0_row;
    int32_t status;
    double  deltaPr;
    double  prRate;
    double  sv_vel[3];
    double  tap_i[GNSS_VT_MC_TAPS];
    double  tap_q[GNSS_VT_MC_TAPS];
} gnss_vt_mc_out;

int gnss_tracking_vt_mc_run(gnss_ctx *ctx, const gnss_file *file, const gnss_signal *signal,
                            const gnss_track *track, int32_t pdi, int32_t n, int32_t nsteps,
                            gnss_vt_chan *chans, const double *codeFreq_new, gnss_vt_mc_out *out);

int gnss_tracking_vt_mc(gnss_ctx *ctx, const gnss_file *file, const gnss_signal *signal,
                        const gnss_track *track, int32_t n, int32_t nsteps, gnss_vt_chan *chans,
                        gnss_vt_nav *nav, gnss_vt_mc_out *out, gnss_vt_navsol *sol);

int gnss_vt_mc_prepare(const gnss_signal *signal, int32_t pdi, const gnss_vt_chan *chan,
                       double codeFreq_new, double tap_a[GNSS_VT_MC_TAPS],
                       double tap_c[GNSS_VT_MC_TAPS], int64_t *numSample);

int gnss_vt_mc_nco_step(const gnss_signal *signal, const gnss_track *track, int32_t pdi,
                        gnss_vt_chan *chan, double codeFreq_new,
                        const double tap_i[GNSS_VT_MC_TAPS], const double tap_q[GNSS_VT_MC_TAPS],
                        gnss_vt_mc_out *out);

int gnss_vt_mc_nav_update(gnss_vt_nav *nav, const double *codeError, const double *codeFreq,
                          const double *carrFreq, gnss_vt_navsol *sol);

#define GNSS_ENOCONV    6
#define GNSS_CT_POS_UPDATED    0
#define GNSS_CT_POS_MULTICORR  1

typedef struct gnss_ct_pos_cfg {
    int32_t n;
    int32_t mode;
    int32_t dataType;
    int32_t msToProcessCT_1ms;
    int32_t pdi;
    int32_t reserved;
    double  navSolPeriod;
    double  Fs, IF, codelength, ms;
    double  cSpeed, doy;
    double  cnslxyz[3];
    double  ALPHA[4], BETA[4];
    int32_t countinx[GNSS_VT_MAX_CH];
    int64_t nav1[GNSS_VT_MAX_CH];
    int64_t sfb1[GNSS_VT_MAX_CH];
    int64_t sampleStart[GNSS_VT_MAX_CH];
    double  TOW1[GNSS_VT_MAX_CH];
    gnss_eph_sv eph[GNSS_VT_MAX_CH];
} gnss_ct_pos_cfg;

typedef struct gnss_nav_sol_ct {
    int64_t cap;
    int64_t rows;
    double *rawPseudorange;
    double *usrPos;
    double *usrVel;
    double *usrPosENU;
    double *usrPosLLH;
    double *clkBias;
    double *usrVelENU;
    double *clkDrift;
    double *DOP;
    double *satEA;
    double *satAZ;
    double *timeTransmit;
    double *codePhaseMeas;
    double *localTime;
    int64_t *Index;
    int64_t *index;
    double  *carrFreqMeas;
    int32_t *iters;
} gnss_nav_sol_ct;

int gnss_ct_pos_solve(gnss_ctx *ctx, const gnss_ct_pos_cfg *cfg, const gnss_track_out *records,
                      gnss_nav_sol_ct *out);

typedef struct gnss_acf_cfg {
    int32_t n;
    int32_t ind_start;
    int32_t numOverLap;
    int32_t reserved;
    double  corrSpacing;
    double  maxDelay;
    double  a[4];
    int32_t prn[GNSS_VT_MAX_CH];
    double  ele[GNSS_VT_MAX_CH];
} gnss_acf_cfg;

typedef struct gnss_acf_out {
    int64_t  cap;
    int64_t *windows;
    double  *meanMax;
    double  *F1;
    double  *F2;
    double  *varDelay;
    double  *meanCodeDisc;
    double  *varCodeDisc;
    uint8_t *maxCorrInd;
    double  *corr;
} gnss_acf_out;

int gnss_acf_features(gnss_ctx *ctx, const gnss_acf_cfg *cfg, const gnss_track_out *records,
                      int32_t n_taps, gnss_acf_out *out);

int gnss_ca_code(int prn, int8_t *out1023);

typedef struct gnss_synth_sv {
    int32_t prn;
    double  doppler_hz;
    double  code_phase0;
    double  carr_phase0;
    double  cn0_dbhz;
    uint64_t bit_seed;
    double  bit_phase_chips;
    int32_t lnav;
    int32_t reserved;
} gnss_synth_sv;

typedef struct gnss_synth {
    double   Fs, IF;
    double   noise_sigma;
    uint64_t seed;
    int32_t  n_sv;
    gnss_synth_sv sv[GNSS_MAX_SV];
} gnss_synth;

int gnss_lnav_bits(int32_t prn, int32_t nbits, int8_t *bits_out);

int gnss_synth_if_device(gnss_ctx *ctx, const gnss_synth *cfg, uint64_t sample0,
                         uint64_t nsamples, void *dev_dst);

#define GNSS_MAX_RAYS 128
typedef struct gnss_synth_ray {
    int32_t  sv;
    int32_t  reserved;
    double   delay_chips;
    double   gain;
    double   phase0_cycles;
    double   fade_hz;
    uint64_t t_on, t_off;
} gnss_synth_ray;

typedef struct gnss_synth_scene {
    double   Fs, IF;
    double   noise_sigma;
    uint64_t seed;
    int32_t  n_sv;
    gnss_synth_sv sv[GNSS_MAX_SV];
    double   los_gain[GNSS_MAX_SV];
    int32_t  n_ray;
    gnss_synth_ray ray[GNSS_MAX_RAYS];
} gnss_synth_scene;

int gnss_synth_scene_device(gnss_ctx *ctx, const gnss_synth_scene *scene, uint64_t sample0,
                            uint64_t nsamples, void *dev_dst);

int gnss_synth_scene_host(const gnss_synth_scene *scene, uint64_t sample0, uint64_t nsamples,
                          void *dst, int nthreads);

#ifdef __cplusplus
}
#endif
#endif
```

Before: 400,000.

## Reuse forward FFTs across Doppler bins related by an integer circular shift

Doppler bins are grouped into classes. Two bins share a class when their frequency difference times S/Fs is an exact integer, which happens only when all parameters are whole numbers. Only one representative bin per class gets a forward FFT, and the column-inverse kernels read that spectrum at a circularly shifted index. This cuts forward-FFT work and the memory for the X buffer, at the cost of wrapped addressing and a bin-map lookup in the correlate kernels. The fine-search FFT tables also move to a dedicated buffer and are rebuilt only when S, L or datalen change.

Result: no change. 403,200, median of 6 (+0.8%).

```diff
diff --git a/assignment-for-aae6102_gnss-sdr_amd/abi.py b/assignment-for-aae6102_gnss-sdr_amd/abi.py
--- a/assignment-for-aae6102_gnss-sdr_amd/abi.py
+++ b/assignment-for-aae6102_gnss-sdr_amd/abi.py
@@ -330,7 +330,8 @@
 LOADED_PATH = None
 
 (OPT_FORCE_SUB, OPT_NO_PERSIST, OPT_FORCE_VPB, OPT_ACQ_ROCFFT, OPT_FINE_ROCFFT, OPT_ACQ_BATCH, OPT_ACQ_FUSED,
- OPT_ACQ_RING, OPT_ACQ_PIPE, OPT_VT_BLOCKS, OPT_FORCE_PEER, OPT_VT_SPAN, OPT_SLOT_PATH) = range(13)
+ OPT_ACQ_RING, OPT_ACQ_PIPE, OPT_VT_BLOCKS, OPT_FORCE_PEER, OPT_VT_SPAN, OPT_SLOT_PATH,
+ OPT_ACQ_OWN_CLASS) = range(14)
 MAX_DEVICES = 16
 
 
diff --git a/assignment-for-aae6102_gnss-sdr_amd/csrc/acq_classes.h b/assignment-for-aae6102_gnss-sdr_amd/csrc/acq_classes.h
--- /dev/null
+++ b/assignment-for-aae6102_gnss-sdr_amd/csrc/acq_classes.h
@@ -0,0 +1,42 @@
+#pragma once
+
+#include <cmath>
+#include <cstdint>
+#include <vector>
+
+namespace gnss {
+
+struct AcqClasses {
+    std::vector<int32_t> cls;
+    std::vector<int32_t> shift;
+    std::vector<int32_t> rep;
+};
+
+inline AcqClasses acq_bin_classes(double freqMin, double freqStep, int nbins, double Fs, int64_t S, bool own)
+{
+    AcqClasses c;
+    auto whole = [](double x) { return std::isfinite(x) && std::trunc(x) == x; };
+    const bool exact = !own && whole(freqMin) && whole(freqStep) && whole(Fs) && Fs > 0 && S > 0;
+    for (int b = 0; b < nbins; b++) {
+        int found = -1;
+        int32_t s = 0;
+        for (size_t k = 0; exact && k < c.rep.size(); k++) {
+            const double num = freqStep * (double)(b - c.rep[k]) * (double)S;
+            if (!(std::fabs(num) < 9007199254740992.0) || std::fmod(num, Fs) != 0.0) continue;
+            const double q = num / Fs;
+            if (std::fabs(q) >= (double)S) continue;
+            found = (int)k;
+            s = (int32_t)q;
+            break;
+        }
+        if (found < 0) {
+            found = (int)c.rep.size();
+            c.rep.push_back(b);
+        }
+        c.cls.push_back(found);
+        c.shift.push_back(s);
+    }
+    return c;
+}
+
+}
diff --git a/assignment-for-aae6102_gnss-sdr_amd/csrc/acq_fft.hip b/assignment-for-aae6102_gnss-sdr_amd/csrc/acq_fft.hip
--- a/assignment-for-aae6102_gnss-sdr_amd/csrc/acq_fft.hip
+++ b/assignment-for-aae6102_gnss-sdr_amd/csrc/acq_fft.hip
@@ -400,13 +400,9 @@
 
 
 struct FwdSet {
-    int nbins, nsig, nprn, bin0, nbc, codes;
-    __device__ __forceinline__ int transform(int y) const
-    {
-        if (codes && y < nprn) return nsig + y;
-        const int u = y - (codes ? nprn : 0), idx = u / nbc;
-        return idx * nbins + bin0 + (u - idx * nbc);
-    }
+    int nclass, nsig, nprn;
+    const int* rep;
+    __device__ __forceinline__ int transform(int y) const { return y < nprn ? nsig + y : y - nprn; }
 };
 
 template <int P, class Src, class V>
@@ -418,12 +414,12 @@
     using R = Re<V>;
     constexpr int64_t S = (int64_t)P * kRow;
     __shared__ V s_a[kRowPad], s_tw[kTwIK];
-    const int nbins = fs.nbins, nsig = fs.nsig;
+    const int nclass = fs.nclass, nsig = fs.nsig;
     const int n2 = blockIdx.x, s = fs.transform(blockIdx.y), tid = threadIdx.x;
     const TwIK<V> twk = load_row_tw_ik(s_tw, tw_row, tid);
     constexpr int NIT = (kRow + kRowThreads - 1) / kRowThreads;
     if (s < nsig) {
-        const int idx = s / nbins, bin = s - idx * nbins;
+        const int idx = s / nclass, bin = fs.rep[s - idx * nclass];
         const double f = (IF + (freqMin + freqStep * (double)bin)) / Fs;
         auto put = [&](int n1, double2 r) {
             const int64_t n = (int64_t)P * n1 + n2;
@@ -518,29 +514,40 @@
 #ifndef GNSS_INVCOLS_WPE
 #define GNSS_INVCOLS_WPE 0
 #endif
+template <int P> __device__ __forceinline__ int shifted_elem0(int k1, int d)
+{
+    const int u = k1 + d;
+    return u >= P * kRow ? u - P * kRow : u;
+}
 template <int P, class V>
 __device__ __forceinline__ void inv_cols_body(
-    int bx, int t, const V* __restrict__ C, const V* __restrict__ X, int nbins, int nprn, int datalen,
-    int first_pair, const V* __restrict__ tw_col, V* __restrict__ A)
+    int bx, int t, const V* __restrict__ C, const V* __restrict__ X, const int2* __restrict__ binmap, int nclass,
+    int nprn, int datalen, int first_pair, const V* __restrict__ tw_col, V* __restrict__ A)
 {
     const int k1 = bx * kColThreads + threadIdx.x;
     if (k1 >= kRow) return;
     const int q = first_pair + t / datalen, idx = t % datalen;
     const int bin = q / nprn, p = q - bin * nprn;
+    const int2 bm = binmap[bin];
+    const V* xrep = X + ((int64_t)idx * nclass + bm.x) * P * kRow;
+    const int u = shifted_elem0<P>(k1, bm.y);
+    constexpr int kB = P * kRow * (int)sizeof(V);
+    const int vo_hi = u * (int)sizeof(V) + kB, vo_lo = u * (int)sizeof(V);
+    auto xvo = [&](int i) { return u >= (P - i) * kRow ? vo_lo : vo_hi; };
     V v[P];
     if (GNSS_COLS_BUF == 2) {
-        constexpr int kB = P * kRow * (int)sizeof(V), G = GNSS_COLS_GROUP;
+        constexpr int G = GNSS_COLS_GROUP;
         const __amdgpu_buffer_rsrc_t rc = __builtin_amdgcn_make_buffer_rsrc(
             (void*)(C + (int64_t)p * P * kRow), (short)0, kB, 0x00020000);
         const __amdgpu_buffer_rsrc_t rx = __builtin_amdgcn_make_buffer_rsrc(
-            (void*)(X + ((int64_t)idx * nbins + bin) * P * kRow), (short)0, kB, 0x00020000);
+            (void*)(xrep - P * kRow), (short)0, 2 * kB, 0x00020000);
         const int vo = k1 * (int)sizeof(V);
         V ca[G], xa[G];
 #pragma unroll
         for (int i = 0; i < G; i++) {
-            const int r = (i < P ? i : P - 1) * kRow * (int)sizeof(V);
-            ca[i] = buf_ld<V>(rc, vo, r);
-            xa[i] = buf_ld<V>(rx, vo, r);
+            const int r = i < P ? i : P - 1;
+            ca[i] = buf_ld<V>(rc, vo, r * kRow * (int)sizeof(V));
+            xa[i] = buf_ld<V>(rx, xvo(r), r * kRow * (int)sizeof(V));
         }
 #pragma unroll
         for (int g = 0; g < P; g += G) {
@@ -549,7 +556,7 @@
             for (int i = 0; i < G; i++)
                 if (g + G + i < P) {
                     cb[i] = buf_ld<V>(rc, vo, (g + G + i) * kRow * (int)sizeof(V));
-                    xb[i] = buf_ld<V>(rx, vo, (g + G + i) * kRow * (int)sizeof(V));
+                    xb[i] = buf_ld<V>(rx, xvo(g + G + i), (g + G + i) * kRow * (int)sizeof(V));
                 }
             __builtin_amdgcn_sched_barrier(0);
 #pragma unroll
@@ -559,23 +566,26 @@
             for (int i = 0; i < G; i++) { ca[i] = cb[i]; xa[i] = xb[i]; }
         }
     } else if (GNSS_COLS_BUF) {
-        constexpr int kB = P * kRow * (int)sizeof(V), G = GNSS_COLS_GROUP;
+        constexpr int G = GNSS_COLS_GROUP;
         const __amdgpu_buffer_rsrc_t rc = __builtin_amdgcn_make_buffer_rsrc(
             (void*)(C + (int64_t)p * P * kRow), (short)0, kB, 0x00020000);
         const __amdgpu_buffer_rsrc_t rx = __builtin_amdgcn_make_buffer_rsrc(
-            (void*)(X + ((int64_t)idx * nbins + bin) * P * kRow), (short)0, kB, 0x00020000);
+            (void*)(xrep - P * kRow), (short)0, 2 * kB, 0x00020000);
         const int vo = k1 * (int)sizeof(V);
 #pragma unroll
         for (int i = 0; i < P; i++) v[i] = buf_ld<V>(rc, vo, i * kRow * (int)sizeof(V));
         V xa[G];
 #pragma unroll
-        for (int i = 0; i < G; i++) xa[i] = buf_ld<V>(rx, vo, (i < P ? i : P - 1) * kRow * (int)sizeof(V));
+        for (int i = 0; i < G; i++) {
+            const int r = i < P ? i : P - 1;
+            xa[i] = buf_ld<V>(rx, xvo(r), r * kRow * (int)sizeof(V));
+        }
 #pragma unroll
         for (int g = 0; g < P; g += G) {
             V xb[G];
 #pragma unroll
             for (int i = 0; i < G; i++)
-                if (g + G + i < P) xb[i] = buf_ld<V>(rx, vo, (g + G + i) * kRow * (int)sizeof(V));
+                if (g + G + i < P) xb[i] = buf_ld<V>(rx, xvo(g + G + i), (g + G + i) * kRow * (int)sizeof(V));
             __builtin_amdgcn_sched_barrier(0);
 #pragma unroll
             for (int i = 0; i < G; i++)
@@ -585,9 +595,11 @@
         }
     } else {
         const V* c = C + (int64_t)p * P * kRow + k1;
-        const V* x = X + ((int64_t)idx * nbins + bin) * P * kRow + k1;
-#pragma unroll
-        for (int i = 0; i < P; i++) v[i] = cmulc(c[(int64_t)i * kRow], x[(int64_t)i * kRow]);
+#pragma unroll
+        for (int i = 0; i < P; i++) {
+            const int e = u + i * kRow;
+            v[i] = cmulc(c[(int64_t)i * kRow], xrep[e >= P * kRow ? e - P * kRow : e]);
+        }
     }
     V* a = A + (int64_t)t * P * kRow + k1;
     const V* tw = tw_col + k1;
@@ -604,10 +616,10 @@
 __attribute__((amdgpu_waves_per_eu(GNSS_INVCOLS_WPE, GNSS_INVCOLS_WPE)))
 #endif
 void inv_cols_kernel(
-    const V* __restrict__ C, const V* __restrict__ X, int nbins, int nprn, int datalen,
-    int first_pair, const V* __restrict__ tw_col, V* __restrict__ A)
-{
-    inv_cols_body<P, V>(blockIdx.x, blockIdx.y, C, X, nbins, nprn, datalen, first_pair, tw_col, A);
+    const V* __restrict__ C, const V* __restrict__ X, const int2* __restrict__ binmap, int nclass, int nprn,
+    int datalen, int first_pair, const V* __restrict__ tw_col, V* __restrict__ A)
+{
+    inv_cols_body<P, V>(blockIdx.x, blockIdx.y, C, X, binmap, nclass, nprn, datalen, first_pair, tw_col, A);
 }
 
 template <int P>
@@ -748,8 +760,8 @@
 
 template <int P>
 __global__ __launch_bounds__(kRowThreads) void inv_pair_kernel_f64(
-    const double2* __restrict__ C, const double2* __restrict__ X, int nbins, int nprn, int datalen,
-    int cols_first, int cols_n, double2* __restrict__ Acols, int rows_first, int rows_n,
+    const double2* __restrict__ C, const double2* __restrict__ X, const int2* __restrict__ binmap, int nclass,
+    int nbins, int nprn, int datalen, int cols_first, int cols_n, double2* __restrict__ Acols, int rows_first, int rows_n,
     const double2* __restrict__ Arows, double scale, const double2* __restrict__ tw_row,
     const double2* __restrict__ tw_col, double* __restrict__ corr, int front)
 {
@@ -763,7 +775,7 @@
         inv_rows_f64_body<P>(tau2, g, Arows, nprn, datalen, rows_first, scale, tw_row, tw_col, corr, nbins);
     } else {
         const int c = (int)(i - r0), t = c / kCx;
-        inv_cols_body<P, double2>(c - t * kCx, t, C, X, nbins, nprn, datalen, cols_first, tw_col, Acols);
+        inv_cols_body<P, double2>(c - t * kCx, t, C, X, binmap, nclass, nprn, datalen, cols_first, tw_col, Acols);
     }
 }
 
@@ -801,8 +813,8 @@
 
 template <int P>
 __global__ __launch_bounds__(kRowThreads, 2) void inv_fused_kernel_f64(
-    const double2* __restrict__ C, const double2* __restrict__ X, int nbins, int nprn, int datalen,
-    int npairs, int nslot, double scale, const double2* __restrict__ tw_row, const double2* __restrict__ tw_col,
+    const double2* __restrict__ C, const double2* __restrict__ X, const int2* __restrict__ binmap, int nclass,
+    int nbins, int nprn, int datalen, int npairs, int nslot, double scale, const double2* __restrict__ tw_row, const double2* __restrict__ tw_col,
     double2* __restrict__ ring, FuseSync* __restrict__ sy, double* __restrict__ corr)
 {
     constexpr int Q = (kRow + kRowThreads - 1) / kRowThreads;
@@ -852,10 +864,15 @@
             const int k1 = ch * kColThreads + tid;
             if (k1 < kRow) {
                 const double2* c = C + (int64_t)p * S + k1;
-                const double2* x = X + ((int64_t)ms * nbins + bin) * S + k1;
+                const int2 bm = binmap[bin];
+                const double2* x = X + ((int64_t)ms * nclass + bm.x) * S;
+                const int u = shifted_elem0<P>(k1, bm.y);
                 double2 v[P];
 #pragma unroll
-                for (int i = 0; i < P; i++) v[i] = cmulc(c[(int64_t)i * kRow], ld_nt(x + (int64_t)i * kRow));
+                for (int i = 0; i < P; i++) {
+                    const int e = u + i * kRow;
+                    v[i] = cmulc(c[(int64_t)i * kRow], ld_nt(x + (e >= P * kRow ? e - P * kRow : e)));
+                }
                 double2* a = ring_x + (int64_t)slot * S + k1;
                 const double2* tw = tw_col + k1;
                 dft_prime<P, 1>(v, [&](int k, double2 y) {
@@ -1175,17 +1192,15 @@
 bool acq_fft_supported(int64_t S) { return S == 13 * kRow || S == 29 * kRow; }
 
 template <class V>
-hipError_t launch_acq_fft_forward(const int8_t* iq, const double2* xs, int64_t S, int datalen, int nbins,
-                                  double IF, double freqMin, double freqStep, double Fs, const float* ca,
-                                  int nprn, double codeFreqBasis, const V* tw_row,
-                                  const V* tw_col, V* B, V* X, hipStream_t s, int bin0, int nbc, bool codes)
-{
-    const int nsig = datalen * nbins;
-    if (nbc < 0) nbc = nbins - bin0;
-    if (bin0 < 0 || nbc < 0 || bin0 + nbc > nbins) return hipErrorInvalidValue;
-    const FwdSet fs{nbins, nsig, nprn, bin0, nbc > 0 ? nbc : 1, codes ? 1 : 0};
-    const int ntr = (codes ? nprn : 0) + datalen * nbc;
-    if (ntr == 0) return hipSuccess;
+hipError_t launch_acq_fft_forward(const int8_t* iq, const double2* xs, int64_t S, int datalen, int nclass,
+                                  const int* cls_rep, double IF, double freqMin, double freqStep, double Fs,
+                                  const float* ca, int nprn, double codeFreqBasis, const V* tw_row,
+                                  const V* tw_col, V* B, V* X, hipStream_t s)
+{
+    if (nclass < 1 || datalen < 1 || nprn < 0) return hipErrorInvalidValue;
+    const int nsig = datalen * nclass;
+    const FwdSet fs{nclass, nsig, nprn, cls_rep};
+    const int ntr = nprn + nsig;
     const double step = codeFreqBasis / Fs;
 #define GNSS_FWD(P_)                                                                            \
     if (S == (int64_t)P_ * kRow) {                                                              \
@@ -1203,16 +1218,15 @@
 #undef GNSS_FWD
     return hipErrorInvalidValue;
 }
-template hipError_t launch_acq_fft_forward<float2>(const int8_t*, const double2*, int64_t, int, int, double,
-                                                   double, double, double, const float*, int, double,
-                                                   const float2*, const float2*, float2*, float2*, hipStream_t, int,
-                                                   int, bool);
-template hipError_t launch_acq_fft_forward<double2>(const int8_t*, const double2*, int64_t, int, int, double,
-                                                    double, double, double, const float*, int, double,
+template hipError_t launch_acq_fft_forward<float2>(const int8_t*, const double2*, int64_t, int, int, const int*,
+                                                   double, double, double, double, const float*, int, double,
+                                                   const float2*, const float2*, float2*, float2*, hipStream_t);
+template hipError_t launch_acq_fft_forward<double2>(const int8_t*, const double2*, int64_t, int, int, const int*,
+                                                    double, double, double, double, const float*, int, double,
                                                     const double2*, const double2*, double2*, double2*,
-                                                    hipStream_t, int, int, bool);
-
-hipError_t launch_acq_fft_correlate(const float2* C, const float2* X, int64_t S, int datalen,
+                                                    hipStream_t);
+
+hipError_t launch_acq_fft_correlate(const float2* C, const float2* X, const AcqShiftMap& sm, int64_t S, int datalen,
                                     int nbins, int nprn, int first_pair, int npair,
                                     const float2* tw_row, const float2* tw_col, float2* A,
                                     float* corr, hipStream_t s, int parts)
@@ -1223,8 +1237,8 @@
         if (parts & kAcqCols)                                                                   \
         hipLaunchKernelGGL((inv_cols_kernel<P_, float2>),                                       \
                            dim3((kRow + kColThreads - 1) / kColThreads, npair * datalen),       \
-                           dim3(kColThreads), 0, s, C, X, nbins, nprn, datalen, first_pair,     \
-                           tw_col, A);                                                          \
+                           dim3(kColThreads), 0, s, C, X, sm.binmap, sm.nclass, nprn, datalen,  \
+                           first_pair, tw_col, A);                                              \
         if (parts & kAcqRows)                                                                   \
         hipLaunchKernelGGL(inv_rows_kernel<P_>, dim3(P_, npair), dim3(kRowThreads), 0, s, A, nprn, \
                            datalen, first_pair, scale, tw_row, tw_col, corr, nbins);            \
@@ -1235,7 +1249,7 @@
     return hipErrorInvalidValue;
 }
 
-hipError_t launch_acq_fft_correlate(const double2* C, const double2* X, int64_t S, int datalen,
+hipError_t launch_acq_fft_correlate(const double2* C, const double2* X, const AcqShiftMap& sm, int64_t S, int datalen,
                                     int nbins, int nprn, int first_pair, int npair,
                                     const double2* tw_row, const double2* tw_col, double2* A,
                                     double* corr, hipStream_t s, int parts)
@@ -1246,8 +1260,8 @@
         if (parts & kAcqCols)                                                                   \
         hipLaunchKernelGGL((inv_cols_kernel<P_, double2>),                                      \
                            dim3((kRow + kColThreads - 1) / kColThreads, npair * datalen),       \
-                           dim3(kColThreads), 0, s, C, X, nbins, nprn, datalen, first_pair,     \
-                           tw_col, A);                                                          \
+                           dim3(kColThreads), 0, s, C, X, sm.binmap, sm.nclass, nprn, datalen,  \
+                           first_pair, tw_col, A);                                              \
         if (parts & kAcqRows)                                                                   \
         hipLaunchKernelGGL(inv_rows_kernel_f64<P_>, dim3(P_, npair), dim3(kRowThreads), 0, s, A, nprn, \
                            datalen, first_pair, scale, tw_row, tw_col, corr, nbins);            \
@@ -1258,7 +1272,8 @@
     return hipErrorInvalidValue;
 }
 
-hipError_t launch_acq_fft_pair(const double2* C, const double2* X, int64_t S, int datalen, int nbins, int nprn,
+hipError_t launch_acq_fft_pair(const double2* C, const double2* X, const AcqShiftMap& sm, int64_t S, int datalen,
+                               int nbins, int nprn,
                                int cols_first, int cols_n, double2* Acols, int rows_first, int rows_n,
                                const double2* Arows, const double2* tw_row, const double2* tw_col, double* corr,
                                int front, hipStream_t s)
@@ -1271,9 +1286,9 @@
         const int64_t nblk = (int64_t)P_ * rows_n + (int64_t)kCx * cols_n * datalen;             \
         if (nblk == 0) return hipSuccess;                                                       \
         if (nblk > INT32_MAX) return hipErrorInvalidConfiguration;                              \
-        hipLaunchKernelGGL(inv_pair_kernel_f64<P_>, dim3((unsigned)nblk), dim3(kRowThreads), 0, s, C, X, nbins, \
-                           nprn, datalen, cols_first, cols_n, Acols, rows_first, rows_n, Arows, scale, tw_row, \
-                           tw_col, corr, front);                                                \
+        hipLaunchKernelGGL(inv_pair_kernel_f64<P_>, dim3((unsigned)nblk), dim3(kRowThreads), 0, s, C, X, sm.binmap, \
+                           sm.nclass, nbins, nprn, datalen, cols_first, cols_n, Acols, rows_first, rows_n, Arows, \
+                           scale, tw_row, tw_col, corr, front);                                 \
         return hipGetLastError();                                                               \
     }
     static_assert(kColThreads == kRowThreads, "the paired launch runs both bodies in one block shape");
@@ -1286,8 +1301,8 @@
 size_t acq_fused_err_offset() { return offsetof(FuseSync, err); }
 size_t acq_fused_ring_bytes(int64_t S) { return sizeof(double2) * (size_t)kFuseX * kFuseSlots * (size_t)S; }
 
-hipError_t launch_acq_fft_correlate_fused(const double2* C, const double2* X, int64_t S, int datalen, int nbins,
-                                          int nprn, int nslot, const double2* tw_row, const double2* tw_col,
+hipError_t launch_acq_fft_correlate_fused(const double2* C, const double2* X, const AcqShiftMap& sm, int64_t S,
+                                          int datalen, int nbins, int nprn, int nslot, const double2* tw_row, const double2* tw_col,
                                           double2* ring, void* sync, double* corr, hipStream_t s)
 {
     if (nslot < 2 || nslot > kFuseSlots) return hipErrorInvalidValue;
@@ -1305,8 +1320,9 @@
         if (e != hipSuccess) return e;                                                          \
         const int grid = ncu * std::min(occ, 2);                                                \
         if (grid < 1) return hipErrorInvalidConfiguration;                                      \
-        hipLaunchKernelGGL(inv_fused_kernel_f64<P_>, dim3(grid), dim3(kRowThreads), 0, s, C, X, nbins, nprn, \
-                           datalen, nbins * nprn, nslot, scale, tw_row, tw_col, ring, sy, corr); \
+        hipLaunchKernelGGL(inv_fused_kernel_f64<P_>, dim3(grid), dim3(kRowThreads), 0, s, C, X, sm.binmap, \
+                           sm.nclass, nbins, nprn, datalen, nbins * nprn, nslot, scale, tw_row, tw_col, ring, sy, \
+                           corr);                                                               \
         return hipGetLastError();                                                               \
     }
     GNSS_FUSED(13) GNSS_FUSED(29)
@@ -1334,8 +1350,12 @@
 
 static size_t fine_prep_offset(const FineLayout& f, int nsv)
 {
-    const size_t b = sizeof(double2) * (size_t)(f.tabs + (int64_t)nsv * f.slab) + sizeof(FineBest) * (size_t)(nsv * f.part);
+    const size_t b = sizeof(double2) * (size_t)((int64_t)nsv * f.slab) + sizeof(FineBest) * (size_t)(nsv * f.part);
     return (b + 255) & ~(size_t)255;
+}
+size_t fine_fft_table_bytes(int64_t S, int L, int datalen)
+{
+    return sizeof(double2) * (size_t)fine_layout(S, L, datalen).tabs;
 }
 size_t fine_fft_scratch_bytes(int64_t S, int L, int datalen, int nsv)
 {
@@ -1344,10 +1364,10 @@
     return fine_prep_offset(f, nsv) + (size_t)nsv * f.M * (sizeof(double2) + sizeof(float));
 }
 
-hipError_t launch_fine_fft_tables(int64_t S, int L, int datalen, void* scratch, hipStream_t s)
+hipError_t launch_fine_fft_tables(int64_t S, int L, int datalen, void* tables, hipStream_t s)
 {
     const int64_t M = (int64_t)L * S;
-    double2* tw_row = static_cast<double2*>(scratch);
+    double2* tw_row = static_cast<double2*>(tables);
     double2* tabA = tw_row + kRow;
     double2* tabB = tabA + (int64_t)kRow * datalen;
     double2* tabK = tabB + (int64_t)kFineT * kRow;
@@ -1365,17 +1385,18 @@
 
 hipError_t launch_fine_fft_argmax(const int8_t* iq, const double2* xs, int64_t S, int L, int datalen,
                                   const int32_t* cd, int nsv, const float* ca, double Fs, double codeFreqBasis,
-                                  double codelength, int shifted, void* scratch, int64_t* kbest, hipStream_t s)
+                                  double codelength, int shifted, const void* tables, void* scratch, int64_t* kbest,
+                                  hipStream_t s)
 {
     if (nsv < 1 || nsv > 65535) return hipErrorInvalidValue;
     const FineLayout f = fine_layout(S, L, datalen);
     const int64_t N = f.N;
-    double2* tw_row = static_cast<double2*>(scratch);
-    double2* tabA = tw_row + kRow;
-    double2* tabB = tabA + (int64_t)kRow * datalen;
-    double2* tabK = tabB + (int64_t)kFineT * kRow;
-    double2* tabS = tabK + S;
-    double2* E = tw_row + f.tabs;
+    const double2* tw_row = static_cast<const double2*>(tables);
+    const double2* tabA = tw_row + kRow;
+    const double2* tabB = tabA + (int64_t)kRow * datalen;
+    const double2* tabK = tabB + (int64_t)kFineT * kRow;
+    const double2* tabS = tabK + S;
+    double2* E = static_cast<double2*>(scratch);
     FineBest* part = reinterpret_cast<FineBest*>(E + (int64_t)nsv * f.slab);
     char* prep = static_cast<char*>(scratch) + fine_prep_offset(f, nsv);
     float* ct = reinterpret_cast<float*>(prep + (size_t)nsv * f.M * sizeof(double2));
diff --git a/assignment-for-aae6102_gnss-sdr_amd/csrc/api_acq.cpp b/assignment-for-aae6102_gnss-sdr_amd/csrc/api_acq.cpp
--- a/assignment-for-aae6102_gnss-sdr_amd/csrc/api_acq.cpp
+++ b/assignment-for-aae6102_gnss-sdr_amd/csrc/api_acq.cpp
@@ -2,6 +2,7 @@
 #include <cstring>
 #include <vector>
 
+#include "acq_classes.h"
 #include "host.h"
 
 using namespace gnss;
@@ -9,10 +10,6 @@
 
 namespace {
 constexpr int kAcqPipeDefault = 2;
-#ifndef GNSS_ACQ_FWD_SPLIT
-#define GNSS_ACQ_FWD_SPLIT 1
-#endif
-constexpr bool kAcqFwdSplit = GNSS_ACQ_FWD_SPLIT;
 constexpr int kAcqPairFront = 60;
 constexpr int kFineBatch = 16;
 
@@ -55,9 +52,25 @@
             ctx->acq_tw_S = S;
             ctx->acq_tw_dbl = dbl;
         }
-        const size_t ntr = (size_t)nsig + np;
+        const AcqClasses cl = acq_bin_classes(acq->freqMin, acq->freqStep, nb, sg->Fs, S,
+                                              ctx->opt[GNSS_OPT_ACQ_OWN_CLASS] != 0);
+        const int ncl = (int)cl.rep.size(), nsig_c = dl * ncl;
+        std::vector<int32_t> tabh((size_t)2 * nb + ncl);
+        for (int b = 0; b < nb; b++) {
+            tabh[(size_t)2 * b] = cl.cls[(size_t)b];
+            tabh[(size_t)2 * b + 1] = (int32_t)(((int64_t)S - cl.shift[(size_t)b]) % S);
+        }
+        for (int c = 0; c < ncl; c++) tabh[(size_t)2 * nb + c] = cl.rep[(size_t)c];
+        DevBuf bins;
+        HIP_TRY(bins.alloc(ctx, "acq.bins", tabh.size() * sizeof(int32_t)));
+        HIP_TRY(hipMemcpyAsync(bins.p, tabh.data(), tabh.size() * sizeof(int32_t), hipMemcpyHostToDevice, ctx->stream));
+        const AcqShiftMap sm{bins.as<int2>(), ncl};
+        const int* cls_rep = bins.as<int>() + (size_t)2 * nb;
+        const size_t ntr = (size_t)nsig_c + np;
         HIP_TRY(B.alloc(ctx, "acq.B", csz * ntr * S));
-        HIP_TRY(X.alloc(ctx, "acq.X", csz * ntr * S));
+        HIP_TRY(X.alloc(ctx, "acq.X", csz * (ntr + 1) * S));
+        V* const Xs = X.as<V>() + S;
+        const V* const C = Xs + (size_t)nsig_c * S;
         const int npairs = nb * np;
         if (dbl && ctx->opt[GNSS_OPT_ACQ_FUSED]) {
             DevBuf ring;
@@ -66,11 +79,11 @@
             HIP_TRY(fsync.alloc(ctx, "acq.fsync", acq_fused_sync_bytes()));
             HIP_TRY(hipStreamSynchronize(ctx->stream));
             HIP_TRY(hipEventRecord(e_all.a, ctx->stream));
-            HIP_TRY(launch_acq_fft_forward<V>(blk, xa, S, dl, nb, sg->IF, acq->freqMin, acq->freqStep, sg->Fs, ca,
-                                              np, sg->codeFreqBasis, d_twr.as<V>(), d_twc.as<V>(), B.as<V>(),
-                                              X.as<V>(), ctx->stream));
-            const V* C = X.as<V>() + (size_t)nsig * S;
-            HIP_TRY(launch_acq_fft_correlate_fused(reinterpret_cast<const double2*>(C), X.as<double2>(), S, dl, nb,
+            HIP_TRY(launch_acq_fft_forward<V>(blk, xa, S, dl, ncl, cls_rep, sg->IF, acq->freqMin, acq->freqStep,
+                                              sg->Fs, ca, np, sg->codeFreqBasis, d_twr.as<V>(), d_twc.as<V>(),
+                                              B.as<V>(), Xs, ctx->stream));
+            HIP_TRY(launch_acq_fft_correlate_fused(reinterpret_cast<const double2*>(C),
+                                                   reinterpret_cast<const double2*>(Xs), sm, S, dl, nb,
                                                    np, nslot, d_twr.as<double2>(), d_twc.as<double2>(),
                                                    ring.as<double2>(), fsync.p, reinterpret_cast<double*>(corr),
                                                    ctx->stream));
@@ -90,22 +103,9 @@
         HIP_TRY(A.alloc(ctx, "acq.A", csz * abuf * (two || pair ? 2 : 1)));
         HIP_TRY(hipStreamSynchronize(ctx->stream));
         HIP_TRY(hipEventRecord(e_all.a, ctx->stream));
-        const bool fwd_split = kAcqFwdSplit && two;
-        auto fwd = [&](int bin0, int nbc, bool codes) {
-            return launch_acq_fft_forward<V>(blk, xa, S, dl, nb, sg->IF, acq->freqMin, acq->freqStep, sg->Fs, ca, np,
-                                             sg->codeFreqBasis, d_twr.as<V>(), d_twc.as<V>(), B.as<V>(), X.as<V>(),
-                                             ctx->stream, bin0, nbc, codes);
-        };
-        int fwd_bins = 0;
-        if (fwd_split) {
-            const int need = std::min(nb, (std::min(batch, npairs) - 1) / np + 1);
-            HIP_TRY(fwd(0, need, true));
-            fwd_bins = need;
-        } else {
-            HIP_TRY(fwd(0, -1, true));
-            fwd_bins = nb;
-        }
-        const V* C = X.as<V>() + (size_t)nsig * S;
+        HIP_TRY(launch_acq_fft_forward<V>(blk, xa, S, dl, ncl, cls_rep, sg->IF, acq->freqMin, acq->freqStep, sg->Fs,
+                                          ca, np, sg->codeFreqBasis, d_twr.as<V>(), d_twc.as<V>(), B.as<V>(), Xs,
+                                          ctx->stream));
         if (pair) {
             const char* fe = probe_env("GNSS_PAIR_FRONT");
             const int front = fe ? atoi(fe) : kAcqPairFront;
@@ -115,7 +115,8 @@
                 const int cq = b * batch, rq = (b - 1) * batch;
                 const int nc = b < nbt ? std::min(batch, npairs - cq) : 0;
                 const int nr = b > 0 ? std::min(batch, npairs - rq) : 0;
-                HIP_TRY(launch_acq_fft_pair(reinterpret_cast<const double2*>(C), X.as<double2>(), S, dl, nb, np, cq,
+                HIP_TRY(launch_acq_fft_pair(reinterpret_cast<const double2*>(C),
+                                            reinterpret_cast<const double2*>(Xs), sm, S, dl, nb, np, cq,
                                             nc, Ah[b & 1], rq, nr, Ah[(b + 1) & 1], d_twr.as<double2>(),
                                             d_twc.as<double2>(), reinterpret_cast<double*>(corr), front,
                                             ctx->stream));
@@ -125,7 +126,7 @@
         if (!two) {
             for (int q0 = 0; q0 < npairs; q0 += batch) {
                 const int nq = std::min(batch, npairs - q0);
-                HIP_TRY(launch_acq_fft_correlate(C, X.as<V>(), S, dl, nb, np, q0, nq, d_twr.as<V>(),
+                HIP_TRY(launch_acq_fft_correlate(C, Xs, sm, S, dl, nb, np, q0, nq, d_twr.as<V>(),
                                                  d_twc.as<V>(), A.as<V>(), corr, ctx->stream));
             }
             return GNSS_OK;
@@ -136,17 +137,12 @@
                 const int nq = std::min(batch, npairs - q0);
                 const int h = b & 1;
                 V* Ah = A.as<V>() + (size_t)h * abuf;
-                if (fwd_split) {
-                    const int need = std::min(nb, (q0 + nq - 1) / np + 1);
-                    if (need > fwd_bins) HIP_TRY(fwd(fwd_bins, need - fwd_bins, false));
-                    fwd_bins = std::max(fwd_bins, need);
-                }
                 if (b >= 2) HIP_TRY(hipStreamWaitEvent(s_cols, ctx->ev_rows[h], 0));
-                HIP_TRY(launch_acq_fft_correlate(C, X.as<V>(), S, dl, nb, np, q0, nq, d_twr.as<V>(), d_twc.as<V>(),
+                HIP_TRY(launch_acq_fft_correlate(C, Xs, sm, S, dl, nb, np, q0, nq, d_twr.as<V>(), d_twc.as<V>(),
                                                  Ah, corr, s_cols, kAcqCols));
                 HIP_TRY(hipEventRecord(ctx->ev_cols[h], s_cols));
                 HIP_TRY(hipStreamWaitEvent(s_rows, ctx->ev_cols[h], 0));
-                HIP_TRY(launch_acq_fft_correlate(C, X.as<V>(), S, dl, nb, np, q0, nq, d_twr.as<V>(), d_twc.as<V>(),
+                HIP_TRY(launch_acq_fft_correlate(C, Xs, sm, S, dl, nb, np, q0, nq, d_twr.as<V>(), d_twc.as<V>(),
                                                  Ah, corr, s_rows, kAcqRows));
                 HIP_TRY(hipEventRecord(ctx->ev_rows[h], s_rows));
                 last = h;
@@ -376,13 +372,23 @@
     if (own_fine) {
         const int fb = std::min(na, kFineBatch);
         HIP_TRY(fx.alloc(ctx, "acq.fx", fine_fft_scratch_bytes(S, L, dl, fb)));
+        DevBuf ftab;
+        HIP_TRY(ftab.alloc(ctx, "acq.fine_tabs", fine_fft_table_bytes(S, L, dl)));
+        const bool have_tabs = ctx->fine_tab_S == S && ctx->fine_tab_L == L && ctx->fine_tab_dl == dl;
         HIP_TRY(hipEventRecord(e_fine.a, ctx->stream));
-        HIP_TRY(launch_fine_fft_tables(S, L, dl, fx.p, ctx->stream));
+        if (!have_tabs) {
+            ctx->fine_tab_S = 0;
+            HIP_TRY(launch_fine_fft_tables(S, L, dl, ftab.p, ctx->stream));
+            ctx->fine_tab_S = S;
+            ctx->fine_tab_L = L;
+            ctx->fine_tab_dl = dl;
+        }
         for (int k0 = 0; k0 < na; k0 += fb) {
             const int nk = std::min(fb, na - k0);
             HIP_TRY(launch_fine_fft_argmax(blk, xf, S, L, dl, fcd.as<int32_t>() + k0, nk,
                                            fca.as<float>() + (size_t)k0 * 1023, sg->Fs, sg->codeFreqBasis,
-                                           sg->codelength, fshift, fx.p, kb.as<int64_t>() + k0, ctx->stream));
+                                           sg->codelength, fshift, ftab.p, fx.p, kb.as<int64_t>() + k0,
+                                           ctx->stream));
         }
     } else {
         HIP_TRY(fx.alloc(ctx, "acq.fx", sizeof(double2) * (size_t)na * N));
diff --git a/assignment-for-aae6102_gnss-sdr_amd/csrc/gnss_internal.h b/assignment-for-aae6102_gnss-sdr_amd/csrc/gnss_internal.h
--- a/assignment-for-aae6102_gnss-sdr_amd/csrc/gnss_internal.h
+++ b/assignment-for-aae6102_gnss-sdr_amd/csrc/gnss_internal.h
@@ -413,36 +413,43 @@
 
 bool acq_fft_supported(int64_t S);
 template <class V>
-hipError_t launch_acq_fft_forward(const int8_t* iq, const double2* xs, int64_t S, int datalen, int nbins, double IF,
-                                  double freqMin, double freqStep, double Fs, const float* ca,
-                                  int nprn, double codeFreqBasis, const V* tw_row,
-                                  const V* tw_col, V* B, V* X, hipStream_t s, int bin0 = 0, int nbc = -1,
-                                  bool codes = true);
+hipError_t launch_acq_fft_forward(const int8_t* iq, const double2* xs, int64_t S, int datalen, int nclass,
+                                  const int* cls_rep, double IF, double freqMin, double freqStep, double Fs,
+                                  const float* ca, int nprn, double codeFreqBasis, const V* tw_row,
+                                  const V* tw_col, V* B, V* X, hipStream_t s);
+struct AcqShiftMap {
+    const int2* binmap;
+    int nclass;
+};
 constexpr int kAcqCols = 1, kAcqRows = 2;
-hipError_t launch_acq_fft_correlate(const float2* C, const float2* X, int64_t S, int datalen,
+hipError_t launch_acq_fft_correlate(const float2* C, const float2* X, const AcqShiftMap& sm, int64_t S, int datalen,
                                     int nbins, int nprn, int first_pair, int npair,
                                     const float2* tw_row, const float2* tw_col, float2* A,
                                     float* corr, hipStream_t s, int parts = kAcqCols | kAcqRows);
-hipError_t launch_acq_fft_correlate(const double2* C, const double2* X, int64_t S, int datalen,
+hipError_t launch_acq_fft_correlate(const double2* C, const double2* X, const AcqShiftMap& sm, int64_t S, int datalen,
                                     int nbins, int nprn, int first_pair, int npair,
                                     const double2* tw_row, const double2* tw_col, double2* A,
                                     double* corr, hipStream_t s, int parts = kAcqCols | kAcqRows);
-hipError_t launch_acq_fft_pair(const double2* C, const double2* X, int64_t S, int datalen, int nbins, int nprn,
+hipError_t launch_acq_fft_pair(const double2* C, const double2* X, const AcqShiftMap& sm, int64_t S, int datalen,
+                               int nbins, int nprn,
                                int cols_first, int cols_n, double2* Acols, int rows_first, int rows_n,
                                const double2* Arows, const double2* tw_row, const double2* tw_col, double* corr,
                                int front, hipStream_t s);
 size_t acq_fused_sync_bytes();
 size_t acq_fused_err_offset();
 size_t acq_fused_ring_bytes(int64_t S);
-hipError_t launch_acq_fft_correlate_fused(const double2* C, const double2* X, int64_t S, int datalen, int nbins,
-                                          int nprn, int nslot, const double2* tw_row, const double2* tw_col,
-                                          double2* ring, void* sync, double* corr, hipStream_t s);
+hipError_t launch_acq_fft_correlate_fused(const double2* C, const double2* X, const AcqShiftMap& sm, int64_t S,
+                                          int datalen, int nbins, int nprn, int nslot, const double2* tw_row,
+                                          const double2* tw_col, double2* ring, void* sync, double* corr,
+                                          hipStream_t s);
 bool fine_fft_supported(int64_t S, int L);
+size_t fine_fft_table_bytes(int64_t S, int L, int datalen);
 size_t fine_fft_scratch_bytes(int64_t S, int L, int datalen, int nsv);
-hipError_t launch_fine_fft_tables(int64_t S, int L, int datalen, void* scratch, hipStream_t s);
+hipError_t launch_fine_fft_tables(int64_t S, int L, int datalen, void* tables, hipStream_t s);
 hipError_t launch_fine_fft_argmax(const int8_t* iq, const double2* xs, int64_t S, int L, int datalen,
                                   const int32_t* cd, int nsv, const float* ca, double Fs, double codeFreqBasis,
-                                  double codelength, int shifted, void* scratch, int64_t* kbest, hipStream_t s);
+                                  double codelength, int shifted, const void* tables, void* scratch,
+                                  int64_t* kbest, hipStream_t s);
 hipError_t launch_fine_build(const int8_t* iq, const double2* xs, int64_t S, int L, const int32_t* codedelay,
                              const float* ca, int nsv, double Fs, double codeFreqBasis,
                              double codelength, int64_t N, double2* out, hipStream_t s);
diff --git a/assignment-for-aae6102_gnss-sdr_amd/csrc/host.h b/assignment-for-aae6102_gnss-sdr_amd/csrc/host.h
--- a/assignment-for-aae6102_gnss-sdr_amd/csrc/host.h
+++ b/assignment-for-aae6102_gnss-sdr_amd/csrc/host.h
@@ -31,6 +31,8 @@
     std::map<std::string, std::pair<void*, size_t>> pinned;
     int64_t acq_tw_S = 0;
     int acq_tw_dbl = -1;
+    int64_t fine_tab_S = 0;
+    int fine_tab_L = 0, fine_tab_dl = 0;
     int acq_fp64 = 1;
     uint64_t window = 0;
     int64_t opt[GNSS_OPT_COUNT] = {};
diff --git a/include/gnss_mi355x.h b/include/gnss_mi355x.h
--- a/include/gnss_mi355x.h
+++ b/include/gnss_mi355x.h
@@ -157,7 +157,8 @@
 #define GNSS_OPT_FORCE_PEER   10
 #define GNSS_OPT_VT_SPAN      11
 #define GNSS_OPT_SLOT_PATH    12
-#define GNSS_OPT_COUNT        13
+#define GNSS_OPT_ACQ_OWN_CLASS 13
+#define GNSS_OPT_COUNT        14
 int  gnss_ctx_set_option(gnss_ctx *ctx, int key, int64_t value);
 int  gnss_lane_boundaries(const double *taps, const double *post, int n_taps, int lane_samples,
                           double cps_max);
```
